# kahrendt/microWakeWord

Measured on AMD Instinct MI355X. Metric: spectrogram-windows/sec (train step) on default mixednet, higher is better.
Workload: dtype f32

## Files before the change

microwakeword_amd/csrc/block_launch.hip.h:

```cpp
#pragma once
#include "kernels_bwd.hip.h"

#define MWW_ODD_KS(X, CI, CO) X(CI, CO, 3) X(CI, CO, 5) X(CI, CO, 7) X(CI, CO, 9) X(CI, CO, 11) X(CI, CO, 13) X(CI, CO, 15) \
  X(CI, CO, 17) X(CI, CO, 19) X(CI, CO, 21) X(CI, CO, 23)
#define MWW_FIRST_KS(X, K1, CO, S) X(K1, 32, CO, 3, S) X(K1, 32, CO, 5, S) X(K1, 32, CO, 7, S)
#define MWW_FIRST_STRIDES(X, K1, CO) MWW_FIRST_KS(X, K1, CO, 1) MWW_FIRST_KS(X, K1, CO, 2) MWW_FIRST_KS(X, K1, CO, 3)
#ifdef MWW_SLIM
#define MWW_FIRST_SHAPES(X) X(3, 32, 48, 5, 1)
#define MWW_BLOCK_SHAPES(X) X(48, 48, 9) X(48, 48, 13) X(48, 48, 21)
#define MWW_FIRST_SHAPES_BF16(X) MWW_FIRST_SHAPES(X)
#define MWW_BLOCK_SHAPES_BF16(X) MWW_BLOCK_SHAPES(X)
#else
#define MWW_FIRST_SHAPES(X)                                                                                   \
  MWW_FIRST_STRIDES(X, 3, 32) MWW_FIRST_STRIDES(X, 3, 48) MWW_FIRST_STRIDES(X, 3, 64)                         \
  MWW_FIRST_STRIDES(X, 5, 32) MWW_FIRST_STRIDES(X, 5, 48) MWW_FIRST_STRIDES(X, 5, 64)
#define MWW_BLOCK_SHAPES(X)                                                                                   \
  MWW_ODD_KS(X, 32, 32) MWW_ODD_KS(X, 48, 48) MWW_ODD_KS(X, 64, 64) MWW_ODD_KS(X, 32, 48) MWW_ODD_KS(X, 32, 64)   \
  MWW_ODD_KS(X, 48, 64) MWW_ODD_KS(X, 48, 32) MWW_ODD_KS(X, 64, 48) MWW_ODD_KS(X, 64, 32)
#define MWW_FIRST_SHAPES_BF16(X) X(3, 32, 48, 5, 1) X(5, 32, 64, 5, 3) X(5, 32, 64, 5, 1) X(3, 32, 64, 5, 1) X(5, 32, 48, 5, 3) X(5, 32, 48, 5, 1)
#define MWW_BLOCK_SHAPES_BF16(X)                                                                              \
  X(48, 48, 5) X(48, 48, 9) X(48, 48, 13) X(48, 48, 21) X(48, 48, 11) X(48, 48, 15) X(48, 48, 23)             \
  X(64, 64, 11) X(64, 64, 15) X(64, 64, 23) X(64, 64, 5) X(64, 64, 9) X(64, 64, 13) X(64, 64, 21)
#endif

namespace mww {

bool k_launch_fwd_first(hipStream_t st, int mode, int k1, int c1, int cout, int k, int stride, const FwdFirstArgs& a, int grid, bool x6);
bool k_launch_fwd_block(hipStream_t st, int mode, int cin, int cout, int k, const FwdBlockArgs& a, int grid);
bool k_launch_bwd_first(hipStream_t st, int mode, int k1, int c1, int cout, int k, int stride, const BwdFirstArgs& a, int grid, bool x6);
bool k_launch_bwd_block(hipStream_t st, int mode, int cin, int cout, int k, bool last, const BwdBlockArgs& a, int grid);
bool k_launch_bwd_blockw(hipStream_t st, int mode, int cin, int cout, int k, bool last, const BwdBlockArgs& a, int grid);
bool k_launch_bwd_firstw(hipStream_t st, int k1, int c1, int cout, int k, int stride, const BwdFirstArgs& a, int grid, bool wide_x6);

}
```

microwakeword_amd/csrc/bwd_first_body.inc:

```
  constexpr int CIN = C1;
  constexpr int CPI = pitch(CIN), CPO = pitch(COUT);
  constexpr int RA = TT + K - 1;
  constexpr int TAIL = S > 1 ? K - 1 : 0;
  constexpr int TAILK = (TAIL + 3) / 4 * 4;
  constexpr int XR = (TT + TAILK - 1) * S + K1;
  constexpr int NT1 = C1 / 16;
  constexpr int M1 = K1 * FBINS;
  constexpr int MT1 = (M1 + 15) / 16;
  constexpr int MPW = (MT1 + 3) / 4;
  constexpr int MT = CIN / 16, NT = COUT / 16, KSO = COUT / 4;
  constexpr int NCH = nchunks(CIN), L = chunk_len(CIN);
  constexpr int QI = CIN / 4;
  constexpr int RAP = halo_rows_padded(CIN, K), TTP = tile_rows_padded(CIN);
  constexpr int OFF_A = 0, OFF_DP = OFF_A + RAP * CPI, OFF_U = OFF_DP + TT * CPO, OFF_DU = OFF_U + TTP * CPI;
  constexpr int PB = 96, PLB = XR * PB, GPB = 2 * CIN, GPL = TT * GPB;
  static_assert(!X6 || (S == 1 && CIN == 32 && (K1 * FBINS) % 8 == 0 && 3 * GPL <= (TT * CPO + TTP * CPI) * 4 && TTP == TT), "the x6 form serves the stride-1 first convolutions");
  constexpr int OFF_G0 = OFF_DU + RAP * CPI, OFF_END = X6 ? OFF_G0 : OFF_G0 + (TTP + TAILK) * CPI;
  static_assert(TAIL <= NCH && TTP + TAIL <= RAP, "tail rows");
  constexpr int PX = FBINS + 1;
  static_assert(OFF_END >= 4 * CIN * COUT && OFF_END >= NCH * (K + 1) * CIN, "scratch aliasing");
  static_assert(TT >= K - 1, "shape");

  float* sA = smem + OFF_A;
  float* sDP = smem + OFF_DP;
  float* sU = smem + OFF_U;
  float* sDU = smem + OFF_DU;
  float* sG0 = smem + OFF_G0;

  const int tid = threadIdx.x, lane = tid & 63, wave = tid >> 6, r16 = lane & 15, g = lane >> 4;
  const int c = tid % CIN, chunk = tid / CIN;
  const bool dw_active = chunk < NCH;
  const int Ta = (a.T - K1) / S + 1;

  const bool tailmode = TAIL > 0 && Ta > TT && Ta <= TT + TAIL;
  const int ntiles = tailmode ? 1 : (Ta + TT - 1) / TT;
  const int nsamp = (int)blockIdx.x < a.B ? (a.B - (int)blockIdx.x + (int)gridDim.x - 1) / (int)gridDim.x : 0;
  const int nitems = nsamp * ntiles;
  XStage<XR, PX, MWW_AUX_LD_XB> xs;
  DpStage<COUT, false, SB> dps;
  constexpr int NA = (RA * QI + kThreads - 1) / kThreads;
  float4 pre_a[NA];
  auto issue = [&](int it) {
    const int s = it / ntiles, b = blockIdx.x + s * gridDim.x, t0 = (it % ntiles) * TT;
    const int nrx = ((tailmode ? Ta : min(TT, Ta - t0)) - 1) * S + K1;
    xs.issue(a.x, a.xg, sXg, s, b, a.T, t0 * S, nrx, tid);
    const BufRsrc ra = tile_rsrc(a.a0 + ((size_t)b * Ta + t0) * CIN, min(RA, Ta - t0) * QI * 16);
#pragma unroll
    for (int j = 0; j < NA; ++j) pre_a[j] = tile_load4<MWW_AUX_LD_A0>(ra, (tid + j * kThreads) * 16);
    const int nvk = max(0, min(TT, a.Tout - t0)) * (COUT / 4);
    const size_t koff = ((size_t)b * a.Tout + t0) * COUT;
    dps.issue(elem_ptr<SB>(a.pk, koff), elem_ptr<SB>(a.gk, koff), nvk, tid);
  };
  int offm[MPW];
  bool okm[MPW];
  int xoff[MPW], goff[NT1];
  if constexpr (X6) {
    const int rowl = 4 * g + (r16 >> 2), cg = 4 * (r16 & 3);
#pragma unroll
    for (int mi = 0; mi < MPW; ++mi) {
      const int m = min((wave * MPW + mi) * 16 + cg, M1 - 4);
      xoff[mi] = (rowl + m / FBINS) * PB + (m % FBINS) * 2;
    }
#pragma unroll
    for (int nt = 0; nt < NT1; ++nt) goff[nt] = rowl * GPB + ((nt * 16 + cg) ^ ((rowl & 4) ? 16 : 0)) * 2;
  } else {
#pragma unroll
  for (int mi = 0; mi < MPW; ++mi) {
    const int m = (wave * MPW + mi) * 16 + r16;
    okm[mi] = m < M1;
    offm[mi] = okm[mi] ? (m / FBINS) * PX + (m % FBINS) : 0;
  }
  }
  if (a.xg.win) xgather_setup(a.xg, sXg, nsamp, tid);
  stagger_start<MWW_STAGGER_BWD>();
  if (nitems > 0) issue(0);

  WeightStage<CIN, COUT, 0, pitch_wt(CIN, BF)> wst;
  wst.load(a.pw_w, nullptr, tid);
  float dww[K], accw[K];
  float accb = 0.f, dwb = 0.f;
#pragma unroll
  for (int i = 0; i < K; ++i) {
    dww[i] = dw_active ? a.dw_w[i * CIN + c] : 0.f;
    accw[i] = 0.f;
  }
  if (dw_active) dwb = a.dw_b[c];
  for (int i = tid; i < COUT; i += kThreads) {
    const float krs = a.k_rstd[i];
    const float kmean = a.k_mean[i];
    float c1, mg, mgx;
    if (a.gfold.acc) {
      bn_grad_fold_channel(a.gfold, COUT, i, krs, c1, mg, mgx);
    } else {
      c1 = a.k_c1[i];
      mg = a.k_mg[i];
      mgx = a.k_mgx[i];
    }
    const float kA = -c1 * krs * mgx;
    sKp[0 * COUT + i] = c1;
    sKp[1 * COUT + i] = kA;
    sKp[2 * COUT + i] = -c1 * mg - kA * kmean;
    sKp[5 * COUT + i] = 0.f;
    sKp[6 * COUT + i] = 0.f;
  }
  wst.store(sWt, nullptr, tid);
  for (int i = RA * CPI + tid; i < RAP * CPI; i += kThreads) {
    sA[i] = 0.f;
    sDU[i] = 0.f;
  }
  if constexpr (!X6)
    for (int i = TTP * CPI + tid; i < (TTP + TAILK) * CPI; i += kThreads) sG0[i] = 0.f;
#pragma unroll
  for (int i = 0; i < K; ++i) pin(dww[i]);
  pin(dwb);
  f32x4 dwacc[MT][NT];
#pragma unroll
  for (int mt = 0; mt < MT; ++mt)
#pragma unroll
    for (int nt = 0; nt < NT; ++nt) dwacc[mt][nt] = zero4();
  f32x4 w1acc[MPW][NT1];
#pragma unroll
  for (int mi = 0; mi < MPW; ++mi)
#pragma unroll
    for (int nt = 0; nt < NT1; ++nt) w1acc[mi][nt] = zero4();
  __syncthreads();

  for (int it = 0; it < nitems; ++it) {
    rotate_priority(it, 2);
    const int t0 = (it % ntiles) * TT;
    const int nrows_new = max(0, min(TT, a.Tout - t0));
    const int rows_da = min(TT, Ta - t0);
    if constexpr (X6) xs.template commit_planes<PB, PLB>(reinterpret_cast<unsigned*>(sX), a.xg, sXg, it / ntiles, t0 * S, tid);
    else xs.commit(sX, a.xg, sXg, it / ntiles, t0 * S, tid);
#pragma unroll
    for (int j = 0; j < NA; ++j) {
      const int i = tid + j * kThreads;
      if (i < RA * QI) {
        const int r = i / QI, q = i - r * QI;
        *reinterpret_cast<float4*>(sA + r * CPI + q * 4) = pre_a[j];
      }
    }
    dps.commit(sDP, sKp, 0.f, nrows_new * (COUT / 4), tid);
    carry_du<K, CPI>(sDU, t0 == 0, tid);
    __syncthreads();
    if (it + 1 < nitems) issue(it + 1);
    if (dw_active) {
      if (chunk * L < nrows_new) {
        float o[L];
        dw_chunk<K, L>(sA, CPI, chunk * L, c, dww, dwb, o);
#pragma unroll
        for (int t = 0; t < L; ++t) {
          const int tl = chunk * L + t;
          sU[tl * CPI + c] = (tl < nrows_new) ? o[t] : 0.f;
        }
      } else {
#pragma unroll
        for (int t = 0; t < L; ++t) sU[(chunk * L + t) * CPI + c] = 0.f;
      }
    }
    __syncthreads();
    pointwise_backward_tile<CIN, COUT, K, BF>(sU, sDP, sDU, wave, r16, g, sWt, dwacc, wave * 16 < nrows_new);
    __syncthreads();
    if (dw_active) {
      float wdu[L + K - 1], wa[L + K - 1];
#pragma unroll
      for (int j = 0; j < L + K - 1; ++j) wdu[j] = sDU[(chunk * L + j) * CPI + c];
#pragma unroll
      for (int j = 0; j < L + K - 1; ++j) wa[j] = sA[(chunk * L + j) * CPI + c];
      lds_reads_first();
#pragma unroll
      for (int t = 0; t < L; ++t) {
        const int sl = chunk * L + t;
        float acc = 0.f;
#pragma unroll
        for (int i = 0; i < K; ++i) acc = fmaf(dww[K - 1 - i], wdu[t + i], acc);
        const float gv = (sl < rows_da && wa[t] > 0.f) ? acc : 0.f;
        if constexpr (X6) {
          unsigned h0, h1, h2;
          split3(gv, h0, h1, h2);
          unsigned short* gp = reinterpret_cast<unsigned short*>(sDP) + sl * CIN + (c ^ ((sl & 4) ? 16 : 0));
          gp[0] = (unsigned short)(h0 >> 16);
          gp[GPL / 2] = (unsigned short)(h1 >> 16);
          gp[GPL] = (unsigned short)(h2 >> 16);
        } else {
          sG0[sl * CPI + c] = gv;
        }
      }
      if (chunk * L < nrows_new) {
#pragma unroll
        for (int t = 0; t < L; ++t) {
          const float dut = wdu[K - 1 + t];
          accb += dut;
#pragma unroll
          for (int i = 0; i < K; ++i) accw[i] = fmaf(dut, wa[t + i], accw[i]);
        }
      }
      if constexpr (TAIL > 0) {
        if (tailmode && chunk < TAIL) {
          const int sl = TT + chunk;
          float acc = 0.f;
#pragma unroll
          for (int j = 0; j < K; ++j) acc = fmaf(dww[K - 1 - j], sl + j < RAP ? sDU[(sl + j) * CPI + c] : 0.f, acc);
          sG0[sl * CPI + c] = (sl < Ta && sA[sl * CPI + c] > 0.f) ? acc : 0.f;
        }
      }
    }
    __syncthreads();
    if constexpr (X6) {
      const char* xb = reinterpret_cast<const char*>(sX);
      const char* gb = reinterpret_cast<const char*>(sDP);
#pragma unroll
      for (int kb = 0; kb < TT / 32; ++kb)
#pragma unroll
        for (int nt = 0; nt < NT1; ++nt) {
          u32x4v gq[3];
#pragma unroll
          for (int p = 0; p < 3; ++p) {
            const u32x2v lo = lds_read_tr16(gb + goff[nt] + p * GPL + (32 * kb) * GPB), hi = lds_read_tr16(gb + goff[nt] + p * GPL + (32 * kb + 16) * GPB);
            gq[p] = u32x4v{lo.x, lo.y, hi.x, hi.y};
          }
#pragma unroll
          for (int mi = 0; mi < MPW; ++mi) {
            u32x4v xq[3];
#pragma unroll
            for (int p = 0; p < 3; ++p) {
              const u32x2v lo = lds_read_tr16(xb + xoff[mi] + p * PLB + (32 * kb) * S * PB), hi = lds_read_tr16(xb + xoff[mi] + p * PLB + (32 * kb + 16) * S * PB);
              xq[p] = u32x4v{lo.x, lo.y, hi.x, hi.y};
            }
            w1acc[mi][nt] = mfma_x6(xq, gq, w1acc[mi][nt]);
          }
        }
    } else {
      float av[2][MPW], bv[2][NT1];
      auto load_w1 = [&](int kk, int sl) {
        const int s = kk * 4 + g;
#pragma unroll
        for (int nt = 0; nt < NT1; ++nt) bv[sl][nt] = sG0[s * CPI + nt * 16 + r16];
#pragma unroll
        for (int mi = 0; mi < MPW; ++mi) {
          const float v = sX[s * S * PX + offm[mi]];
          av[sl][mi] = okm[mi] ? v : 0.f;
        }
      };
      load_w1(0, 0);
#pragma unroll
      for (int kk = 0; kk < TT / 4; ++kk) {
        if (kk + 1 < TT / 4) load_w1(kk + 1, (kk + 1) & 1);
#pragma unroll
        for (int mi = 0; mi < MPW; ++mi)
#pragma unroll
          for (int nt = 0; nt < NT1; ++nt) w1acc[mi][nt] = mfma4(av[kk & 1][mi], bv[kk & 1][nt], w1acc[mi][nt]);
      }
      __builtin_amdgcn_sched_group_barrier(0x100, MPW + NT1, 0);
      sched_read_mfma_groups<TT / 4 - 1, MPW + NT1, MPW * NT1>();
      sched_read_mfma_groups<1, 0, MPW * NT1>();
      if constexpr (TAIL > 0) {
        if (tailmode) {
#pragma unroll
          for (int ks = 0; ks < TAILK / 4; ++ks) {
            load_w1(TT / 4 + ks, 0);
#pragma unroll
            for (int mi = 0; mi < MPW; ++mi)
#pragma unroll
              for (int nt = 0; nt < NT1; ++nt) w1acc[mi][nt] = mfma4(av[0][mi], bv[0][nt], w1acc[mi][nt]);
          }
        }
      }
    }
    __syncthreads();
  }
  float* gdst = a.grad_part + (size_t)blockIdx.x * (M1 * C1 + (K + 1) * CIN + CIN * COUT);
#pragma unroll
  for (int mi = 0; mi < MPW; ++mi)
#pragma unroll
    for (int nt = 0; nt < NT1; ++nt)
#pragma unroll
      for (int r = 0; r < 4; ++r) {
        const int m = (wave * MPW + mi) * 16 + g * 4 + r;
        if (m < M1) gdst[m * C1 + nt * 16 + r16] = w1acc[mi][nt][r];
      }
  write_block_grad_partials<CIN, COUT, K>(smem, gdst + M1 * C1, dwacc, accw, accb, dw_active, c, chunk, tid, wave, r16, g);
```

microwakeword_amd/csrc/common.hip.h:

```cpp
#pragma once
#include <hip/hip_runtime.h>
#include <stdint.h>

namespace mww {

typedef float f32x4 __attribute__((ext_vector_type(4)));

constexpr int kThreads = 256;
constexpr int TT = 64;
constexpr int FBINS = 40;
constexpr float kBnEps = 1e-3f;
constexpr float kBnMomentum = 0.99f;
constexpr float kKerasEps = 1e-7f;

constexpr int kHeadTraining = 1, kHeadClippedLoss = 2;
__device__ __forceinline__ float bce_value(float z, float pr, float yy, bool clipped_form) {
  if (!clipped_form) return fmaxf(z, 0.f) - z * yy + log1pf(expf(-fabsf(z)));
  const float pc = fminf(fmaxf(pr, kKerasEps), 1.0f - kKerasEps);
  return -(yy * logf(pc) + (1.0f - yy) * logf(1.0f - pc));
}
__device__ __forceinline__ float bce_dz(float pr, float yy, bool clipped_form) {
  if (clipped_form && ((pr < kKerasEps) || (pr > 1.0f - kKerasEps))) return 0.f;
  return pr - yy;
}

__device__ __forceinline__ f32x4 mfma4(float a, float b, f32x4 c) {
  return __builtin_amdgcn_mfma_f32_16x16x4f32(a, b, c, 0, 0, 0);
}

typedef __bf16 bf16x4 __attribute__((ext_vector_type(4)));
typedef short s16x4 __attribute__((ext_vector_type(4)));

__device__ __forceinline__ f32x4 mfma_bf16(bf16x4 a, bf16x4 b, f32x4 c) {
  return __builtin_amdgcn_mfma_f32_16x16x16bf16_1k(__builtin_bit_cast(s16x4, a), __builtin_bit_cast(s16x4, b), c, 0, 0, 0);
}

__device__ __forceinline__ bf16x4 to_bf16x4(float a, float b, float c, float d) {
  bf16x4 v = {(__bf16)a, (__bf16)b, (__bf16)c, (__bf16)d};
  return v;
}

typedef __bf16 bf16x8 __attribute__((ext_vector_type(8)));
typedef unsigned u32x4v __attribute__((ext_vector_type(4)));
typedef unsigned u32x2v __attribute__((ext_vector_type(2)));
__device__ __forceinline__ f32x4 mfma_bf16k32(u32x4v a, u32x4v b, f32x4 c) {
  return __builtin_amdgcn_mfma_f32_16x16x32_bf16(__builtin_bit_cast(bf16x8, a), __builtin_bit_cast(bf16x8, b), c, 0, 0, 0);
}
__device__ __forceinline__ void split3(float v, unsigned& h0, unsigned& h1, unsigned& h2) {
  h0 = __float_as_uint(v) & 0xffff0000u;
  const float r1 = v - __uint_as_float(h0);
  h1 = __float_as_uint(r1) & 0xffff0000u;
  const float r2 = r1 - __uint_as_float(h1);
  h2 = __float_as_uint(r2) & 0xffff0000u;
}
__device__ __forceinline__ unsigned pack_hi2(unsigned a, unsigned b) { return (a >> 16) | b; }
__device__ __forceinline__ void split3x8(const float (&v)[8], u32x4v (&q)[3]) {
  unsigned h[3][8];
#pragma unroll
  for (int e = 0; e < 8; ++e) split3(v[e], h[0][e], h[1][e], h[2][e]);
#pragma unroll
  for (int p = 0; p < 3; ++p)
#pragma unroll
    for (int d = 0; d < 4; ++d) q[p][d] = pack_hi2(h[p][2 * d], h[p][2 * d + 1]);
}
__device__ __forceinline__ f32x4 mfma_x6(const u32x4v (&xs)[3], const u32x4v (&ws)[3], f32x4 acc) {
  acc = mfma_bf16k32(xs[2], ws[0], acc);
  acc = mfma_bf16k32(xs[1], ws[1], acc);
  acc = mfma_bf16k32(xs[0], ws[2], acc);
  acc = mfma_bf16k32(xs[1], ws[0], acc);
  acc = mfma_bf16k32(xs[0], ws[1], acc);
  acc = mfma_bf16k32(xs[0], ws[0], acc);
  return acc;
}
__device__ __forceinline__ void pin4(u32x4v& v) { asm volatile("" : "+v"(v)); }
__device__ __forceinline__ u32x2v lds_read_tr16(const void* lds_ptr) {
  typedef short s16x4t __attribute__((ext_vector_type(4)));
  const s16x4t v = __builtin_amdgcn_ds_read_tr16_b64_v4i16((__attribute__((address_space(3))) s16x4t*)(lds_ptr));
  return __builtin_bit_cast(u32x2v, v);
}

__device__ __forceinline__ f32x4 zero4() {
  f32x4 z = {0.f, 0.f, 0.f, 0.f};
  return z;
}

__host__ __device__ constexpr int pitch(int c) { return c + 4; }
#ifndef MWW_FWD_PITCH_A
#define MWW_FWD_PITCH_A 1
#endif
#ifndef MWW_FWD_PITCH_U
#define MWW_FWD_PITCH_U 1
#endif
__host__ __device__ constexpr int pitch_fa(int c) { return (MWW_FWD_PITCH_A && c == 48) ? 48 : c + 4; }
__host__ __device__ constexpr int pitch_fu(int c, bool bf) { return (MWW_FWD_PITCH_U && !bf) ? c + 2 : c + 4; }

__host__ __device__ constexpr int pitch_wt(int c, bool bf) { return bf ? c + 4 : (c % 32 == 16 ? c : c + 16); }

__host__ __device__ constexpr int nchunks(int c) { return kThreads / c; }
__host__ __device__ constexpr int chunk_len(int c) { return (TT + nchunks(c) - 1) / nchunks(c); }
__host__ __device__ constexpr int tile_rows_padded(int c) { return nchunks(c) * chunk_len(c); }
__host__ __device__ constexpr int halo_rows_padded(int c, int k) { return tile_rows_padded(c) + k - 1; }

typedef __amdgpu_buffer_rsrc_t BufRsrc;
typedef unsigned u32x4 __attribute__((ext_vector_type(4)));
typedef unsigned u32x2 __attribute__((ext_vector_type(2)));

__device__ __forceinline__ BufRsrc tile_rsrc(const void* base, int bytes) {
  const int n = __builtin_amdgcn_readfirstlane(bytes > 0 ? bytes : 0);
  return __builtin_amdgcn_make_buffer_rsrc(const_cast<void*>(base), (short)0, n, 0x00020000);
}
#ifndef MWW_AUX_ST_P
#define MWW_AUX_ST_P 16
#endif
#ifndef MWW_AUX_ST_G
#define MWW_AUX_ST_G 16
#endif
#ifndef MWW_AUX_ST_A0
#define MWW_AUX_ST_A0 2
#endif
#ifndef MWW_AUX_LD_FP
#define MWW_AUX_LD_FP 0
#endif
#ifndef MWW_AUX_LD_BP
#define MWW_AUX_LD_BP 2
#endif
#ifndef MWW_AUX_LD_A0
#define MWW_AUX_LD_A0 2
#endif
#ifndef MWW_AUX_LD_PK
#define MWW_AUX_LD_PK 2
#endif
#ifndef MWW_AUX_LD_GK
#define MWW_AUX_LD_GK 2
#endif
#ifndef MWW_AUX_LD_XF
#define MWW_AUX_LD_XF 0
#endif
#ifndef MWW_AUX_LD_XB
#define MWW_AUX_LD_XB 0
#endif
#ifndef MWW_AUX_LD_HP
#define MWW_AUX_LD_HP 0
#endif
#ifndef MWW_AUX_ST_GP
#define MWW_AUX_ST_GP 1
#endif
#ifndef MWW_AUX_GR_ST_P
#define MWW_AUX_GR_ST_P 1
#endif
#ifndef MWW_AUX_GR_ST_G
#define MWW_AUX_GR_ST_G 0
#endif
#ifndef MWW_AUX_GR_LD_GOLD
#define MWW_AUX_GR_LD_GOLD 0
#endif
#ifndef MWW_AUX_GR_ST_GP
#define MWW_AUX_GR_ST_GP 0
#endif
#ifndef MWW_AUX_GR_LD_DP
#define MWW_AUX_GR_LD_DP 0
#endif
template <int WT>
__device__ __forceinline__ void store_stream(float* p, float v) {
  if constexpr (WT != 0) __hip_atomic_store(p, v, __ATOMIC_RELAXED, __HIP_MEMORY_SCOPE_AGENT);
  else *p = v;
}
template <int AUX = 0>
__device__ __forceinline__ float4 tile_load4(BufRsrc r, int byte_off) {
  const u32x4 v = __builtin_amdgcn_raw_buffer_load_b128(r, byte_off, 0, AUX);
  return make_float4(__uint_as_float(v.x), __uint_as_float(v.y), __uint_as_float(v.z), __uint_as_float(v.w));
}
template <int AUX = 0>
__device__ __forceinline__ uint2 tile_load2(BufRsrc r, int byte_off) {
  const u32x2 v = __builtin_amdgcn_raw_buffer_load_b64(r, byte_off, 0, AUX);
  uint2 o;
  o.x = v.x;
  o.y = v.y;
  return o;
}
template <int AUX = 0>
__device__ __forceinline__ float tile_load1(BufRsrc r, int byte_off) {
  return __uint_as_float(__builtin_amdgcn_raw_buffer_load_b32(r, byte_off, 0, AUX));
}
template <int AUX = 0>
__device__ __forceinline__ void tile_store1(BufRsrc r, int byte_off, float v) {
  __builtin_amdgcn_raw_buffer_store_b32(__float_as_uint(v), r, byte_off, 0, AUX);
}
template <bool SB, int AUX = 0>
__device__ __forceinline__ float4 tile_load4s(BufRsrc r, int group) {
  if constexpr (!SB) {
    return tile_load4<AUX>(r, group * 16);
  } else {
    const uint2 v = tile_load2<AUX>(r, group * 8);
    return make_float4(__uint_as_float(v.x << 16), __uint_as_float(v.x & 0xffff0000u), __uint_as_float(v.y << 16),
                       __uint_as_float(v.y & 0xffff0000u));
  }
}
template <bool SB, int AUX = 0>
__device__ __forceinline__ void tile_store1s(BufRsrc r, int elem, float v) {
  if constexpr (!SB) {
    tile_store1<AUX>(r, elem * 4, v);
  } else {
    const __bf16 h = (__bf16)v;
    __builtin_amdgcn_raw_buffer_store_b16(__builtin_bit_cast(unsigned short, h), r, elem * 2, 0, AUX);
  }
}
template <bool SB>
__device__ __forceinline__ float load_elem(const float* base, size_t elem) {
  if constexpr (!SB) {
    return base[elem];
  } else {
    const unsigned dw = reinterpret_cast<const unsigned*>(base)[elem >> 1];
    return __uint_as_float((elem & 1) ? (dw & 0xffff0000u) : (dw << 16));
  }
}
__host__ __device__ constexpr int elem_bytes(bool sb) { return sb ? 2 : 4; }
template <bool SB>
__device__ __forceinline__ const float* elem_ptr(const float* base, size_t elem) {
  return reinterpret_cast<const float*>(reinterpret_cast<const char*>(base) + elem * (SB ? 2 : 4));
}
template <bool SB>
__device__ __forceinline__ float* elem_ptr(float* base, size_t elem) {
  return reinterpret_cast<float*>(reinterpret_cast<char*>(base) + elem * (SB ? 2 : 4));
}

constexpr int kOobOffset = 0x40000000;

__device__ __forceinline__ void lds_reads_first() {
  __builtin_amdgcn_sched_group_barrier(0x100, 64, 0);
  __builtin_amdgcn_sched_group_barrier(0x002, 2048, 0);
}

__device__ __forceinline__ void rotate_priority(int item, int levels) {
  const int p = ((int)(blockIdx.x >> 8) + item) & (levels - 1);
  if (levels == 2) {
    if (p) __builtin_amdgcn_s_setprio(1);
    else __builtin_amdgcn_s_setprio(0);
  } else {
    if (p == 0) __builtin_amdgcn_s_setprio(0);
    else if (p == 1) __builtin_amdgcn_s_setprio(1);
    else if (p == 2) __builtin_amdgcn_s_setprio(2);
    else __builtin_amdgcn_s_setprio(3);
  }
}

#ifndef MWW_STAGGER_BWD
#define MWW_STAGGER_BWD 47
#endif
#ifndef MWW_STAGGER_FWD
#define MWW_STAGGER_FWD 0
#endif
#ifndef MWW_STAGGER_GRAPH
#define MWW_STAGGER_GRAPH 0
#endif
#ifndef MWW_G_FWD_DIRECT
#define MWW_G_FWD_DIRECT 1
#endif
#ifndef MWW_G_WGRAD_EVEN
#define MWW_G_WGRAD_EVEN 1
#endif
#ifndef MWW_G_STEM_BREG
#define MWW_G_STEM_BREG 0
#endif
#ifndef MWW_G_WGRAD_XG_NARROW
#define MWW_G_WGRAD_XG_NARROW 0
#endif
template <int UNITS>
__device__ __forceinline__ void stagger_start() {
  if constexpr (UNITS > 0) {
    const int pos = (int)(blockIdx.x >> 8);
    for (int i = 0; i < pos; ++i) __builtin_amdgcn_s_sleep(UNITS);
  }
}

__device__ __forceinline__ void pin(float& v) { asm volatile("" : "+v"(v)); }
__device__ __forceinline__ void pin(int& v) { asm volatile("" : "+v"(v)); }

#ifdef MWW_PROFILE
#define MWW_ABLATE(a, bits) ((a).ablate & (bits))
#else
#define MWW_ABLATE(a, bits) 0
#endif
#ifdef MWW_PROFILE
#define MWW_PC_DECL PhaseClock pc;
#define MWW_PC_START(en) pc.start(en)
#define MWW_PC_MARK(i) pc.mark(i)
#define MWW_PC_DUMP(p) do { if (p) pc.dump(p); } while (0)
#define MWW_PC_AT(i) pc.at(i)
#else
#define MWW_PC_AT(i) ((void)0)
#define MWW_PC_DECL
#define MWW_PC_START(en) ((void)0)
#define MWW_PC_MARK(i) ((void)0)
#define MWW_PC_DUMP(p) ((void)0)
#endif
constexpr int kClkSlots = 12;
struct PhaseClock {
  unsigned long long last = 0, acc[8] = {0, 0, 0, 0, 0, 0, 0, 0}, stamp[4] = {0, 0, 0, 0};
  bool on = false;
  __device__ __forceinline__ void at(int i) { stamp[i] = __builtin_amdgcn_s_memtime(); }
  __device__ __forceinline__ void start(bool enable) {
    on = enable;
    if (on) last = __builtin_amdgcn_s_memtime();
  }
  __device__ __forceinline__ void mark(int slot) {
    if (on) {
      const unsigned long long t = __builtin_amdgcn_s_memtime();
      acc[slot] += t - last;
      last = t;
    }
  }
  __device__ __forceinline__ void dump(unsigned long long* dst) const {
    if (on) {
      for (int i = 0; i < 8; ++i) dst[i] = acc[i];
      for (int i = 0; i < 4; ++i) dst[8 + i] = stamp[i];
    }
  }
};

__device__ __forceinline__ void fast_divmod(int a, int b, int& q, int& r) {
  q = (int)((float)a * __frcp_rn((float)b));
  r = a - q * b;
  if (r >= b) {
    ++q;
    r -= b;
  } else if (r < 0) {
    --q;
    r += b;
  }
}
__device__ __forceinline__ int fast_div(int a, int b) {
  int q, r;
  fast_divmod(a, b, q, r);
  return q;
}

__device__ __forceinline__ int uniform_int(int v) { return __builtin_amdgcn_readfirstlane(v); }
__device__ __forceinline__ long long uniform_i64(long long v) {
  const unsigned lo = (unsigned)__builtin_amdgcn_readfirstlane((int)(unsigned)(unsigned long long)v);
  const unsigned hi = (unsigned)__builtin_amdgcn_readfirstlane((int)(unsigned)((unsigned long long)v >> 32));
  return (long long)(((unsigned long long)hi << 32) | lo);
}
__device__ __forceinline__ const void* uniform_ptr(const void* p) {
  return reinterpret_cast<const void*>((uintptr_t)uniform_i64((long long)(uintptr_t)p));
}

__device__ __forceinline__ float sum_over_groups(float v) {
  v += __shfl_xor(v, 16);
  v += __shfl_xor(v, 32);
  return v;
}

__device__ __forceinline__ float wave_sum(float v) {
  v += __shfl_xor(v, 1);
  v += __shfl_xor(v, 2);
  v += __shfl_xor(v, 4);
  v += __shfl_xor(v, 8);
  v += __shfl_xor(v, 16);
  v += __shfl_xor(v, 32);
  return v;
}

constexpr int kStatRows = 8;

struct StatAcc {
  double* acc;
  double* clear;
};

__device__ __forceinline__ void publish_stat(const StatAcc& s, float* row, int C2, int tid, float v) {
  if (s.acc) {
    unsafeAtomicAdd(s.acc + (size_t)(blockIdx.x % kStatRows) * C2 + tid, (double)v);
    for (int r = blockIdx.x; r < kStatRows; r += gridDim.x)
      __hip_atomic_store(s.clear + (size_t)r * C2 + tid, 0.0, __ATOMIC_RELAXED, __HIP_MEMORY_SCOPE_AGENT);
  } else {
    row[tid] = v;
  }
}

struct BnFoldArgs {
  const double* acc;
  float inv_n;
  int update_moving;
  const float* gamma;
  const float* beta;
  float* moving_mean;
  float* moving_var;
  float* scale;
  float* shift;
  float* mean;
  float* rstd;
};

__device__ __forceinline__ void bn_fold_channel(const BnFoldArgs& f, int C, int ch, float& sc, float& sh, float& meanf, float& rstd) {
  double s1 = 0.0, s2 = 0.0;
  double v1[kStatRows], v2[kStatRows];
#pragma unroll
  for (int j = 0; j < kStatRows; ++j) {
    v1[j] = f.acc[(size_t)j * 2 * C + ch];
    v2[j] = f.acc[(size_t)j * 2 * C + C + ch];
  }
  const float gam = f.gamma[ch], bet = f.beta[ch];
  float mm_old = 0.f, mv_old = 0.f;
  if (blockIdx.x == 0 && f.update_moving) {
    mm_old = f.moving_mean[ch];
    mv_old = f.moving_var[ch];
  }
#pragma unroll
  for (int j = 0; j < kStatRows; ++j) {
    s1 += v1[j];
    s2 += v2[j];
  }
  const double m = s1 * (double)f.inv_n;
  double var = s2 * (double)f.inv_n - m * m;
  if (var < 0.0) var = 0.0;
  meanf = (float)m;
  const float varf = (float)var;
  rstd = 1.0f / sqrtf(varf + kBnEps);
  sc = gam * rstd;
  sh = bet - meanf * sc;
  if (blockIdx.x == 0) {
    f.scale[ch] = sc;
    f.shift[ch] = sh;
    f.mean[ch] = meanf;
    f.rstd[ch] = rstd;
    if (f.update_moving) {
      f.moving_mean[ch] = mm_old * kBnMomentum + meanf * (1.0f - kBnMomentum);
      f.moving_var[ch] = mv_old * kBnMomentum + varf * (1.0f - kBnMomentum);
    }
  }
}

struct BnGradFoldArgs {
  const double* acc;
  float inv_n;
  float dscale;
  const float* gamma;
  float* c1;
  float* mg;
  float* mgx;
  float* dgamma;
  float* dbeta;
};

__device__ __forceinline__ void bn_grad_fold_channel(const BnGradFoldArgs& f, int C, int ch, float rstd, float& c1, float& mg, float& mgx) {
  double s1 = 0.0, s2 = 0.0;
  double v1[kStatRows], v2[kStatRows];
#pragma unroll
  for (int j = 0; j < kStatRows; ++j) {
    v1[j] = f.acc[(size_t)j * 2 * C + ch];
    v2[j] = f.acc[(size_t)j * 2 * C + C + ch];
  }
  const float gam = f.gamma[ch];
#pragma unroll
  for (int j = 0; j < kStatRows; ++j) {
    s1 += v1[j];
    s2 += v2[j];
  }
  c1 = gam * rstd;
  mg = (float)(s1 * (double)f.inv_n);
  mgx = (float)(s2 * (double)f.inv_n);
  if (blockIdx.x == 0) {
    f.dbeta[ch] = (float)s1 * f.dscale;
    f.dgamma[ch] = (float)s2 * f.dscale;
    f.c1[ch] = c1;
    f.mg[ch] = mg;
    f.mgx[ch] = mgx;
  }
}

}
```

microwakeword_amd/csrc/engine.hip.h:

```cpp
#pragma once
#include <hip/hip_runtime.h>

#include <map>
#include <string>
#include <utility>
#include <vector>

#include "../../include/mww.h"
#include "kernels_bwd.hip.h"
#include "kernels_data.hip.h"

#ifndef MWW_CONV1_X6_DEFAULT
#define MWW_CONV1_X6_DEFAULT 1
#endif
#ifndef MWW_CONV1_X6_FWD_DEFAULT
#define MWW_CONV1_X6_FWD_DEFAULT 0
#endif
#ifndef MWW_BWD_FIRST_WIDE_DEFAULT
#define MWW_BWD_FIRST_WIDE_DEFAULT 0
#endif
#ifndef MWW_BWD_WIDE_DEFAULT
#define MWW_BWD_WIDE_DEFAULT 1
#endif

namespace mww {

struct MetricState;

int fail(int code, const std::string& msg);

#define HIPCHK(expr)                                                                              \
  do {                                                                                            \
    hipError_t e_ = (expr);                                                                       \
    if (e_ != hipSuccess)                                                                         \
      return fail(MWW_ERR_HIP, std::string(#expr) + ": " + hipGetErrorString(e_));                \
  } while (0)

struct Layer {
  int cin, cout, k, tin, tout;
  int64_t o_dw_w, o_dw_b, o_pw_w, o_gamma, o_beta, o_mm, o_mv;
  float* p = nullptr;
  float* g = nullptr;
  float* stat_part = nullptr;
  float* gstat_part = nullptr;
  float* grad_part = nullptr;
  int grad_part_stride = 0;
  float* bn = nullptr;
  double* facc[2] = {nullptr, nullptr};
  double* gacc[2] = {nullptr, nullptr};
  double* facc_cur = nullptr;
  double* gacc_cur = nullptr;
};

struct GOp {
  int n_src = 0, src[MWW_MAX_OP_SOURCES] = {0, 0, 0}, toff[MWW_MAX_OP_SOURCES] = {0, 0, 0};
  int sc0[MWW_MAX_OP_SOURCES] = {0, 0, 0}, scn[MWW_MAX_OP_SOURCES] = {0, 0, 0};
  bool src_first[MWW_MAX_OP_SOURCES] = {false, false, false}, src_last[MWW_MAX_OP_SOURCES] = {false, false, false};
  int k = 1, dil = 1, cin = 0, cout = 0, groups = 1, slots = 0, tin = 0, tout = 0;
  int kind = MWW_OP_CONV, stride = 1, norm = MWW_NORM_BN, act = MWW_ACT_RELU;
  int res_src = -1, res_drop = 0;
  std::vector<int> adders;
  int64_t o_w = 0, o_gamma = 0, o_beta = 0, o_mm = 0, o_mv = 0;
  float *p = nullptr, *g = nullptr, *stat_part = nullptr, *gstat_part = nullptr, *grad_part = nullptr, *bn = nullptr;
  bool needs_dx = false;
  bool twin_next = false;
  int planes = 1, pc = 0;
  size_t lds_fwd = 0, lds_dx = 0, lds_wg = 0;
  double* facc[2] = {nullptr, nullptr};
  double* gacc[2] = {nullptr, nullptr};
  double* facc_cur = nullptr;
  double* gacc_cur = nullptr;
  int first_consumer = -1;
};

struct ProfileEntry {
  std::string name;
  hipEvent_t a, b;
};

struct RcclApi {
  void* so = nullptr;
  struct UniqueId { char internal[128]; };
  int (*GetUniqueId)(UniqueId*) = nullptr;
  int (*CommInitRank)(void**, int, UniqueId, int) = nullptr;
  int (*AllReduce)(const void*, void*, size_t, int, int, void*, hipStream_t) = nullptr;
  int (*CommDestroy)(void*) = nullptr;
  int (*CommCount)(void*, int*) = nullptr;
  const char* (*GetErrorString)(int) = nullptr;
};

constexpr int kRing = 8;
constexpr int kDenseChunks = 32;

}

struct mww_ctx {
  mww_mixednet_desc d;
  int device = 0;
  hipStream_t stream = nullptr;
  bool own_stream = false;
  int n_cu = 256;
  int grid_fwd = 0, grid_bwd = 0, grid_head = 0;
  bool conv1_x6 = MWW_CONV1_X6_DEFAULT != 0;
  bool conv1_x6_fwd = MWW_CONV1_X6_FWD_DEFAULT != 0;
  bool bwd_first_wide = MWW_BWD_FIRST_WIDE_DEFAULT != 0;
  bool bwd_wide = MWW_BWD_WIDE_DEFAULT != 0;
  int64_t P = 0, S = 0;
  int64_t o_conv1 = 0, o_dense_w = 0, o_dense_b = 0;
  int t_last = 0, c_last = 0, dwd_stride = 0;
  std::vector<mww::Layer> L;
  bool generic = false;
  std::vector<mww::GOp> G;
  float dropout = 0.f;
  float* keep = nullptr;
  bool keep_explicit = false;
  unsigned long long dropout_seed = 0x5EEDull, dropout_counter = 0;
  bool head2 = false;
  bool head_att = false;
  int head_pool = 0;
  int64_t o_att = 0;
  float *hact = nullptr, *watt_part = nullptr;
  size_t lds_head2 = 0;
  float *ones = nullptr, *zeros = nullptr;
  int grid_g = 0;
  int g_cap_fwd = 4, g_cap_bwd = 4;
  int metric_launches = 0;
  bool g_planar = true;
  bool g_static = true;
  int g_chunks = 0;
  int g_dgrad_share = 50;
  bool grid_g_auto = true;
  std::map<std::pair<const void*, size_t>, int> g_occ;
  mww_allreduce_fn hook = nullptr;
  void* hook_user = nullptr;
  int world = 1;
  bool sync_bn = false, reduce_grads = false;
  struct RcclState* rccl = nullptr;
  float* sync_buf = nullptr;
  std::vector<int64_t> sync_off;
  float *params = nullptr, *grads = nullptr, *adam_m = nullptr, *adam_v = nullptr, *mask = nullptr;
  unsigned char* direct = nullptr;
  std::vector<unsigned char> direct_host;
  bool exchange_pending = false;
  int grad_buckets = 1;
  float* bn_state = nullptr;
  float *x = nullptr, *y = nullptr, *sw = nullptr, *z = nullptr, *prob = nullptr, *dz = nullptr, *loss_part = nullptr;
  float* a0 = nullptr;
  float* gbuf[2] = {nullptr, nullptr};
  float* dwd_part = nullptr;
  mww::MetricState* metrics = nullptr;
  char* mail_host[mww::kRing] = {};
  char* mail_dev[mww::kRing] = {};
  hipEvent_t mail_ev[mww::kRing] = {};
  int mail_cur = 0;
  bool mail_open = false;
  size_t mail_off_masks = 0, mail_off_y = 0, mail_off_sw = 0, mail_off_hyper = 0, mail_bytes = 0;
  int targets_in_mail = 0;
  hipStream_t copy_stream = nullptr;
  char* mail_hbm[mww::kRing] = {};
  hipEvent_t ev_copy[mww::kRing] = {};
  hipStream_t side = nullptr;
  hipEvent_t ev_fork = nullptr, ev_join = nullptr;
  bool side_pending = false;
  int asm_split = 2;
  bool fused_input = true;
  bool x_lazy = false;
  int lazy_slot = -1;
  mww::AssembleArgs lazy_a;
  const float* y_cur = nullptr;
  const float* sw_cur = nullptr;
  bool bn_inline = true;
  bool g_role_split = true;
  bool g_inline_ok = false;
  int fpar = 0, gpar = 0;
  bool tail_pending = false, tail_metrics = false;
  bool tail_in_reduce = false;
  bool tail_roles = true;
  void* store[MWW_MAX_STORES] = {};
  int store_dtype[MWW_MAX_STORES] = {};
  int64_t store_elems[MWW_MAX_STORES] = {};
  int64_t step = 0;
  int have_batch = 0, have_targets = 0;
  bool use_graphs = false, profile = false;
  bool profile_split = false;
  bool use_side = false;
  bool pw_bf16 = false;
  bool st_bf16 = false;
  bool bce_clipped = false;
  bool bn_eval_ready = false;
  int ablate = 0;
  unsigned long long* phase_clk = nullptr;
  std::vector<mww::ProfileEntry> prof;
  struct GraphEntry { int B, flags, mail, par; hipGraphExec_t exec; };
  std::vector<GraphEntry> graphs;
};

namespace mww {

struct Launcher {
  mww_ctx* c;
  hipEvent_t ea = nullptr;
  const char* name = nullptr;
  size_t idx = 0;
  void begin(const char* n, int layer = -1) {
    if (!c->profile) return;
    name = n;
    idx = c->prof.size();
    ProfileEntry e;
    e.name = n;
    if (layer >= 0) e.name += std::to_string(layer + 1);
    (void)hipEventCreate(&e.a);
    (void)hipEventCreate(&e.b);
    (void)hipEventRecord(e.a, c->stream);
    c->prof.push_back(e);
  }
  void end() {
    if (!c->profile || idx >= c->prof.size()) return;
    (void)hipEventRecord(c->prof[idx].b, c->stream);
  }
};

enum { BN_SCALE = 0, BN_SHIFT, BN_MEAN, BN_RSTD, BN_C1, BN_MG, BN_MGX };

const float* mail_hyper(mww_ctx* c);
int materialise_x(mww_ctx* c);
XGather x_gather(mww_ctx* c);
int enqueue_side_work(mww_ctx* c, int B, bool metrics, bool loss, const float* p_last, const float* scale, const float* shift, const float* keep);
struct StatSource { const float* part; int G; float inv_n; float dscale; };
int exchange_stats(mww_ctx* c, Launcher& lp, const char* what, int layer, const float* part, int G, int C, int bwd, float local_inv_n, StatSource* out);
int enqueue_grad_assembly(mww_ctx* c, int B, GradReduceArgs& ga, bool fuse_adam, int64_t lo = 0, int64_t hi = -1, bool last_range = true);

constexpr size_t kMaxDynLds = 144 * 1024;
constexpr long long kPlanePad = 1088;
int g_planes(const mww_ctx* c, const GOp& o);
long long g_pstride(const mww_ctx* c, const GOp& o);
bool g_stem_gathers(const mww_ctx* c);
struct GPlan {
  std::vector<GOp> ops;
  int64_t P = 0, S = 0;
  bool inline_ok = false;
  int chunks = 0;
};
int g_plan_convnet(const mww_convnet_desc& d, GPlan* plan);
int g_enqueue_forward(mww_ctx* c, int B, bool training, bool update_moving, bool loss, bool metrics);
int g_enqueue_backward(mww_ctx* c, int B, bool fuse_adam);

}
```

microwakeword_amd/csrc/kernels_bwd.hip.h:

```cpp
#pragma once
#include "kernels_fwd.hip.h"

namespace mww {

struct BwdBlockArgs {
  const float* in;
  const float* in_scale;
  const float* in_shift;
  const float* in_mean;
  const float* in_rstd;
  const float* pk;
  const float* gk;
  const float* k_mean;
  const float* k_rstd;
  const float* k_c1;
  const float* k_mg;
  const float* k_mgx;
  const float* k_scale;
  const float* k_shift;
  const float* wd;
  const float* dz;
  const float* dw_w;
  const float* dw_b;
  const float* pw_w;
  float* g_out;
  float* gstat_part;
  float* grad_part;
  int B, Tin, Tout;
  int ablate;
  unsigned long long* phase_clk;
  StatAcc gacc;
  BnGradFoldArgs gfold;
};

template <int COUT, bool LAST, bool SB = false>
struct DpStage {
  static constexpr int QO = COUT / 4, CPO = pitch(COUT), N = (TT * QO + kThreads - 1) / kThreads;
  float4 pk[N], gg[N];

  __device__ __forceinline__ void issue(const float* pk_base, const float* g_base, int nvalid, int tid) {
    constexpr bool SG = SB && !LAST;
    const BufRsrc rp = tile_rsrc(pk_base, nvalid * 4 * elem_bytes(SB)), rg = tile_rsrc(g_base, nvalid * 4 * elem_bytes(SG));
#pragma unroll
    for (int j = 0; j < N; ++j) {
      pk[j] = tile_load4s<SB, MWW_AUX_LD_PK>(rp, tid + j * kThreads);
      gg[j] = tile_load4s<SG, MWW_AUX_LD_GK>(rg, tid + j * kThreads);
    }
  }

  __device__ __forceinline__ void commit(float* sDP, const float* sKp, float dzb, int nvalid, int tid) const {
#pragma unroll
    for (int j = 0; j < N; ++j) {
      const int i = tid + j * kThreads;
      if (i < TT * QO) {
        const int r = i / QO, q = i - r * QO;
        float4 dp = make_float4(0.f, 0.f, 0.f, 0.f);
        if (i < nvalid) {
          const float4 p = pk[j];
          const float4 c1 = *reinterpret_cast<const float4*>(sKp + 0 * COUT + q * 4);
          const float4 kA = *reinterpret_cast<const float4*>(sKp + 1 * COUT + q * 4);
          const float4 kB = *reinterpret_cast<const float4*>(sKp + 2 * COUT + q * 4);
          float4 g = gg[j];
          if (LAST) {
            const float4 sc = *reinterpret_cast<const float4*>(sKp + 5 * COUT + q * 4);
            const float4 sh = *reinterpret_cast<const float4*>(sKp + 6 * COUT + q * 4);
            g.x = fmaf(p.x, sc.x, sh.x) > 0.f ? dzb * g.x : 0.f;
            g.y = fmaf(p.y, sc.y, sh.y) > 0.f ? dzb * g.y : 0.f;
            g.z = fmaf(p.z, sc.z, sh.z) > 0.f ? dzb * g.z : 0.f;
            g.w = fmaf(p.w, sc.w, sh.w) > 0.f ? dzb * g.w : 0.f;
          }
          dp.x = fmaf(g.x, c1.x, fmaf(p.x, kA.x, kB.x));
          dp.y = fmaf(g.y, c1.y, fmaf(p.y, kA.y, kB.y));
          dp.z = fmaf(g.z, c1.z, fmaf(p.z, kA.z, kB.z));
          dp.w = fmaf(g.w, c1.w, fmaf(p.w, kA.w, kB.w));
        }
        *reinterpret_cast<float4*>(sDP + r * CPO + q * 4) = dp;
      }
    }
  }
};

template <int CIN, int COUT, int KD, int PWT = pitch(CIN)>
struct WeightStage {
  static constexpr int CPI = PWT, NW = (CIN * COUT + kThreads - 1) / kThreads, ND = KD > 0 ? (KD * CIN + kThreads - 1) / kThreads : 1;
  float w[NW], d[ND];
  __device__ __forceinline__ void load(const float* pw_w, const float* dw_w, int tid) {
#pragma unroll
    for (int j = 0; j < NW; ++j) w[j] = (tid + j * kThreads < CIN * COUT) ? pw_w[tid + j * kThreads] : 0.f;
#pragma unroll
    for (int j = 0; j < ND; ++j) d[j] = (KD > 0 && tid + j * kThreads < KD * CIN) ? dw_w[tid + j * kThreads] : 0.f;
  }
  __device__ __forceinline__ void store(float* sWt, float* sDW, int tid) const {
#pragma unroll
    for (int j = 0; j < NW; ++j) {
      const int i = tid + j * kThreads;
      if (i < CIN * COUT) sWt[(i % COUT) * CPI + i / COUT] = w[j];
    }
    if (KD > 0) {
#pragma unroll
      for (int j = 0; j < ND; ++j)
        if (tid + j * kThreads < KD * CIN) sDW[tid + j * kThreads] = d[j];
    }
  }
};

template <int K, int CPI>
__device__ __forceinline__ void carry_du(float* sDU, bool first_tile, int tid) {
  for (int i = tid; i < (K - 1) * CPI; i += kThreads) sDU[i] = first_tile ? 0.f : sDU[TT * CPI + i];
}

template <int REPS, int READS, int MFMAS>
__device__ __forceinline__ void sched_read_mfma_groups() {
  if constexpr (REPS > 0) {
    if constexpr (READS > 0) __builtin_amdgcn_sched_group_barrier(0x100, READS, 0);
    __builtin_amdgcn_sched_group_barrier(0x008, MFMAS, 0);
    sched_read_mfma_groups<REPS - 1, READS, MFMAS>();
  }
}

template <int CIN, int COUT, int K, bool BF>
__device__ __forceinline__ void pointwise_backward_tile(const float* sU, const float* sDP, float* sDU, int wave, int r16,
                                                        int g, const float* sWt,
                                                        f32x4 (&dwacc)[CIN / 16][COUT / 16], bool live) {
  constexpr int CPI = pitch(CIN), CPO = pitch(COUT), MT = CIN / 16, NT = COUT / 16, KSO = COUT / 4;
  constexpr int PWT = pitch_wt(CIN, BF);
  f32x4 du[MT];
#pragma unroll
  for (int mt = 0; mt < MT; ++mt) du[mt] = zero4();
  if (!live) {
  } else if constexpr (!BF) {
    {
      float av[2][MT], bv[2][NT];
      auto load_dw = [&](int kk, int s) {
        const int row = wave * 16 + kk + 4 * g;
#pragma unroll
        for (int mt = 0; mt < MT; ++mt) av[s][mt] = sU[row * CPI + mt * 16 + r16];
#pragma unroll
        for (int nt = 0; nt < NT; ++nt) bv[s][nt] = sDP[row * CPO + nt * 16 + r16];
      };
      float a2[2], b2[2][MT];
      auto load_du = [&](int kk, int s) {
        a2[s] = sDP[(wave * 16 + r16) * CPO + kk * 4 + g];
#pragma unroll
        for (int mt = 0; mt < MT; ++mt) b2[s][mt] = sWt[(kk * 4 + g) * PWT + mt * 16 + r16];
      };
      load_dw(0, 0);
#pragma unroll
      for (int kk = 0; kk < 4; ++kk) {
        if (kk + 1 < 4) load_dw(kk + 1, (kk + 1) & 1);
        else load_du(0, 0);
#pragma unroll
        for (int mt = 0; mt < MT; ++mt)
#pragma unroll
          for (int nt = 0; nt < NT; ++nt) dwacc[mt][nt] = mfma4(av[kk & 1][mt], bv[kk & 1][nt], dwacc[mt][nt]);
      }
#pragma unroll
      for (int kk = 0; kk < KSO; ++kk) {
        if (kk + 1 < KSO) load_du(kk + 1, (kk + 1) & 1);
#pragma unroll
        for (int mt = 0; mt < MT; ++mt) du[mt] = mfma4(a2[kk & 1], b2[kk & 1][mt], du[mt]);
      }
      __builtin_amdgcn_sched_group_barrier(0x100, MT + NT, 0);
      sched_read_mfma_groups<3, MT + NT, MT * NT>();
      sched_read_mfma_groups<1, 1 + MT, MT * NT>();
      sched_read_mfma_groups<KSO - 1, 1 + MT, MT>();
      sched_read_mfma_groups<1, 0, MT>();
    }
  } else {
    const int row = wave * 16 + 4 * g;
    bf16x4 av[MT], bv[NT];
#pragma unroll
    for (int mt = 0; mt < MT; ++mt) {
      const float* col = sU + row * CPI + mt * 16 + r16;
      av[mt] = to_bf16x4(col[0], col[CPI], col[2 * CPI], col[3 * CPI]);
    }
#pragma unroll
    for (int nt = 0; nt < NT; ++nt) {
      const float* col = sDP + row * CPO + nt * 16 + r16;
      bv[nt] = to_bf16x4(col[0], col[CPO], col[2 * CPO], col[3 * CPO]);
    }
#pragma unroll
    for (int mt = 0; mt < MT; ++mt)
#pragma unroll
      for (int nt = 0; nt < NT; ++nt) dwacc[mt][nt] = mfma_bf16(av[mt], bv[nt], dwacc[mt][nt]);
#pragma unroll
    for (int kk = 0; kk < COUT / 16; ++kk) {
      const float4 v = *reinterpret_cast<const float4*>(sDP + (wave * 16 + r16) * CPO + kk * 16 + 4 * g);
      const bf16x4 a4 = to_bf16x4(v.x, v.y, v.z, v.w);
#pragma unroll
      for (int mt = 0; mt < MT; ++mt) {
        const float* col = sWt + (kk * 16 + 4 * g) * PWT + mt * 16 + r16;
        du[mt] = mfma_bf16(a4, to_bf16x4(col[0], col[PWT], col[2 * PWT], col[3 * PWT]), du[mt]);
      }
    }
  }
#pragma unroll
  for (int mt = 0; mt < MT; ++mt)
#pragma unroll
    for (int r = 0; r < 4; ++r) sDU[(K - 1 + wave * 16 + g * 4 + r) * CPI + mt * 16 + r16] = du[mt][r];
}

template <int CIN, int COUT, int K>
__device__ __forceinline__ void write_block_grad_partials(float* scratch, float* dst, const f32x4 (&dwacc)[CIN / 16][COUT / 16],
                                                          const float (&accw)[K], float accb, bool dw_active, int c,
                                                          int chunk, int tid, int wave, int r16, int g) {
  constexpr int MT = CIN / 16, NT = COUT / 16, NCH = nchunks(CIN);
  __syncthreads();
#pragma unroll
  for (int mt = 0; mt < MT; ++mt)
#pragma unroll
    for (int nt = 0; nt < NT; ++nt)
#pragma unroll
      for (int r = 0; r < 4; ++r)
        scratch[(wave * CIN + mt * 16 + g * 4 + r) * COUT + nt * 16 + r16] = dwacc[mt][nt][r];
  __syncthreads();
  for (int e = tid; e < CIN * COUT; e += kThreads)
    store_stream<MWW_AUX_ST_GP>(dst + (K + 1) * CIN + e, (scratch[e] + scratch[CIN * COUT + e]) + (scratch[2 * CIN * COUT + e] + scratch[3 * CIN * COUT + e]));
  __syncthreads();
  if (dw_active) {
#pragma unroll
    for (int i = 0; i < K; ++i) scratch[(chunk * (K + 1) + i) * CIN + c] = accw[i];
    scratch[(chunk * (K + 1) + K) * CIN + c] = accb;
  }
  __syncthreads();
  for (int e = tid; e < (K + 1) * CIN; e += kThreads) {
    float v = 0.f;
#pragma unroll
    for (int j = 0; j < NCH; ++j) v += scratch[j * (K + 1) * CIN + e];
    store_stream<MWW_AUX_ST_GP>(dst + e, v);
  }
  __syncthreads();
}


template <int CIN, int COUT, int K>
struct BwdBlockLds {
  static constexpr int CPI = pitch(CIN), CPO = pitch(COUT);
  static constexpr int RAP = halo_rows_padded(CIN, K), TTP = tile_rows_padded(CIN);
  static constexpr int OFF_END = RAP * CPI + TT * CPO + TTP * CPI + RAP * CPI;
  static constexpr int up4(int v) { return (v + 3) / 4 * 4; }
  static constexpr int KP = OFF_END, WT = KP + up4(7 * COUT), DW = WT + COUT * pitch_wt(CIN, false), ACT = DW + up4(K * CIN), END = ACT + 2 * CIN;
};
template <int K1, int C1, int COUT, int K, int S>
struct BwdFirstLds {
  static constexpr int CIN = C1, CPI = pitch(CIN), CPO = pitch(COUT);
  static constexpr int RAP = halo_rows_padded(CIN, K), TTP = tile_rows_padded(CIN);
  static constexpr int TAIL = S > 1 ? K - 1 : 0;
  static constexpr int TAILK = (TAIL + 3) / 4 * 4;
  static constexpr int OFF_END = RAP * CPI + TT * CPO + TTP * CPI + RAP * CPI + (TTP + TAILK) * CPI;
  static constexpr int XR = (TT + TAILK - 1) * S + K1, PX = FBINS + 1;
  static constexpr int up4(int v) { return (v + 3) / 4 * 4; }
  static constexpr int KP = OFF_END, WT = KP + up4(7 * COUT), X = WT + COUT * pitch_wt(CIN, false), XG = X + up4(XR * PX);
  static constexpr int END = XG + up4((int)(sizeof(XShared) + 3) / 4);
};

template <int CIN, int COUT, int K, bool LAST, bool BF, bool SB = false>
__global__ __launch_bounds__(kThreads, ((CIN > 48 || BwdBlockLds<CIN, COUT, K>::END * 4 > 80 * 1024) ? 1 : 2)) void bwd_block_kernel(BwdBlockArgs a) {
  typedef BwdBlockLds<CIN, COUT, K> Lds;
  __shared__ __attribute__((aligned(16))) float smem[Lds::OFF_END];
  __shared__ __attribute__((aligned(16))) float sKp[7 * COUT];
  __shared__ __attribute__((aligned(16))) float sWt[COUT * pitch_wt(CIN, BF)];
  __shared__ __attribute__((aligned(16))) float sDW[K * CIN];
  __shared__ __attribute__((aligned(16))) float sAct[2 * CIN];
#include "bwd_block_body.inc"
}

struct BwdFirstArgs {
  const float* x;
  const float* a0;
  const float* pk;
  const float* gk;
  const float* k_mean;
  const float* k_rstd;
  const float* k_c1;
  const float* k_mg;
  const float* k_mgx;
  const float* dw_w;
  const float* dw_b;
  const float* pw_w;
  float* grad_part;
  int B, T, Tout;
  BnGradFoldArgs gfold;
  XGather xg;
};

template <int K1, int C1, int COUT, int K, int S, bool BF, bool SB = false, bool X6 = false>
__global__ __launch_bounds__(kThreads, (S > 1 ? 1 : 2)) void bwd_first_kernel(BwdFirstArgs a) {
  typedef BwdFirstLds<K1, C1, COUT, K, S> Lds;
  __shared__ __attribute__((aligned(16))) float sX[X6 ? 3 * Lds::XR * 96 / 4 : Lds::XR * Lds::PX];
  __shared__ XShared sXg;
  __shared__ __attribute__((aligned(16))) float smem[X6 ? Lds::OFF_END - (Lds::TTP + Lds::TAILK) * Lds::CPI : Lds::OFF_END];
  __shared__ __attribute__((aligned(16))) float sKp[7 * COUT];
  __shared__ __attribute__((aligned(16))) float sWt[COUT * pitch_wt(C1, BF)];
#include "bwd_first_body.inc"
}

struct BnBwdFinalizeArgs {
  const float* gstat_part;
  int G, C;
  float inv_n;
  const float* gamma;
  const float* rstd;
  float* c1;
  float* mg;
  float* mgx;
  float* dgamma;
  float* dbeta;
  float dscale;
};

__device__ __forceinline__ void bn_bwd_finalize_body(const BnBwdFinalizeArgs& a, int c, double* sAcc, double* sOut, int tid) {
  float gam = 0.f, rs = 0.f;
  if (tid == 0) {
    gam = a.gamma[c];
    rs = a.rstd[c];
  }
  const double r = reduce_partials_256(a.gstat_part, a.G, a.C, c, sAcc, tid);
  if ((tid & 127) == 0) sOut[tid >> 7] = r;
  __syncthreads();
  if (tid == 0) {
    const double s1 = sOut[0], s2 = sOut[1];
    a.dbeta[c] = (float)s1 * a.dscale;
    a.dgamma[c] = (float)s2 * a.dscale;
    a.c1[c] = gam * rs;
    a.mg[c] = (float)(s1 * (double)a.inv_n);
    a.mgx[c] = (float)(s2 * (double)a.inv_n);
  }
}

#ifndef MWW_BLOCK_TU
__global__ __launch_bounds__(kThreads) void bn_bwd_finalize_kernel(BnBwdFinalizeArgs a) {
  __shared__ __attribute__((aligned(16))) double sAcc[256 + 16];
  __shared__ double sOut[2];
  bn_bwd_finalize_body(a, blockIdx.x, sAcc, sOut, threadIdx.x);
}
#endif

struct GradSegment {
  const float* part;
  int G;
  int stride;
  int n;
  int dst;
};
constexpr int kMaxSegments = 112;
struct GradReduceArgs {
  GradSegment seg[kMaxSegments];
  int nseg;
};

struct AdamArgs {
  float* param;
  const float* grad;
  float* m;
  float* v;
  const float* hyper;
  int P;
  float beta1, beta2, eps;
};

#ifndef MWW_BLOCK_TU
__global__ __launch_bounds__(kThreads) void adam_kernel(AdamArgs a) {
  const int p = blockIdx.x * kThreads + threadIdx.x;
  if (p >= a.P) return;
  const float alpha = a.hyper[0];
  const float gg = a.grad[p] * a.hyper[1];
  float m = a.m[p], v = a.v[p];
  m += (gg - m) * (1.0f - a.beta1);
  v += (gg * gg - v) * (1.0f - a.beta2);
  a.m[p] = m;
  a.v[p] = v;
  a.param[p] -= alpha * m / (sqrtf(v) + a.eps);
}
#endif

}
```

microwakeword_amd/csrc/kernels_bwdw.hip.h:

```cpp
#pragma once
#include "kernels_bwd.hip.h"

#ifndef MWW_WIDE_RELANE_K
#define MWW_WIDE_RELANE_K 15
#endif
#ifndef MWW_WIDE_TWO_GROUPS_UPTO
#define MWW_WIDE_TWO_GROUPS_UPTO 19
#endif

namespace mww {

template <int C, int NTH>
struct WidePitch;
template <>
struct WidePitch<48, 512> {
  static constexpr int P = 48, D = 1, PW = 52;
};
template <>
struct WidePitch<64, 512> {
  static constexpr int P = 72, D = 2, PW = 68;
};

template <int C, bool LAST, bool SB, int NTH, int P>
struct DpStageW {
  static constexpr int Q = C / 4, N = (TT * Q + NTH - 1) / NTH;
  float4 pk[N], gg[N];

  __device__ __forceinline__ void issue(const float* pk_base, const float* g_base, int nvalid, int tid) {
    constexpr bool SG = SB && !LAST;
    const BufRsrc rp = tile_rsrc(pk_base, nvalid * 4 * elem_bytes(SB)), rg = tile_rsrc(g_base, nvalid * 4 * elem_bytes(SG));
#pragma unroll
    for (int j = 0; j < N; ++j) {
      pk[j] = tile_load4s<SB, MWW_AUX_LD_PK>(rp, tid + j * NTH);
      gg[j] = tile_load4s<SG, MWW_AUX_LD_GK>(rg, tid + j * NTH);
    }
  }

  __device__ __forceinline__ void commit(float* sDP, const float* sKp, float dzb, int nvalid, int tid) const {
#pragma unroll
    for (int j = 0; j < N; ++j) {
      const int i = tid + j * NTH;
      if (i < TT * Q) {
        const int r = i / Q, q = i - r * Q;
        float4 dp = make_float4(0.f, 0.f, 0.f, 0.f);
        if (i < nvalid) {
          const float4 p = pk[j];
          const float4 c1 = *reinterpret_cast<const float4*>(sKp + 0 * C + q * 4);
          const float4 kA = *reinterpret_cast<const float4*>(sKp + 1 * C + q * 4);
          const float4 kB = *reinterpret_cast<const float4*>(sKp + 2 * C + q * 4);
          float4 g = gg[j];
          if (LAST) {
            const float4 sc = *reinterpret_cast<const float4*>(sKp + 5 * C + q * 4);
            const float4 sh = *reinterpret_cast<const float4*>(sKp + 6 * C + q * 4);
            g.x = fmaf(p.x, sc.x, sh.x) > 0.f ? dzb * g.x : 0.f;
            g.y = fmaf(p.y, sc.y, sh.y) > 0.f ? dzb * g.y : 0.f;
            g.z = fmaf(p.z, sc.z, sh.z) > 0.f ? dzb * g.z : 0.f;
            g.w = fmaf(p.w, sc.w, sh.w) > 0.f ? dzb * g.w : 0.f;
          }
          dp.x = fmaf(g.x, c1.x, fmaf(p.x, kA.x, kB.x));
          dp.y = fmaf(g.y, c1.y, fmaf(p.y, kA.y, kB.y));
          dp.z = fmaf(g.z, c1.z, fmaf(p.z, kA.z, kB.z));
          dp.w = fmaf(g.w, c1.w, fmaf(p.w, kA.w, kB.w));
        }
        *reinterpret_cast<float4*>(sDP + r * P + q * 4) = dp;
      }
    }
  }
};

template <int NTW, int NBLK, int BLK, int D, int PA, int PB = PA>
__device__ __forceinline__ void wide_dw_rows(const float* sU, const float* sDP, int row0, int nrows, int mcol, int ncol0,
                                             int r16, int g, f32x4 (&acc)[NTW]) {
  constexpr int KSB = BLK / 4;
  static_assert(BLK % (4 * D) == 0, "a block holds whole groups of 4 D rows");
  const float* pu = sU + (row0 + D * g) * PA + mcol + r16;
  const float* pd = sDP + (row0 + D * g) * PB + ncol0 + r16;
#pragma unroll
  for (int blk = 0; blk < NBLK; ++blk) {
    if (row0 + blk * BLK < nrows) {
      float av[2], bv[2][NTW];
      auto ld = [&](int kk, int s) {
        const int ro = blk * BLK + (kk / D) * 4 * D + (kk % D);
        av[s] = pu[ro * PA];
#pragma unroll
        for (int nt = 0; nt < NTW; ++nt) bv[s][nt] = pd[ro * PB + nt * 16];
      };
      ld(0, 0);
#pragma unroll
      for (int kk = 0; kk < KSB; ++kk) {
        if (kk + 1 < KSB) ld(kk + 1, (kk + 1) & 1);
#pragma unroll
        for (int nt = 0; nt < NTW; ++nt) acc[nt] = mfma4(av[kk & 1], bv[kk & 1][nt], acc[nt]);
      }
      __builtin_amdgcn_sched_group_barrier(0x100, 1 + NTW, 0);
      sched_read_mfma_groups<KSB - 1, 1 + NTW, NTW>();
      sched_read_mfma_groups<1, 0, NTW>();
    }
  }
}

template <int C, int NMU, int K, int P, int PW, int PD = P>
__device__ __forceinline__ void wide_du_tiles(const float* sDP, const float* sWt, float* sDU, int rt, int nrows, int mcol0,
                                              int r16, int g) {
  f32x4 du[NMU];
#pragma unroll
  for (int mu = 0; mu < NMU; ++mu) du[mu] = zero4();
  if (rt * 16 < nrows) {
    const float* pa = sDP + (rt * 16 + r16) * P + 4 * g;
    const float* pb = sWt + (4 * g) * PW + mcol0 + r16;
    float4 a4[2];
    a4[0] = *reinterpret_cast<const float4*>(pa);
#pragma unroll
    for (int kb = 0; kb < C / 16; ++kb) {
      if (kb + 1 < C / 16) a4[(kb + 1) & 1] = *reinterpret_cast<const float4*>(pa + (kb + 1) * 16);
      float bv[4][NMU];
#pragma unroll
      for (int s = 0; s < 4; ++s)
#pragma unroll
        for (int mu = 0; mu < NMU; ++mu) bv[s][mu] = pb[(kb * 16 + s) * PW + mu * 16];
      const float4 av = a4[kb & 1];
      const float as[4] = {av.x, av.y, av.z, av.w};
#pragma unroll
      for (int s = 0; s < 4; ++s)
#pragma unroll
        for (int mu = 0; mu < NMU; ++mu) du[mu] = mfma4(as[s], bv[s][mu], du[mu]);
    }
  }
  float* pd = sDU + (K - 1 + rt * 16 + g * 4) * PD + mcol0 + r16;
#pragma unroll
  for (int mu = 0; mu < NMU; ++mu)
#pragma unroll
    for (int r = 0; r < 4; ++r) pd[r * PD + mu * 16] = du[mu][r];
}

template <int NTW, int NBLK, int PA, int PB = PA>
__device__ __forceinline__ void wide_dw_rows_bf16(const float* sU, const float* sDP, int row0, int nrows, int mcol, int ncol0,
                                                  int r16, int g, f32x4 (&acc)[NTW]) {
  const float* pu = sU + (row0 + g) * PA + mcol + r16;
  const float* pd = sDP + (row0 + g) * PB + ncol0 + r16;
#pragma unroll
  for (int blk = 0; blk < NBLK; ++blk) {
    if (row0 + blk * 16 < nrows) {
      const float* cu = pu + blk * 16 * PA;
      const bf16x4 av = to_bf16x4(cu[0], cu[4 * PA], cu[8 * PA], cu[12 * PA]);
      bf16x4 bv[NTW];
#pragma unroll
      for (int nt = 0; nt < NTW; ++nt) {
        const float* cd = pd + blk * 16 * PB + nt * 16;
        bv[nt] = to_bf16x4(cd[0], cd[4 * PB], cd[8 * PB], cd[12 * PB]);
      }
#pragma unroll
      for (int nt = 0; nt < NTW; ++nt) acc[nt] = mfma_bf16(av, bv[nt], acc[nt]);
    }
  }
}

template <int C, int NMU, int K, int P, int PW, int PD = P>
__device__ __forceinline__ void wide_du_tiles_bf16(const float* sDP, const float* sWt, float* sDU, int rt, int nrows, int mcol0,
                                                   int r16, int g) {
  f32x4 du[NMU];
#pragma unroll
  for (int mu = 0; mu < NMU; ++mu) du[mu] = zero4();
  if (rt * 16 < nrows) {
    const float* pa = sDP + (rt * 16 + r16) * P + 4 * g;
    const float* pb = sWt + (4 * g) * PW + mcol0 + r16;
#pragma unroll
    for (int kb = 0; kb < C / 16; ++kb) {
      const float4 v = *reinterpret_cast<const float4*>(pa + kb * 16);
      const bf16x4 a4 = to_bf16x4(v.x, v.y, v.z, v.w);
#pragma unroll
      for (int mu = 0; mu < NMU; ++mu) {
        const float* col = pb + kb * 16 * PW + mu * 16;
        du[mu] = mfma_bf16(a4, to_bf16x4(col[0], col[PW], col[2 * PW], col[3 * PW]), du[mu]);
      }
    }
  }
  float* pd = sDU + (K - 1 + rt * 16 + g * 4) * PD + mcol0 + r16;
#pragma unroll
  for (int mu = 0; mu < NMU; ++mu)
#pragma unroll
    for (int r = 0; r < 4; ++r) pd[r * PD + mu * 16] = du[mu][r];
}

template <int K, int L, int I0, int I1, bool REV>
__device__ __forceinline__ void dw_tap_group(const float* src_c, int pitch, const float* taps_c, int tap_pitch, float (&acc)[L]) {
  constexpr int N = I1 - I0;
  float win[L + N - 1], w[N];
#pragma unroll
  for (int j = 0; j < L + N - 1; ++j) win[j] = src_c[(I0 + j) * pitch];
#pragma unroll
  for (int i = 0; i < N; ++i) w[i] = taps_c[(REV ? K - 1 - (I0 + i) : I0 + i) * tap_pitch];
#ifndef MWW_WIDE_NOREADSFIRST
  lds_reads_first();
#endif
#pragma unroll
  for (int t = 0; t < L; ++t)
#pragma unroll
    for (int i = 0; i < N; ++i) acc[t] = fmaf(w[i], win[t + i], acc[t]);
}
template <int K, int L, int I0, int I1>
__device__ __forceinline__ void dw_wgrad_group(const float* src_c, int pitch, const float (&du)[L], float (&accw)[K]) {
  constexpr int N = I1 - I0;
  float win[L + N - 1];
#pragma unroll
  for (int j = 0; j < L + N - 1; ++j) win[j] = src_c[(I0 + j) * pitch];
#ifndef MWW_WIDE_NOREADSFIRST
  lds_reads_first();
#endif
#pragma unroll
  for (int t = 0; t < L; ++t)
#pragma unroll
    for (int i = 0; i < N; ++i) accw[I0 + i] = fmaf(du[t], win[t + i], accw[I0 + i]);
}
template <int K>
struct TapGroups {
#ifdef MWW_WIDE_FEWGROUPS
  static constexpr int N = K <= 15 ? 1 : 2;
#else
  static constexpr int N = K <= 11 ? 1 : (K <= MWW_WIDE_TWO_GROUPS_UPTO ? 2 : 3);
#endif
  static constexpr int lo(int gidx) { return gidx * K / N; }
};
template <int K, int L, bool REV, int G = 0>
__device__ __forceinline__ void dw_all_groups(const float* src_c, int pitch, const float* taps_c, int tap_pitch, float (&acc)[L]) {
  if constexpr (G < TapGroups<K>::N) {
    dw_tap_group<K, L, TapGroups<K>::lo(G), TapGroups<K>::lo(G + 1), REV>(src_c, pitch, taps_c, tap_pitch, acc);
    if constexpr (G + 1 < TapGroups<K>::N) __builtin_amdgcn_sched_barrier(0);
    dw_all_groups<K, L, REV, G + 1>(src_c, pitch, taps_c, tap_pitch, acc);
  }
}
template <int K, int L, int G = 0>
__device__ __forceinline__ void dw_wgrad_all_groups(const float* src_c, int pitch, const float (&du)[L], float (&accw)[K]) {
  if constexpr (G < TapGroups<K>::N) {
    dw_wgrad_group<K, L, TapGroups<K>::lo(G), TapGroups<K>::lo(G + 1)>(src_c, pitch, du, accw);
    if constexpr (G + 1 < TapGroups<K>::N) __builtin_amdgcn_sched_barrier(0);
    dw_wgrad_all_groups<K, L, G + 1>(src_c, pitch, du, accw);
  }
}

template <int C, int NW>
struct WideRoles;
template <>
struct WideRoles<48, 8> {
  static constexpr int NTW = 3, NPART = 2;
  static __device__ __forceinline__ bool has_dw(int w) { return w < 6; }
  static __device__ __forceinline__ int part(int w) { return w / 3; }
  static __device__ __forceinline__ int mt(int w) { return w % 3; }
  static __device__ __forceinline__ int nt0(int) { return 0; }
};
template <>
struct WideRoles<64, 8> {
  static constexpr int NTW = 2, NPART = 1;
  static __device__ __forceinline__ bool has_dw(int) { return true; }
  static __device__ __forceinline__ int part(int) { return 0; }
  static __device__ __forceinline__ int mt(int w) { return w / 2; }
  static __device__ __forceinline__ int nt0(int w) { return 2 * (w % 2); }
};

template <int C, int K, int NTH>
struct BwdWideLds {
  typedef WidePitch<C, NTH> WP;
  static constexpr int NCH = NTH / C, L = (TT + NCH - 1) / NCH, TTP = NCH * L, RAP = TTP + K - 1;
  static constexpr int OFF_P = 0, OFF_DP = OFF_P + RAP * WP::P, OFF_U = OFF_DP + TT * WP::P, OFF_DU = OFF_U + TTP * WP::P;
  static constexpr int OFF_END = OFF_DU + RAP * WP::P;
  static constexpr int BYTES = (OFF_END + 7 * C + C * WP::PW + K * C + 2 * C) * 4;
};

template <int C, int K, int NTH>
constexpr int wide_waves_per_simd() {
  return (BwdWideLds<C, K, NTH>::BYTES <= 80 * 1024 ? 2 : 1) * (NTH / 64) / 4;
}

template <int CIN, int COUT, int K, bool LAST, int NTH, bool BF = false, bool SB = false>
__global__ __launch_bounds__(NTH, (wide_waves_per_simd<CIN, K, NTH>())) void bwd_blockw_kernel(BwdBlockArgs a) {
  static_assert(CIN == COUT, "the wide form is instantiated for square blocks");
  constexpr int C = CIN;
  typedef WidePitch<C, NTH> WP;
  typedef BwdWideLds<C, K, NTH> Lds;
  constexpr int NW = NTH / 64;
  typedef WideRoles<C, NW> Roles;
  constexpr int P = WP::P, PW = WP::PW, D = WP::D;
  constexpr int NCH = Lds::NCH, L = Lds::L, TTP = Lds::TTP, RA = TT + K - 1, RAP = Lds::RAP;
  constexpr int Q = C / 4, MT = C / 16;
  static_assert(NCH * L >= TT && TT >= K - 1, "tile geometry");
  static_assert(Lds::OFF_END >= Roles::NPART * C * C && Lds::OFF_END >= NCH * (K + 1) * C, "scratch aliasing");

  __shared__ __attribute__((aligned(16))) float smem[Lds::OFF_END];
  __shared__ __attribute__((aligned(16))) float sKp[7 * C];
  __shared__ __attribute__((aligned(16))) float sWt[C * PW];
  __shared__ __attribute__((aligned(16))) float sDW[K * C];
  __shared__ __attribute__((aligned(16))) float sAct[2 * C];
  float* sP = smem + Lds::OFF_P;
  float* sDP = smem + Lds::OFF_DP;
  float* sU = smem + Lds::OFF_U;
  float* sDU = smem + Lds::OFF_DU;

  const int tid = threadIdx.x, lane = tid & 63, wave = __builtin_amdgcn_readfirstlane(tid >> 6), r16_ = lane & 15, g_ = lane >> 4;
  const int c = tid % C, chunk = tid / C;
  const bool dw_active = chunk < NCH;
  MWW_PC_DECL
  MWW_PC_AT(0);

  const int ntiles = (a.Tin + TT - 1) / TT;
  const int nsamp = (int)blockIdx.x < a.B ? (a.B - (int)blockIdx.x + (int)gridDim.x - 1) / (int)gridDim.x : 0;
  const int nitems = nsamp * ntiles;
  constexpr int NP = (RA * Q + NTH - 1) / NTH;
  float4 pre_p[NP];
  DpStageW<C, LAST, SB, NTH, P> dps;
  float pre_dz = 0.f;
  auto issue = [&](int it) {
    const int b = blockIdx.x + (it / ntiles) * gridDim.x, t0 = (it % ntiles) * TT;
    const int nvp = min(RA, a.Tin - t0) * Q;
    const BufRsrc src = tile_rsrc(elem_ptr<SB>(a.in, ((size_t)b * a.Tin + t0) * C), nvp * 4 * elem_bytes(SB));
#pragma unroll
    for (int j = 0; j < NP; ++j) pre_p[j] = tile_load4s<SB, MWW_AUX_LD_BP>(src, tid + j * NTH);
    const int nvk = max(0, min(TT, a.Tout - t0)) * Q;
    const size_t koff = ((size_t)b * a.Tout + t0) * C;
    dps.issue(elem_ptr<SB>(a.pk, koff), LAST ? a.wd + (size_t)t0 * C : elem_ptr<SB>(a.gk, koff), nvk, tid);
    if (LAST) pre_dz = tile_load1(tile_rsrc(a.dz, a.B * 4), b * 4);
  };
  stagger_start<MWW_STAGGER_BWD>();
  if (nitems > 0) issue(0);

  constexpr int NWL = (C * C + NTH - 1) / NTH, NDL = (K * C + NTH - 1) / NTH;
  float wl[NWL], dl[NDL];
#pragma unroll
  for (int j = 0; j < NWL; ++j) wl[j] = (tid + j * NTH < C * C) ? a.pw_w[tid + j * NTH] : 0.f;
#pragma unroll
  for (int j = 0; j < NDL; ++j) dl[j] = (tid + j * NTH < K * C) ? a.dw_w[tid + j * NTH] : 0.f;
  float accw[K];
  float accb = 0.f, gs1 = 0.f, gs2 = 0.f, dwb = 0.f;
  float sc_c = 0.f, sh_c = 0.f, mu_c = 0.f, rs_c = 0.f;
#pragma unroll
  for (int i = 0; i < K; ++i) accw[i] = 0.f;
  if (dw_active) {
    dwb = a.dw_b[c];
    sc_c = a.in_scale[c];
    sh_c = a.in_shift[c];
    mu_c = a.in_mean[c];
    rs_c = a.in_rstd[c];
  }
  for (int i = tid; i < C; i += NTH) {
    const float krs = a.k_rstd[i];
    const float kmean = a.k_mean[i];
    const float ksc = LAST ? a.k_scale[i] : 0.f, ksh = LAST ? a.k_shift[i] : 0.f;
    float c1, mg, mgx;
    if (a.gfold.acc) {
      bn_grad_fold_channel(a.gfold, C, i, krs, c1, mg, mgx);
    } else {
      c1 = a.k_c1[i];
      mg = a.k_mg[i];
      mgx = a.k_mgx[i];
    }
    const float kA = -c1 * krs * mgx;
    sKp[0 * C + i] = c1;
    sKp[1 * C + i] = kA;
    sKp[2 * C + i] = -c1 * mg - kA * kmean;
    sKp[5 * C + i] = ksc;
    sKp[6 * C + i] = ksh;
  }
#pragma unroll
  for (int j = 0; j < NWL; ++j) {
    const int i = tid + j * NTH;
    if (i < C * C) sWt[(i % C) * PW + i / C] = wl[j];
  }
#pragma unroll
  for (int j = 0; j < NDL; ++j)
    if (tid + j * NTH < K * C) sDW[tid + j * NTH] = dl[j];
  for (int i = RA * P + tid; i < RAP * P; i += NTH) {
    sP[i] = 0.f;
    sDU[i] = 0.f;
  }
  f32x4 dwacc[Roles::NTW];
#pragma unroll
  for (int nt = 0; nt < Roles::NTW; ++nt) dwacc[nt] = zero4();
  if (chunk == 0) {
    sAct[c] = sc_c;
    sAct[C + c] = sh_c;
  }
  float xk1 = sc_c != 0.f ? rs_c / sc_c : 0.f;
  float xk0 = -(sh_c + mu_c * sc_c) * xk1;
  pin(dwb); pin(xk1); pin(xk0);
  __syncthreads();

  MWW_PC_AT(1);
  MWW_PC_START(MWW_ABLATE(a, 16) && tid == 0);
  for (int it = 0; it < nitems; ++it) {
#ifndef MWW_WIDE_NOPRIO
    rotate_priority(it, 2);
#endif
    const int b = blockIdx.x + (it / ntiles) * gridDim.x, t0 = (it % ntiles) * TT;
    const int nrows_new = max(0, min(TT, a.Tout - t0));
    const int rows_da = min(TT, a.Tin - t0);
#pragma unroll
    for (int j = 0; j < NP; ++j) {
      const int i = tid + j * NTH;
      if (i < RA * Q) {
        const int r = i / Q, q = i - r * Q;
        const float4 s4 = *reinterpret_cast<const float4*>(sAct + q * 4), h4 = *reinterpret_cast<const float4*>(sAct + C + q * 4);
        float4 v = pre_p[j];
        v.x = fmaxf(fmaf(v.x, s4.x, h4.x), 0.f);
        v.y = fmaxf(fmaf(v.y, s4.y, h4.y), 0.f);
        v.z = fmaxf(fmaf(v.z, s4.z, h4.z), 0.f);
        v.w = fmaxf(fmaf(v.w, s4.w, h4.w), 0.f);
        *reinterpret_cast<float4*>(sP + r * P + q * 4) = v;
      }
    }
    dps.commit(sDP, sKp, pre_dz, nrows_new * Q, tid);
    for (int i = tid; i < (K - 1) * P; i += NTH) sDU[i] = (t0 == 0) ? 0.f : sDU[TT * P + i];
    MWW_PC_MARK(0);
    __syncthreads();
    MWW_PC_MARK(1);
    if (it + 1 < nitems) issue(it + 1);
    if (dw_active) {
      if (chunk * L < nrows_new) {
        float o[L];
#pragma unroll
        for (int t = 0; t < L; ++t) o[t] = dwb;
        dw_all_groups<K, L, false>(sP + chunk * L * P + c, P, sDW + c, C, o);
#pragma unroll
        for (int t = 0; t < L; ++t) {
          const int tl = chunk * L + t;
          sU[tl * P + c] = (tl < nrows_new) ? o[t] : 0.f;
        }
      } else {
#pragma unroll
        for (int t = 0; t < L; ++t) sU[(chunk * L + t) * P + c] = 0.f;
      }
    }
    MWW_PC_MARK(2);
    __syncthreads();
    MWW_PC_MARK(3);
    int r16 = r16_, g = g_;
    if constexpr (MWW_WIDE_RELANE_K > 0 && K >= MWW_WIDE_RELANE_K) {
      int lm = lane;
      pin(lm);
      r16 = lm & 15;
      g = lm >> 4;
    }
    if constexpr (C == 48 && NW == 8) {
      if (wave < 6) {
        if constexpr (BF) {
          wide_dw_rows_bf16<3, 2, P>(sU, sDP, 32 * (wave / 3), nrows_new, 16 * (wave % 3), 0, r16, g, dwacc);
          wide_du_tiles_bf16<C, 1, K, P, PW>(sDP, sWt, sDU, 2 + wave / 3, nrows_new, 16 * (wave % 3), r16, g);
        } else {
          wide_dw_rows<3, 2, 16, D, P>(sU, sDP, 32 * (wave / 3), nrows_new, 16 * (wave % 3), 0, r16, g, dwacc);
          wide_du_tiles<C, 1, K, P, PW>(sDP, sWt, sDU, 2 + wave / 3, nrows_new, 16 * (wave % 3), r16, g);
        }
      } else {
        if constexpr (BF) wide_du_tiles_bf16<C, 3, K, P, PW>(sDP, sWt, sDU, wave - 6, nrows_new, 0, r16, g);
        else wide_du_tiles<C, 3, K, P, PW>(sDP, sWt, sDU, wave - 6, nrows_new, 0, r16, g);
      }
    } else if constexpr (BF) {
      wide_dw_rows_bf16<2, 4, P>(sU, sDP, 0, nrows_new, 16 * (wave / 2), 32 * (wave % 2), r16, g, dwacc);
      wide_du_tiles_bf16<C, 2, K, P, PW>(sDP, sWt, sDU, wave / 2, nrows_new, 32 * (wave % 2), r16, g);
    } else {
      wide_dw_rows<2, 4, 16, D, P>(sU, sDP, 0, nrows_new, 16 * (wave / 2), 32 * (wave % 2), r16, g, dwacc);
      wide_du_tiles<C, 2, K, P, PW>(sDP, sWt, sDU, wave / 2, nrows_new, 32 * (wave % 2), r16, g);
    }
    MWW_PC_MARK(4);
    __syncthreads();
    MWW_PC_MARK(5);
    {
      const int cch = dw_active ? chunk : NCH - 1;
      const BufRsrc gtile = tile_rsrc(elem_ptr<SB>(a.g_out, ((size_t)b * a.Tin + t0) * C), rows_da * C * elem_bytes(SB));
      const int goff = (dw_active ? 0 : kOobOffset / 4) + cch * L * C + c;
      const float* wdu_p = sDU + cch * L * P + c;
      const float* wa_p = sP + cch * L * P + c;
      {
        float da[L], am[L];
#pragma unroll
        for (int t = 0; t < L; ++t) da[t] = 0.f;
        if (cch * L < rows_da) dw_all_groups<K, L, true>(wdu_p, P, sDW + c, C, da);
        __builtin_amdgcn_sched_barrier(0);
#pragma unroll
        for (int t = 0; t < L; ++t) am[t] = wa_p[t * P];
#pragma unroll
        for (int t = 0; t < L; ++t) {
          const int sl = cch * L + t;
          const float gg = (sl < rows_da && am[t] > 0.f) ? da[t] : 0.f;
          tile_store1s<SB, MWW_AUX_ST_G>(gtile, goff + t * C, gg);
          gs1 += gg;
          gs2 = fmaf(gg, fmaf(am[t], xk1, xk0), gs2);
        }
      }
      __builtin_amdgcn_sched_barrier(0);
      if (cch * L < nrows_new) {
        float duk[L];
#pragma unroll
        for (int t = 0; t < L; ++t) duk[t] = wdu_p[(K - 1 + t) * P];
#pragma unroll
        for (int t = 0; t < L; ++t) accb += duk[t];
        dw_wgrad_all_groups<K, L>(wa_p, P, duk, accw);
      }
    }
    MWW_PC_MARK(6);
    __syncthreads();
    MWW_PC_MARK(7);
  }
  MWW_PC_AT(2);

  float* gdst = a.grad_part + (size_t)blockIdx.x * ((K + 1) * C + C * C);
  float* scratch = smem;
  if (Roles::has_dw(wave)) {
    float* sp = scratch + Roles::part(wave) * C * C + (Roles::mt(wave) * 16 + g_ * 4) * C + Roles::nt0(wave) * 16 + r16_;
#pragma unroll
    for (int nt = 0; nt < Roles::NTW; ++nt)
#pragma unroll
      for (int r = 0; r < 4; ++r) sp[r * C + nt * 16] = dwacc[nt][r];
  }
  __syncthreads();
  for (int e = tid; e < C * C; e += NTH) {
    float v = scratch[e];
    if constexpr (Roles::NPART == 2) v += scratch[C * C + e];
    store_stream<MWW_AUX_ST_GP>(gdst + (K + 1) * C + e, v);
  }
  __syncthreads();
  if (dw_active) {
#pragma unroll
    for (int i = 0; i < K; ++i) scratch[(chunk * (K + 1) + i) * C + c] = accw[i];
    scratch[(chunk * (K + 1) + K) * C + c] = accb;
  }
  __syncthreads();
  for (int e = tid; e < (K + 1) * C; e += NTH) {
    float v = 0.f;
#pragma unroll
    for (int j = 0; j < NCH; ++j) v += scratch[j * (K + 1) * C + e];
    store_stream<MWW_AUX_ST_GP>(gdst + e, v);
  }
  __syncthreads();
  if (dw_active) {
    scratch[(chunk * 2 + 0) * C + c] = gs1;
    scratch[(chunk * 2 + 1) * C + c] = gs2;
  }
  __syncthreads();
  if (tid < 2 * C) {
    float v = 0.f;
#pragma unroll
    for (int j = 0; j < NCH; ++j) v += scratch[j * 2 * C + tid];
    publish_stat(a.gacc, a.gstat_part + (size_t)blockIdx.x * 2 * C, 2 * C, tid, v);
  }
  MWW_PC_AT(3);
  MWW_PC_DUMP(a.phase_clk ? a.phase_clk + (size_t)blockIdx.x * kClkSlots : nullptr);
}

template <int K1, int C1, int COUT, int K, int S, int NTH, bool X6 = false>
struct BwdFirstWideLds {
  static constexpr int PI = C1 + 4;
  static constexpr int PO = COUT + 4;
  static constexpr int PG = C1 + 5;
  static constexpr int PW = C1 + 4;
  static constexpr int PX = FBINS + 1;
  static constexpr int NCH = NTH / C1, L = (TT + NCH - 1) / NCH, TTP = NCH * L, RAP = TTP + K - 1;
  static constexpr int TAIL = S > 1 ? K - 1 : 0;
  static constexpr int TAILK = (TAIL + 3) / 4 * 4;
  static constexpr int XR = (TT + TAILK - 1) * S + K1;
  static constexpr int up4(int v) { return (v + 3) / 4 * 4; }
  static constexpr int OFF_A = 0, OFF_DP = OFF_A + up4(RAP * PI), OFF_U = OFF_DP + TT * PO, OFF_DU = OFF_U + up4(TTP * PI);
  static constexpr int PB = 96, PLB = XR * PB, GPB = 2 * C1, GPL = TT * GPB;
  static constexpr int XFLOATS = X6 ? 3 * PLB / 4 : up4(XR * PX);
  static constexpr int OFF_G0 = OFF_DU + up4(RAP * PI), OFF_END = X6 ? OFF_G0 : OFF_G0 + up4((TTP + TAILK) * PG);
  static constexpr int BYTES = (OFF_END + XFLOATS + 7 * COUT + COUT * PW) * 4 + (int)sizeof(XShared);
};

template <int K1, int C1, int COUT, int K, int S, int NTH, bool X6 = false>
constexpr int wide_first_waves_per_simd() {
  return (BwdFirstWideLds<K1, C1, COUT, K, S, NTH, X6>::BYTES <= 80 * 1024 ? 2 : 1) * (NTH / 64) / 4;
}

template <int K1, int C1, int COUT, int K, int S, int NTH, bool X6 = false>
__global__ __launch_bounds__(NTH, (wide_first_waves_per_simd<K1, C1, COUT, K, S, NTH, X6>())) void bwd_firstw_kernel(BwdFirstArgs a) {
  typedef BwdFirstWideLds<K1, C1, COUT, K, S, NTH, X6> Lds;
  constexpr bool SB = false;
  constexpr int CIN = C1;
  constexpr int PI = Lds::PI, PO = Lds::PO, PG = Lds::PG, PW = Lds::PW, PX = Lds::PX;
  constexpr int NW = NTH / 64, NCH = Lds::NCH, L = Lds::L, TTP = Lds::TTP, RA = TT + K - 1, RAP = Lds::RAP;
  constexpr int TAIL = Lds::TAIL, XR = Lds::XR;
  constexpr int NT1 = C1 / 16, M1 = K1 * FBINS, MT1 = (M1 + 15) / 16, MPW = (MT1 + NW - 1) / NW;
  constexpr int MT = CIN / 16, NT = COUT / 16, QI = CIN / 4, QO = COUT / 4;
  static_assert(NW == 8 && MT == 2 && NCH * L == TT && TT >= K - 1, "geometry of the wide first-block kernel");
  static_assert(TAIL <= NCH && TTP + TAIL <= RAP, "tail rows");
  static_assert(Lds::OFF_END >= 2 * CIN * COUT && Lds::OFF_END >= NCH * (K + 1) * CIN, "scratch aliasing");
  constexpr int PB = Lds::PB, PLB = Lds::PLB, GPB = Lds::GPB, GPL = Lds::GPL;
  static_assert(!X6 || (S == 1 && CIN == 32 && (K1 * FBINS) % 8 == 0 && 3 * GPL <= (TT * PO + TTP * PI) * 4 && TTP == TT), "the x6 form serves the stride-1 first convolutions");

  __shared__ __attribute__((aligned(16))) float sX[Lds::XFLOATS];
  __shared__ XShared sXg;
  __shared__ __attribute__((aligned(16))) float smem[Lds::OFF_END];
  __shared__ __attribute__((aligned(16))) float sKp[7 * COUT];
  __shared__ __attribute__((aligned(16))) float sWt[COUT * PW];
  float* sA = smem + Lds::OFF_A;
  float* sDP = smem + Lds::OFF_DP;
  float* sU = smem + Lds::OFF_U;
  float* sDU = smem + Lds::OFF_DU;
  float* sG0 = smem + Lds::OFF_G0;

  const int tid = threadIdx.x, lane = tid & 63, wave = __builtin_amdgcn_readfirstlane(tid >> 6), r16 = lane & 15, g = lane >> 4;
  const int c = tid % CIN, chunk = tid / CIN;
  const int Ta = (a.T - K1) / S + 1;

  const bool tailmode = TAIL > 0 && Ta > TT && Ta <= TT + TAIL;
  const int ntiles = tailmode ? 1 : (Ta + TT - 1) / TT;
  const int nsamp = (int)blockIdx.x < a.B ? (a.B - (int)blockIdx.x + (int)gridDim.x - 1) / (int)gridDim.x : 0;
  const int nitems = nsamp * ntiles;
  XStage<XR, PX, MWW_AUX_LD_XB, NTH> xs;
  DpStageW<COUT, false, SB, NTH, PO> dps;
  constexpr int NA = (RA * QI + NTH - 1) / NTH;
  float4 pre_a[NA];
  auto issue = [&](int it) {
    const int s = it / ntiles, b = blockIdx.x + s * gridDim.x, t0 = (it % ntiles) * TT;
    const int nrx = ((tailmode ? Ta : min(TT, Ta - t0)) - 1) * S + K1;
    xs.issue(a.x, a.xg, sXg, s, b, a.T, t0 * S, nrx, tid);
    const BufRsrc ra = tile_rsrc(a.a0 + ((size_t)b * Ta + t0) * CIN, min(RA, Ta - t0) * QI * 16);
#pragma unroll
    for (int j = 0; j < NA; ++j) pre_a[j] = tile_load4<MWW_AUX_LD_A0>(ra, (tid + j * NTH) * 16);
    const int nvk = max(0, min(TT, a.Tout - t0)) * QO;
    const size_t koff = ((size_t)b * a.Tout + t0) * COUT;
    dps.issue(elem_ptr<SB>(a.pk, koff), elem_ptr<SB>(a.gk, koff), nvk, tid);
  };
  int offm[MPW];
  bool okm[MPW];
  int xoff[MPW], goff[NT1];
  if constexpr (X6) {
    const int rowl = 4 * g + (r16 >> 2), cg = 4 * (r16 & 3);
#pragma unroll
    for (int mi = 0; mi < MPW; ++mi) {
      const int m = min((mi * NW + wave) * 16 + cg, M1 - 4);
      xoff[mi] = (rowl + m / FBINS) * PB + (m % FBINS) * 2;
    }
#pragma unroll
    for (int nt = 0; nt < NT1; ++nt) goff[nt] = rowl * GPB + ((nt * 16 + cg) ^ ((rowl & 4) ? 16 : 0)) * 2;
  } else {
#pragma unroll
  for (int mi = 0; mi < MPW; ++mi) {
    const int m = (mi * NW + wave) * 16 + r16;
    okm[mi] = m < M1;
    offm[mi] = okm[mi] ? (m / FBINS) * PX + (m % FBINS) : 0;
  }
  }
  if (a.xg.win) xgather_setup(a.xg, sXg, nsamp, tid);
  stagger_start<MWW_STAGGER_BWD>();
  if (nitems > 0) issue(0);

  constexpr int NWL = (CIN * COUT + NTH - 1) / NTH;
  float wl[NWL];
#pragma unroll
  for (int j = 0; j < NWL; ++j) wl[j] = (tid + j * NTH < CIN * COUT) ? a.pw_w[tid + j * NTH] : 0.f;
  float accw[K];
  float accb = 0.f;
#pragma unroll
  for (int i = 0; i < K; ++i) accw[i] = 0.f;
  float dwb = a.dw_b[c];
  float dww[K];
#pragma unroll
  for (int i = 0; i < K; ++i) dww[i] = a.dw_w[i * CIN + c];
  for (int i = tid; i < COUT; i += NTH) {
    const float krs = a.k_rstd[i];
    const float kmean = a.k_mean[i];
    float c1, mg, mgx;
    if (a.gfold.acc) {
      bn_grad_fold_channel(a.gfold, COUT, i, krs, c1, mg, mgx);
    } else {
      c1 = a.k_c1[i];
      mg = a.k_mg[i];
      mgx = a.k_mgx[i];
    }
    const float kA = -c1 * krs * mgx;
    sKp[0 * COUT + i] = c1;
    sKp[1 * COUT + i] = kA;
    sKp[2 * COUT + i] = -c1 * mg - kA * kmean;
    sKp[5 * COUT + i] = 0.f;
    sKp[6 * COUT + i] = 0.f;
  }
#pragma unroll
  for (int j = 0; j < NWL; ++j) {
    const int i = tid + j * NTH;
    if (i < CIN * COUT) sWt[(i % COUT) * PW + i / COUT] = wl[j];
  }
  for (int i = RA * PI + tid; i < RAP * PI; i += NTH) {
    sA[i] = 0.f;
    sDU[i] = 0.f;
  }
  if constexpr (!X6)
    for (int i = TT * PG + tid; i < (TTP + Lds::TAILK) * PG; i += NTH) sG0[i] = 0.f;
#pragma unroll
  for (int i = 0; i < K; ++i) pin(dww[i]);
  pin(dwb);
  f32x4 dwacc[NT];
#pragma unroll
  for (int nt = 0; nt < NT; ++nt) dwacc[nt] = zero4();
  f32x4 w1acc[MPW][NT1];
#pragma unroll
  for (int mi = 0; mi < MPW; ++mi)
#pragma unroll
    for (int nt = 0; nt < NT1; ++nt) w1acc[mi][nt] = zero4();
  __syncthreads();

  for (int it = 0; it < nitems; ++it) {
#ifndef MWW_WIDE_NOPRIO
    rotate_priority(it, 2);
#endif
    const int t0 = (it % ntiles) * TT;
    const int nrows_new = max(0, min(TT, a.Tout - t0));
    const int rows_da = min(TT, Ta - t0);
    if constexpr (X6) xs.template commit_planes<PB, PLB>(reinterpret_cast<unsigned*>(sX), a.xg, sXg, it / ntiles, t0 * S, tid);
    else xs.commit(sX, a.xg, sXg, it / ntiles, t0 * S, tid);
#pragma unroll
    for (int j = 0; j < NA; ++j) {
      const int i = tid + j * NTH;
      if (i < RA * QI) {
        const int r = i / QI, q = i - r * QI;
        *reinterpret_cast<float4*>(sA + r * PI + q * 4) = pre_a[j];
      }
    }
    dps.commit(sDP, sKp, 0.f, nrows_new * QO, tid);
    for (int i = tid; i < (K - 1) * PI; i += NTH) sDU[i] = (t0 == 0) ? 0.f : sDU[TT * PI + i];
    __syncthreads();
    if (it + 1 < nitems) issue(it + 1);
    if (chunk * L < nrows_new) {
      float o[L];
      dw_chunk<K, L>(sA, PI, chunk * L, c, dww, dwb, o);
#pragma unroll
      for (int t = 0; t < L; ++t) {
        const int tl = chunk * L + t;
        sU[tl * PI + c] = (tl < nrows_new) ? o[t] : 0.f;
      }
    } else {
#pragma unroll
      for (int t = 0; t < L; ++t) sU[(chunk * L + t) * PI + c] = 0.f;
    }
    __syncthreads();
    if (wave < 4) {
      wide_du_tiles<COUT, MT, K, PO, PW, PI>(sDP, sWt, sDU, wave, nrows_new, 0, r16, g);
    } else {
      const int v = wave - 4;
      wide_dw_rows<NT, 2, 16, 4, PI, PO>(sU, sDP, 32 * (v / 2), nrows_new, 16 * (v % 2), 0, r16, g, dwacc);
    }
    __syncthreads();
    {
      float wdu[L + K - 1], wa[L + K - 1];
#pragma unroll
      for (int j = 0; j < L + K - 1; ++j) wdu[j] = sDU[(chunk * L + j) * PI + c];
#pragma unroll
      for (int j = 0; j < L + K - 1; ++j) wa[j] = sA[(chunk * L + j) * PI + c];
      lds_reads_first();
#pragma unroll
      for (int t = 0; t < L; ++t) {
        const int sl = chunk * L + t;
        float acc = 0.f;
#pragma unroll
        for (int i = 0; i < K; ++i) acc = fmaf(dww[K - 1 - i], wdu[t + i], acc);
        const float gv = (sl < rows_da && wa[t] > 0.f) ? acc : 0.f;
        if constexpr (X6) {
          unsigned h0, h1, h2;
          split3(gv, h0, h1, h2);
          unsigned short* gp = reinterpret_cast<unsigned short*>(sDP) + sl * CIN + (c ^ ((sl & 4) ? 16 : 0));
          gp[0] = (unsigned short)(h0 >> 16);
          gp[GPL / 2] = (unsigned short)(h1 >> 16);
          gp[GPL] = (unsigned short)(h2 >> 16);
        } else {
          sG0[sl * PG + c] = gv;
        }
      }
      if (chunk * L < nrows_new) {
#pragma unroll
        for (int t = 0; t < L; ++t) {
          const float dut = wdu[K - 1 + t];
          accb += dut;
#pragma unroll
          for (int i = 0; i < K; ++i) accw[i] = fmaf(dut, wa[t + i], accw[i]);
        }
      }
      if constexpr (TAIL > 0) {
        if (tailmode && chunk < TAIL) {
          const int sl = TT + chunk;
          float acc = 0.f;
#pragma unroll
          for (int j = 0; j < K; ++j) acc = fmaf(dww[K - 1 - j], sl + j < RAP ? sDU[(sl + j) * PI + c] : 0.f, acc);
          sG0[sl * PG + c] = (sl < Ta && sA[sl * PI + c] > 0.f) ? acc : 0.f;
        }
      }
    }
    __syncthreads();
    if constexpr (X6) {
      const char* xb = reinterpret_cast<const char*>(sX);
      const char* gb = reinterpret_cast<const char*>(sDP);
#pragma unroll
      for (int kb = 0; kb < TT / 32; ++kb)
#pragma unroll
        for (int nt = 0; nt < NT1; ++nt) {
          u32x4v gq[3];
#pragma unroll
          for (int p = 0; p < 3; ++p) {
            const u32x2v lo = lds_read_tr16(gb + goff[nt] + p * GPL + (32 * kb) * GPB), hi = lds_read_tr16(gb + goff[nt] + p * GPL + (32 * kb + 16) * GPB);
            gq[p] = u32x4v{lo.x, lo.y, hi.x, hi.y};
          }
#pragma unroll
          for (int mi = 0; mi < MPW; ++mi)
            if (mi * NW + wave < MT1) {
              u32x4v xq[3];
#pragma unroll
              for (int p = 0; p < 3; ++p) {
                const u32x2v lo = lds_read_tr16(xb + xoff[mi] + p * PLB + (32 * kb) * S * PB), hi = lds_read_tr16(xb + xoff[mi] + p * PLB + (32 * kb + 16) * S * PB);
                xq[p] = u32x4v{lo.x, lo.y, hi.x, hi.y};
              }
              w1acc[mi][nt] = mfma_x6(xq, gq, w1acc[mi][nt]);
            }
        }
    } else {
      float av[2][MPW], bv[2][NT1];
      auto load_w1 = [&](int srow, int sl) {
#pragma unroll
        for (int nt = 0; nt < NT1; ++nt) bv[sl][nt] = sG0[srow * PG + nt * 16 + r16];
#pragma unroll
        for (int mi = 0; mi < MPW; ++mi) {
          const float v = sX[srow * S * PX + offm[mi]];
          av[sl][mi] = okm[mi] ? v : 0.f;
        }
      };
      load_w1(16 * g, 0);
#pragma unroll
      for (int kk = 0; kk < TT / 4; ++kk) {
        if (kk + 1 < TT / 4) load_w1(kk + 1 + 16 * g, (kk + 1) & 1);
#pragma unroll
        for (int mi = 0; mi < MPW; ++mi)
          if (mi * NW + wave < MT1) {
#pragma unroll
            for (int nt = 0; nt < NT1; ++nt) w1acc[mi][nt] = mfma4(av[kk & 1][mi], bv[kk & 1][nt], w1acc[mi][nt]);
          }
      }
      if constexpr (TAIL > 0) {
        if (tailmode) {
#pragma unroll
          for (int ks = 0; ks < Lds::TAILK / 4; ++ks) {
            load_w1(TT + 4 * ks + g, 0);
#pragma unroll
            for (int mi = 0; mi < MPW; ++mi)
              if (mi * NW + wave < MT1) {
#pragma unroll
                for (int nt = 0; nt < NT1; ++nt) w1acc[mi][nt] = mfma4(av[0][mi], bv[0][nt], w1acc[mi][nt]);
              }
          }
        }
      }
    }
    __syncthreads();
  }

  float* gdst = a.grad_part + (size_t)blockIdx.x * (M1 * C1 + (K + 1) * CIN + CIN * COUT);
#pragma unroll
  for (int mi = 0; mi < MPW; ++mi)
#pragma unroll
    for (int nt = 0; nt < NT1; ++nt)
#pragma unroll
      for (int r = 0; r < 4; ++r) {
        const int m = (mi * NW + wave) * 16 + g * 4 + r;
        if (m < M1) store_stream<MWW_AUX_ST_GP>(gdst + m * C1 + nt * 16 + r16, w1acc[mi][nt][r]);
      }
  float* gblk = gdst + M1 * C1;
  float* scratch = smem;
  if (wave >= 4) {
    const int v = wave - 4;
    float* sp = scratch + (v / 2) * CIN * COUT + ((v % 2) * 16 + g * 4) * COUT + r16;
#pragma unroll
    for (int nt = 0; nt < NT; ++nt)
#pragma unroll
      for (int r = 0; r < 4; ++r) sp[r * COUT + nt * 16] = dwacc[nt][r];
  }
  __syncthreads();
  for (int e = tid; e < CIN * COUT; e += NTH) store_stream<MWW_AUX_ST_GP>(gblk + (K + 1) * CIN + e, scratch[e] + scratch[CIN * COUT + e]);
  __syncthreads();
#pragma unroll
  for (int i = 0; i < K; ++i) scratch[(chunk * (K + 1) + i) * CIN + c] = accw[i];
  scratch[(chunk * (K + 1) + K) * CIN + c] = accb;
  __syncthreads();
  for (int e = tid; e < (K + 1) * CIN; e += NTH) {
    float v = 0.f;
#pragma unroll
    for (int j = 0; j < NCH; ++j) v += scratch[j * (K + 1) * CIN + e];
    store_stream<MWW_AUX_ST_GP>(gblk + e, v);
  }
}

}
```

microwakeword_amd/csrc/mww_lib.hip:

```cpp
#include <hip/hip_runtime.h>

#include <dlfcn.h>

#include <cmath>
#include <cstdio>
#include <climits>
#include <cstring>
#include <map>
#include <string>
#include <vector>

#include "engine.hip.h"
#include "block_launch.hip.h"
#include "kernels_data.hip.h"
#include "kernels_head.hip.h"
#include "kernels_tail.hip.h"

using namespace mww;

namespace {
thread_local std::string g_err;
}

int mww::fail(int code, const std::string& msg) {
  g_err = msg;
  return code;
}

namespace {

int launch_fwd_first(mww_ctx* c, int k1, int c1, int cout, int k, int st, const FwdFirstArgs& a, int grid) {
  if (k_launch_fwd_first(c->stream, c->st_bf16 ? 2 : (c->pw_bf16 ? 1 : 0), k1, c1, cout, k, st, a, grid, c->conv1_x6_fwd)) return MWW_OK;
  return fail(MWW_ERR_UNSUPPORTED, "no first-block kernel for this (conv1 kernel, filters, pointwise, depthwise) shape");
}

int launch_bwd_first(mww_ctx* c, int k1, int c1, int cout, int k, int st, const BwdFirstArgs& a, int grid) {
  if (c->bwd_wide && !c->pw_bf16 && !c->st_bf16 && k_launch_bwd_firstw(c->stream, k1, c1, cout, k, st, a, grid, c->conv1_x6 && c->bwd_first_wide)) return MWW_OK;
  if (k_launch_bwd_first(c->stream, c->st_bf16 ? 2 : (c->pw_bf16 ? 1 : 0), k1, c1, cout, k, st, a, grid, c->conv1_x6)) return MWW_OK;
  return fail(MWW_ERR_UNSUPPORTED, "no first-block backward kernel for this shape");
}

int launch_fwd_block(mww_ctx* c, int cin, int cout, int k, const FwdBlockArgs& a, int grid) {
  if (k_launch_fwd_block(c->stream, c->st_bf16 ? 2 : (c->pw_bf16 ? 1 : 0), cin, cout, k, a, grid)) return MWW_OK;
  return fail(MWW_ERR_UNSUPPORTED, "no block kernel for this (cin, cout, depthwise) shape");
}

int launch_bwd_block(mww_ctx* c, int cin, int cout, int k, bool last, const BwdBlockArgs& a, int grid) {
  const int mode = c->st_bf16 ? 2 : (c->pw_bf16 ? 1 : 0);
  if (c->bwd_wide && k_launch_bwd_blockw(c->stream, mode, cin, cout, k, last, a, grid)) return MWW_OK;
  if (k_launch_bwd_block(c->stream, c->st_bf16 ? 2 : (c->pw_bf16 ? 1 : 0), cin, cout, k, last, a, grid)) return MWW_OK;
  return fail(MWW_ERR_UNSUPPORTED, "no block backward kernel for this shape");
}

constexpr int kHeadMaxRows = 24;
int head_frame_limit(int ch) { return (kThreads / (ch / 4)) * kHeadMaxRows; }

int launch_head(mww_ctx* c, int ch, int jmax, const HeadArgs& a, int grid) {
#define X(C, J)                                                                                                \
  if (ch == C && jmax <= J) {                                                                                  \
    if (c->st_bf16)                                                                                            \
      hipLaunchKernelGGL((head_kernel<C, J, true>), dim3(grid), dim3(kThreads), 0, c->stream, a);              \
    else                                                                                                       \
      hipLaunchKernelGGL((head_kernel<C, J>), dim3(grid), dim3(kThreads), 0, c->stream, a);                    \
    return MWW_OK;                                                                                             \
  }
  static_assert(kHeadMaxRows == 24, "the widest instantiation below");
  X(32, 2) X(32, 4) X(32, 8) X(32, 12) X(32, 16) X(32, 24) X(48, 2) X(48, 4) X(48, 8) X(48, 12) X(48, 16) X(48, 24) X(64, 2) X(64, 4) X(64, 8) X(64, 12) X(64, 16) X(64, 24)
#undef X
  return fail(MWW_ERR_UNSUPPORTED, "no head kernel for this (channels, frames) shape");
}

bool shape_supported(const mww_mixednet_desc& d, std::string* why, bool bf16 = false) {
  if (d.n_blocks < 2 || d.n_blocks > MWW_MAX_BLOCKS) { *why = "the block kernels serve 2.." + std::to_string(MWW_MAX_BLOCKS) + " blocks"; return false; }
  bool ok = false;
#define X(K1, C1, CO, K, S) ok = ok || (d.conv1_kernel == K1 && d.conv1_filters == C1 && d.block_filters[0] == CO && d.block_kernel[0] == K && d.conv1_stride == S);
  if (bf16) { MWW_FIRST_SHAPES_BF16(X) } else { MWW_FIRST_SHAPES(X) }
#undef X
  if (!ok) { *why = "first block (conv1 kernel/filters/stride, pointwise filters, depthwise kernel) not instantiated"; return false; }
  for (int i = 1; i < d.n_blocks; ++i) {
    ok = false;
#define X(CI, CO, K) ok = ok || (d.block_filters[i - 1] == CI && d.block_filters[i] == CO && d.block_kernel[i] == K);
    if (bf16) { MWW_BLOCK_SHAPES_BF16(X) } else { MWW_BLOCK_SHAPES(X) }
#undef X
    if (!ok) { *why = "block " + std::to_string(i) + " (cin, cout, depthwise kernel) not instantiated"; return false; }
  }
  const int cl = d.block_filters[d.n_blocks - 1];
  if (cl != 32 && cl != 48 && cl != 64) { *why = "head kernel needs 32, 48 or 64 channels"; return false; }
  int t = d.frames >= d.conv1_kernel && d.conv1_stride > 0 ? (d.frames - d.conv1_kernel) / d.conv1_stride + 1 : 0;
  for (int i = 0; i < d.n_blocks; ++i) t -= d.block_kernel[i] - 1;
  if (t > head_frame_limit(cl)) {
    *why = "head kernel holds at most " + std::to_string(head_frame_limit(cl)) + " final frames at " + std::to_string(cl) + " channels (" + std::to_string(t) + " here)";
    return false;
  }
  return true;
}

float* bn_slot(Layer& l, int i) { return l.bn + (size_t)i * l.cout; }

}

namespace mww {

const float* mail_hyper(mww_ctx* c) { return reinterpret_cast<const float*>(c->mail_dev[c->mail_cur] + c->mail_off_hyper); }

static int bring_targets(mww_ctx* c) {
  if (c->y_cur == c->y) return MWW_OK;
  const size_t n = (size_t)c->lazy_a.B * sizeof(float);
  HIPCHK(hipMemcpyAsync(c->y, c->y_cur, n, hipMemcpyDeviceToDevice, c->stream));
  HIPCHK(hipMemcpyAsync(c->sw, c->sw_cur, n, hipMemcpyDeviceToDevice, c->stream));
  c->y_cur = c->y;
  c->sw_cur = c->sw;
  return MWW_OK;
}

int materialise_x(mww_ctx* c) {
  int rc = bring_targets(c);
  if (rc || !c->x_lazy) return rc;
  AssembleArgs a = c->lazy_a;
  a.n_targets = 0;
  Launcher lp{c};
  lp.begin("assemble");
  hipLaunchKernelGGL(assemble_kernel, dim3(a.B * a.split), dim3(kThreads), 0, c->stream, a);
  lp.end();
  HIPCHK(hipGetLastError());
  c->x_lazy = false;
  return MWW_OK;
}

XGather x_gather(mww_ctx* c) {
  XGather g;
  memset(&g, 0, sizeof(g));
  if (!c->x_lazy) return g;
  const AssembleArgs& a = c->lazy_a;
  g.win = a.win;
  g.masks = a.masks;
  for (int i = 0; i < MWW_MAX_STORES; ++i) { g.store[i] = a.store[i]; g.dtype[i] = a.dtype[i]; }
  g.ntm = a.ntm;
  g.nfm = a.nfm;
  g.T = a.T;
  return g;
}

static int join_side(mww_ctx* c) {
  if (c->side_pending) {
    HIPCHK(hipStreamWaitEvent(c->stream, c->ev_join, 0));
    c->side_pending = false;
  }
  return MWW_OK;
}

int enqueue_side_work(mww_ctx* c, int B, bool metrics, bool loss, const float* p_last, const float* scale,
                      const float* shift, const float* keep) {
  Launcher lp{c};
  if (metrics || loss) {
    const bool inline_side = c->profile || !c->use_side;
    hipStream_t ss = inline_side ? c->stream : c->side;
    if (!inline_side) {
      HIPCHK(hipEventRecord(c->ev_fork, c->stream));
      HIPCHK(hipStreamWaitEvent(c->side, c->ev_fork, 0));
    }
    const bool one_launch = metrics && loss && inline_side;
    if (metrics && !one_launch) {
      MetricsArgs ma{c->prob, c->y_cur, c->metrics, B, c->bce_clipped ? nullptr : c->z};
      lp.begin("metrics");
      hipLaunchKernelGGL(metrics_kernel, dim3(1), dim3(1024), 0, ss, ma);
      c->metric_launches += 1;
      lp.end();
    }
    if (loss) {
      const int dchunk = (B + kDenseChunks - 1) / kDenseChunks;
      const int ndchunks = (B + dchunk - 1) / dchunk;
      DenseGradArgs dg{p_last, scale, shift, c->dz, c->dwd_part, B, c->t_last * c->c_last, c->c_last, c->dwd_stride, dchunk, keep,
                       nullptr, nullptr, nullptr, 0, 0, c->st_bf16 ? 1 : 0};
      if (c->generic && !c->head2 && c->G.back().res_src >= 0) {
        GOp& rr = c->G[c->G.back().res_src];
        dg.rp = rr.p;
        dg.rscale = rr.bn + (size_t)BN_SCALE * rr.cout;
        dg.rshift = rr.bn + (size_t)BN_SHIFT * rr.cout;
        dg.rT = rr.tout;
        dg.rdrop = c->G.back().res_drop;
      }
      if (one_launch) {
        HeadTailArgs ht;
        memset(&ht, 0, sizeof(ht));
        ht.dense = dg;
        ht.met = MetricsArgs{c->prob, c->y_cur, c->metrics, B, c->bce_clipped ? nullptr : c->z};
        ht.n_fin = 0;
        ht.ndx = (dg.n + 1 + kThreads - 1) / kThreads;
        ht.ndy = ndchunks;
        ht.do_metrics = 1;
        c->metric_launches += 1;
        lp.begin("dense_grad+metrics");
        hipLaunchKernelGGL(head_tail_kernel, dim3(ht.ndx * ht.ndy + 1), dim3(kThreads), 0, ss, ht);
        lp.end();
      } else {
        lp.begin("dense_grad");
        hipLaunchKernelGGL(dense_grad_kernel, dim3((dg.n + 1 + kThreads - 1) / kThreads, ndchunks), dim3(kThreads), 0, ss, dg);
        lp.end();
      }
    }
    if (!inline_side) {
      HIPCHK(hipEventRecord(c->ev_join, c->side));
      c->side_pending = true;
    }
  }
  return MWW_OK;
}


int exchange_stats(mww_ctx* c, Launcher& lp, const char* what, int layer, const float* part, int G, int C, int bwd,
                   float local_inv_n, StatSource* out) {
  out->part = part;
  out->G = G;
  out->inv_n = local_inv_n;
  out->dscale = 1.0f;
  if (!(c->hook && c->sync_bn)) return MWW_OK;
  float* buf = c->sync_buf + c->sync_off[layer] + (bwd ? 2 * C : 0);
  StatCollapseArgs a{part, G, C, buf};
  lp.begin(what, layer);
  hipLaunchKernelGGL(stat_collapse_kernel, dim3(C), dim3(kThreads), 0, c->stream, a);
  lp.end();
  if (c->hook(c->hook_user, buf, 2 * C, MWW_EXCHANGE_IN_ORDER) != 0) return fail(MWW_ERR_STATE, "all-reduce hook failed");
  out->part = buf;
  out->G = 1;
  out->inv_n = local_inv_n / (float)c->world;
  out->dscale = 1.0f / (float)c->world;
  return MWW_OK;
}

}

namespace {

int fwd_block_grid(const mww_ctx* c, const Layer& l, int B) {
  const int per_cu = l.cin > 48 ? 2 : (l.k > 13 ? 3 : 4);
  const long long items = (long long)B * ((l.tout + TT - 1) / TT);
  return (int)std::min<long long>(items, std::min(c->grid_fwd, c->n_cu * per_cu));
}

int enqueue_forward(mww_ctx* c, int B, bool training, bool update_moving, bool loss, bool metrics) {
  if (c->generic) return g_enqueue_forward(c, B, training, update_moving, loss, metrics);
  Launcher lp{c};
  const mww_mixednet_desc& d = c->d;
  const int nb = d.n_blocks;
  if (!training && !c->bn_eval_ready) {
    for (int i = 0; i < nb; ++i) {
      Layer& l = c->L[i];
      BnEvalPrepareArgs a{c->params + l.o_gamma, c->params + l.o_beta, c->bn_state + l.o_mm, c->bn_state + l.o_mv,
                          bn_slot(l, BN_SCALE), bn_slot(l, BN_SHIFT), l.cout};
      lp.begin("bn_eval_prepare", i);
      hipLaunchKernelGGL(bn_eval_prepare_kernel, dim3(1), dim3(64), 0, c->stream, a);
      lp.end();
    }
  }
  const bool inl = training && c->bn_inline && !(c->hook && c->sync_bn);
  auto fold_of = [&](Layer& pl) {
    BnFoldArgs f;
    memset(&f, 0, sizeof(f));
    if (!inl) return f;
    f.acc = pl.facc_cur;
    f.inv_n = 1.0f / ((float)B * (float)pl.tout);
    f.update_moving = update_moving ? 1 : 0;
    f.gamma = c->params + pl.o_gamma;
    f.beta = c->params + pl.o_beta;
    f.moving_mean = c->bn_state + pl.o_mm;
    f.moving_var = c->bn_state + pl.o_mv;
    f.scale = bn_slot(pl, BN_SCALE);
    f.shift = bn_slot(pl, BN_SHIFT);
    f.mean = bn_slot(pl, BN_MEAN);
    f.rstd = bn_slot(pl, BN_RSTD);
    return f;
  };
  for (int i = 0; i < nb; ++i) {
    Layer& l = c->L[i];
    const int grid = i == 0 ? std::min(B, c->grid_fwd) : fwd_block_grid(c, l, B);
    StatAcc sacc{nullptr, nullptr};
    if (inl) {
      sacc.acc = l.facc[c->fpar];
      sacc.clear = l.facc[c->fpar ^ 1];
      l.facc_cur = sacc.acc;
    }
    if (i == 0) {
      FwdFirstArgs a{c->x, c->params + c->o_conv1, c->params + l.o_dw_w, c->params + l.o_dw_b, c->params + l.o_pw_w,
                     l.p, l.stat_part, B, d.frames, l.tout, 0, sacc, x_gather(c), training ? c->a0 : nullptr};
      lp.begin("fwd_block", i);
      int rc = launch_fwd_first(c, d.conv1_kernel, d.conv1_filters, l.cout, l.k, d.conv1_stride, a, grid);
      lp.end();
      if (rc) return rc;
    } else {
      Layer& pl = c->L[i - 1];
      FwdBlockArgs a{pl.p, bn_slot(pl, BN_SCALE), bn_slot(pl, BN_SHIFT), c->params + l.o_dw_w, c->params + l.o_dw_b,
                     c->params + l.o_pw_w, l.p, l.stat_part, B, l.tin, l.tout, c->ablate, c->phase_clk + (size_t)(2 * i) * 2048 * kClkSlots,
                     sacc, fold_of(pl)};
      lp.begin("fwd_block", i);
      int rc = launch_fwd_block(c, l.cin, l.cout, l.k, a, grid);
      lp.end();
      if (rc) return rc;
    }
    if (training && !inl) {
      StatSource ss;
      int rcs = exchange_stats(c, lp, "bn_stat_exchange", i, l.stat_part, grid, l.cout, 0, 1.0f / ((float)B * (float)l.tout), &ss);
      if (rcs) return rcs;
      BnFwdFinalizeArgs f{ss.part, ss.G, l.cout, ss.inv_n, c->params + l.o_gamma,
                          c->params + l.o_beta, c->bn_state + l.o_mm, c->bn_state + l.o_mv, bn_slot(l, BN_SCALE),
                          bn_slot(l, BN_SHIFT), bn_slot(l, BN_MEAN), bn_slot(l, BN_RSTD), update_moving ? 1 : 0};
      lp.begin("bn_fwd_finalize", i);
      hipLaunchKernelGGL(bn_fwd_finalize_kernel, dim3(l.cout), dim3(kThreads), 0, c->stream, f);
      lp.end();
    }
  }
  Layer& ll = c->L[nb - 1];
  const int ghead = std::min(B, c->grid_head);
  HeadArgs h;
  h.p = ll.p;
  h.scale = bn_slot(ll, BN_SCALE);
  h.shift = bn_slot(ll, BN_SHIFT);
  h.mean = bn_slot(ll, BN_MEAN);
  h.rstd = bn_slot(ll, BN_RSTD);
  h.wd = c->params + c->o_dense_w;
  h.bd = c->params + c->o_dense_b;
  h.y = (loss || metrics) ? c->y_cur : nullptr;
  h.sw = c->sw_cur;
  h.z = c->z;
  h.prob = c->prob;
  h.dz = c->dz;
  h.loss_part = c->loss_part;
  h.gstat_part = ll.gstat_part;
  h.B = B;
  h.T = ll.tout;
  h.inv_b = 1.0f / (float)B;
  h.training = (loss ? kHeadTraining : 0) | (c->bce_clipped ? kHeadClippedLoss : 0);
  h.fold = fold_of(ll);
  if (inl) c->fpar ^= 1;
  const bool tail_late = loss && inl && c->tail_roles;
  h.gacc = StatAcc{nullptr, nullptr};
  if (tail_late) {
    h.gacc.acc = ll.gacc[c->gpar];
    h.gacc.clear = ll.gacc[c->gpar ^ 1];
    ll.gacc_cur = h.gacc.acc;
  }
  const int q = ll.cout / 4, nrg = kThreads / q;
  lp.begin("head");
  int rc = launch_head(c, ll.cout, (ll.tout + nrg - 1) / nrg, h, ghead);
  lp.end();
  if (rc) return rc;
  if (tail_late) {
    c->tail_in_reduce = true;
    c->tail_metrics = metrics;
    return MWW_OK;
  }
  if (loss && !(c->hook && c->sync_bn)) {
    c->tail_pending = true;
    c->tail_metrics = metrics;
    return MWW_OK;
  }
  return enqueue_side_work(c, B, metrics, loss, ll.p, bn_slot(ll, BN_SCALE), bn_slot(ll, BN_SHIFT), nullptr);
}

int enqueue_adam(mww_ctx* c);

int assemble_range(mww_ctx* c, int B, const GradReduceArgs& ga, int64_t lo, int64_t hi, bool tail_dense, bool metrics, bool apply_adam) {
  Launcher lp{c};
  std::vector<FinalSegment> segs;
  for (int i = 0; i < ga.nseg; ++i) {
    const GradSegment& g = ga.seg[i];
    if (g.dst < lo || g.dst >= hi) continue;
    if (g.dst + g.n > hi) return fail(MWW_ERR_STATE, "gradient segment straddles a bucket boundary");
    segs.push_back(FinalSegment{g.part, g.G, g.stride, g.n, g.dst, kSegPartials, 0});
  }
  GradFinalArgs a;
  memset(&a, 0, sizeof(a));
  if (tail_dense && c->o_dense_w >= lo && c->o_dense_w < hi) {
    Layer& ll = c->L[c->d.n_blocks - 1];
    a.dense = DenseGradArgs{ll.p, bn_slot(ll, BN_SCALE), bn_slot(ll, BN_SHIFT), c->dz, nullptr, B, c->t_last * c->c_last,
                            c->c_last, 0, (B + kDenseChunks - 1) / kDenseChunks, nullptr, nullptr, nullptr, nullptr, 0, 0, c->st_bf16 ? 1 : 0};
    segs.push_back(FinalSegment{nullptr, B, 0, c->t_last * c->c_last + 1, (int)c->o_dense_w, kSegDense, 0});
  }
  std::sort(segs.begin(), segs.end(), [](const FinalSegment& x, const FinalSegment& y) { return x.dst < y.dst; });
  std::vector<FinalSegment> all;
  int64_t cur = lo;
  auto fill = [&](int64_t upto) {
    while (cur < upto) {
      const bool dir = c->direct_host[(size_t)cur] != 0;
      int64_t e = cur;
      while (e < upto && (c->direct_host[(size_t)e] != 0) == dir) ++e;
      all.push_back(FinalSegment{nullptr, 1, 0, (int)(e - cur), (int)cur, dir ? kSegDirect : kSegZero, 0});
      cur = e;
    }
  };
  for (const FinalSegment& sgm : segs) {
    if (sgm.dst < cur) return fail(MWW_ERR_STATE, "overlapping gradient segments");
    fill(sgm.dst);
    all.push_back(sgm);
    cur = sgm.dst + sgm.n;
  }
  fill(hi);
  a.met = MetricsArgs{c->prob, c->y_cur, c->metrics, B, c->bce_clipped ? nullptr : c->z};
  a.mask = c->mask;
  a.grad = c->grads;
  a.scale = 1.0f;
  a.adam = AdamArgs{c->params, c->grads, c->adam_m, c->adam_v, mail_hyper(c), (int)c->P, 0.9f, 0.999f, 1e-7f};
  a.apply_adam = apply_adam ? 1 : 0;
  for (size_t first = 0; first < all.size() || (metrics && first == 0); first += kMaxFinalSegments) {
    const int n = (int)std::min<size_t>(kMaxFinalSegments, all.size() - first);
    int nb = 0, ns = 0;
    for (int pass = 0; pass < 2; ++pass)
      for (int i = 0; i < n; ++i) {
        const FinalSegment& sg = all[first + i];
        if ((sg.kind == kSegDense) != (pass == 0)) continue;
        a.seg[ns] = sg;
        a.seg[ns].block0 = nb;
        a.block0[ns] = nb;
        nb += (sg.n + kFinalCols - 1) / kFinalCols;
        ++ns;
      }
    for (int i = ns; i < kMaxFinalSegments; ++i) a.block0[i] = INT_MAX;
    a.nseg = n;
    a.nblocks = nb;
    a.do_metrics = (metrics && first == 0) ? 1 : 0;
    if (nb + a.do_metrics == 0) break;
    c->metric_launches += a.do_metrics;
    lp.begin(apply_adam ? "grad_final+adam" : "grad_final");
    hipLaunchKernelGGL(grad_final_kernel, dim3(nb + a.do_metrics), dim3(kThreads), 0, c->stream, a);
    lp.end();
    if (all.empty()) break;
  }
  return MWW_OK;
}

int exchange_range(mww_ctx* c, int64_t lo, int64_t hi, int flags) {
  if (c->hook(c->hook_user, flags == MWW_EXCHANGE_FLUSH ? nullptr : c->grads + lo, flags == MWW_EXCHANGE_FLUSH ? 0 : hi - lo, flags) != 0)
    return fail(MWW_ERR_STATE, "all-reduce hook failed");
  return MWW_OK;
}

}

namespace mww {

int enqueue_grad_assembly(mww_ctx* c, int B, GradReduceArgs& ga, bool fuse_adam, int64_t lo, int64_t hi, bool last_range) {
  if (hi < 0) hi = c->P;
  int rcj = join_side(c);
  if (rcj) return rcj;
  const bool tail_here = c->tail_in_reduce && c->o_dense_w >= lo && c->o_dense_w < hi;
  if (tail_here) c->tail_in_reduce = false;
  if (!tail_here && c->o_dense_w >= lo && c->o_dense_w < hi) {
    const int dchunk = (B + kDenseChunks - 1) / kDenseChunks;
    GradSegment s;
    s.part = c->dwd_part;
    s.G = (B + dchunk - 1) / dchunk;
    s.stride = c->dwd_stride;
    s.n = c->t_last * c->c_last + 1;
    s.dst = (int)c->o_dense_w;
    ga.seg[ga.nseg++] = s;
  }
  const bool exchange = fuse_adam && c->hook && c->reduce_grads;
  int rc = assemble_range(c, B, ga, lo, hi, tail_here, tail_here && c->tail_metrics, fuse_adam && !exchange);
  if (rc || !exchange) return rc;
  rc = exchange_range(c, lo, hi, last_range ? MWW_EXCHANGE_IN_ORDER : MWW_EXCHANGE_DEFERRED);
  if (!last_range) c->exchange_pending = true;
  if (rc || !last_range) return rc;
  if (c->exchange_pending) {
    rc = exchange_range(c, 0, 0, MWW_EXCHANGE_FLUSH);
    c->exchange_pending = false;
    if (rc) return rc;
  }
  return enqueue_adam(c);
}

}

namespace {

void block_segments(mww_ctx* c, int gbwd, int b0, int b1, GradReduceArgs* ga) {
  memset(ga, 0, sizeof(*ga));
  for (int i = b0; i < b1; ++i) {
    Layer& l = c->L[i];
    GradSegment s;
    s.part = l.grad_part;
    s.G = gbwd;
    s.stride = l.grad_part_stride;
    s.n = l.grad_part_stride;
    s.dst = (int)(i == 0 ? c->o_conv1 : l.o_dw_w);
    ga->seg[ga->nseg++] = s;
  }
}

int enqueue_backward(mww_ctx* c, int B, bool fuse_adam) {
  if (c->generic) return g_enqueue_backward(c, B, fuse_adam);
  Launcher lp{c};
  const mww_mixednet_desc& d = c->d;
  const int nb = d.n_blocks;
  const int gbwd = std::min(B, c->grid_bwd);
  const int ghead = std::min(B, c->grid_head);
  const bool inl = c->bn_inline && !(c->hook && c->sync_bn);
  const int split = nb >= 3 ? nb - 2 : 0;
  const bool bucketed = fuse_adam && c->hook && c->reduce_grads && !c->sync_bn && inl && c->tail_in_reduce && c->grad_buckets == 2 && split > 0;
  for (int i = nb - 1; i >= 0; --i) {
    Layer& l = c->L[i];
    const bool last = (i == nb - 1);
    const bool fold_here = inl && (!last || c->tail_in_reduce);
    StatSource ss{nullptr, 0, 0.f, 1.0f};
    if (!fold_here) {
      int rcs = exchange_stats(c, lp, "bn_gstat_exchange", i, l.gstat_part, last ? ghead : gbwd, l.cout, 1,
                               1.0f / ((float)B * (float)l.tout), &ss);
      if (rcs) return rcs;
    }
    BnBwdFinalizeArgs f{ss.part, ss.G, l.cout, ss.inv_n,
                        c->params + l.o_gamma, bn_slot(l, BN_RSTD), bn_slot(l, BN_C1), bn_slot(l, BN_MG),
                        bn_slot(l, BN_MGX), c->grads + l.o_gamma, c->grads + l.o_beta, ss.dscale};
    BnGradFoldArgs gf;
    memset(&gf, 0, sizeof(gf));
    if (fold_here) {
      gf.acc = l.gacc_cur;
      gf.inv_n = 1.0f / ((float)B * (float)l.tout);
      gf.dscale = 1.0f;
      gf.gamma = c->params + l.o_gamma;
      gf.c1 = bn_slot(l, BN_C1);
      gf.mg = bn_slot(l, BN_MG);
      gf.mgx = bn_slot(l, BN_MGX);
      gf.dgamma = c->grads + l.o_gamma;
      gf.dbeta = c->grads + l.o_beta;
    }
    if (fold_here) {
    } else if (last && c->tail_pending) {
      c->tail_pending = false;
      const int dchunk = (B + kDenseChunks - 1) / kDenseChunks;
      HeadTailArgs ht;
      ht.fin = f;
      ht.dense = DenseGradArgs{l.p, bn_slot(l, BN_SCALE), bn_slot(l, BN_SHIFT), c->dz, c->dwd_part, B, c->t_last * c->c_last,
                               c->c_last, c->dwd_stride, dchunk, nullptr, nullptr, nullptr, nullptr, 0, 0, c->st_bf16 ? 1 : 0};
      ht.met = MetricsArgs{c->prob, c->y_cur, c->metrics, B, c->bce_clipped ? nullptr : c->z};
      ht.n_fin = l.cout;
      ht.ndx = (ht.dense.n + 1 + kThreads - 1) / kThreads;
      ht.ndy = (B + dchunk - 1) / dchunk;
      ht.do_metrics = c->tail_metrics ? 1 : 0;
      c->metric_launches += ht.do_metrics;
      lp.begin("head_tail");
      hipLaunchKernelGGL(head_tail_kernel, dim3(ht.n_fin + ht.ndx * ht.ndy + ht.do_metrics), dim3(kThreads), 0, c->stream, ht);
      lp.end();
    } else {
      lp.begin("bn_bwd_finalize", i);
      hipLaunchKernelGGL(bn_bwd_finalize_kernel, dim3(l.cout), dim3(kThreads), 0, c->stream, f);
      lp.end();
    }
    if (i > 0) {
      Layer& pl = c->L[i - 1];
      BwdBlockArgs a;
      a.in = pl.p;
      a.in_scale = bn_slot(pl, BN_SCALE);
      a.in_shift = bn_slot(pl, BN_SHIFT);
      a.in_mean = bn_slot(pl, BN_MEAN);
      a.in_rstd = bn_slot(pl, BN_RSTD);
      a.pk = l.p;
      a.gk = l.g;
      a.k_mean = bn_slot(l, BN_MEAN);
      a.k_rstd = bn_slot(l, BN_RSTD);
      a.k_c1 = bn_slot(l, BN_C1);
      a.k_mg = bn_slot(l, BN_MG);
      a.k_mgx = bn_slot(l, BN_MGX);
      a.k_scale = bn_slot(l, BN_SCALE);
      a.k_shift = bn_slot(l, BN_SHIFT);
      a.wd = c->params + c->o_dense_w;
      a.dz = c->dz;
      a.dw_w = c->params + l.o_dw_w;
      a.dw_b = c->params + l.o_dw_b;
      a.pw_w = c->params + l.o_pw_w;
      a.g_out = pl.g;
      a.gstat_part = pl.gstat_part;
      a.grad_part = l.grad_part;
      a.B = B;
      a.Tin = l.tin;
      a.Tout = l.tout;
      a.ablate = c->ablate;
      a.phase_clk = c->phase_clk + (size_t)(2 * i + 1) * 2048 * kClkSlots;
      a.gacc = StatAcc{nullptr, nullptr};
      if (inl) {
        a.gacc.acc = pl.gacc[c->gpar];
        a.gacc.clear = pl.gacc[c->gpar ^ 1];
        pl.gacc_cur = a.gacc.acc;
      }
      a.gfold = gf;
      lp.begin("bwd_block", i);
      int rc = launch_bwd_block(c, l.cin, l.cout, l.k, last, a, gbwd);
      lp.end();
      if (rc) return rc;
      if (bucketed && i == split) {
        GradReduceArgs gb;
        block_segments(c, gbwd, split, nb, &gb);
        rc = enqueue_grad_assembly(c, B, gb, fuse_adam, l.o_dw_w, c->P, false);
        if (rc) return rc;
      }
    } else {
      if (last) return fail(MWW_ERR_UNSUPPORTED, "single-block models are not supported");
      BwdFirstArgs a{c->x, c->a0, l.p, l.g, bn_slot(l, BN_MEAN), bn_slot(l, BN_RSTD), bn_slot(l, BN_C1),
                     bn_slot(l, BN_MG), bn_slot(l, BN_MGX), c->params + l.o_dw_w, c->params + l.o_dw_b,
                     c->params + l.o_pw_w, l.grad_part, B, d.frames, l.tout, gf, x_gather(c)};
      lp.begin("bwd_block", i);
      int rc = launch_bwd_first(c, d.conv1_kernel, d.conv1_filters, l.cout, l.k, d.conv1_stride, a, gbwd);
      lp.end();
      if (rc) return rc;
    }
  }
  if (inl) c->gpar ^= 1;
  GradReduceArgs ga;
  block_segments(c, gbwd, 0, bucketed ? split : nb, &ga);
  return enqueue_grad_assembly(c, B, ga, fuse_adam, 0, bucketed ? c->L[split].o_dw_w : c->P, true);
}

int enqueue_adam(mww_ctx* c) {
  Launcher lp{c};
  AdamArgs a{c->params, c->grads, c->adam_m, c->adam_v, mail_hyper(c), (int)c->P, 0.9f, 0.999f, 1e-7f};
  lp.begin("adam");
  hipLaunchKernelGGL(adam_kernel, dim3(((int)c->P + kThreads - 1) / kThreads), dim3(kThreads), 0, c->stream, a);
  lp.end();
  return MWW_OK;
}

int mail_begin(mww_ctx* c) {
  if (!c->mail_open) {
    HIPCHK(hipEventSynchronize(c->mail_ev[c->mail_cur]));
    c->mail_open = true;
  }
  return MWW_OK;
}
int mail_commit(mww_ctx* c) {
  HIPCHK(hipEventRecord(c->mail_ev[c->mail_cur], c->stream));
  c->mail_cur = (c->mail_cur + 1) % kRing;
  c->mail_open = false;
  c->targets_in_mail = 0;
  return MWW_OK;
}
int push_hyper(mww_ctx* c, float alpha, float gscale) {
  int rc = mail_begin(c);
  if (rc) return rc;
  float* h = reinterpret_cast<float*>(c->mail_host[c->mail_cur] + c->mail_off_hyper);
  h[0] = alpha;
  h[1] = gscale;
  return MWW_OK;
}
int flush_targets(mww_ctx* c) {
  if (c->targets_in_mail > 0) {
    const char* m = c->mail_host[c->mail_cur];
    const size_t n = (size_t)c->targets_in_mail * sizeof(float);
    HIPCHK(hipMemcpyAsync(c->y, m + c->mail_off_y, n, hipMemcpyHostToDevice, c->stream));
    HIPCHK(hipMemcpyAsync(c->sw, m + c->mail_off_sw, n, hipMemcpyHostToDevice, c->stream));
    c->targets_in_mail = 0;
    c->y_cur = c->y;
    c->sw_cur = c->sw;
  }
  return MWW_OK;
}

float adam_alpha(float lr, int64_t t) {
  const float b1p = powf(0.9f, (float)t), b2p = powf(0.999f, (float)t);
  return lr * sqrtf(1.0f - b2p) / (1.0f - b1p);
}

int step_sequence(mww_ctx* c, int B, int flags) {
  c->metric_launches = 0;
  int rc = enqueue_forward(c, B, true, true, true, !(flags & MWW_STEP_NO_METRICS));
  if (rc) return rc;
  rc = enqueue_backward(c, B, !(flags & MWW_STEP_NO_APPLY));
  if (rc) return rc;
  if (c->metric_launches > 1) return fail(MWW_ERR_STATE, "internal: more than one launch of this step carries the metric update");
  return MWW_OK;
}

template <typename T>
int dev_alloc(T** p, size_t n) {
  HIPCHK(hipMalloc((void**)p, std::max<size_t>(n, 1) * sizeof(T)));
  HIPCHK(hipMemset(*p, 0, std::max<size_t>(n, 1) * sizeof(T)));
  return MWW_OK;
}

struct BnSlots { int64_t o_gamma, o_beta, o_mv; int n; };

int init_defaults(mww_ctx* c, const std::vector<BnSlots>& bn) {
  std::vector<float> ones((size_t)c->P, 1.0f);
  std::vector<unsigned char> dir((size_t)c->P, 0);
  std::vector<float> st((size_t)c->S, 0.0f);
  for (const BnSlots& b : bn)
    for (int j = 0; j < b.n; ++j) {
      dir[(size_t)b.o_gamma + j] = 1;
      dir[(size_t)b.o_beta + j] = 1;
      if (b.o_mv >= 0) st[(size_t)b.o_mv + j] = 1.0f;
    }
  HIPCHK(hipMemcpy(c->mask, ones.data(), ones.size() * sizeof(float), hipMemcpyHostToDevice));
  HIPCHK(hipMemcpy(c->direct, dir.data(), dir.size(), hipMemcpyHostToDevice));
  c->direct_host = dir;
  HIPCHK(hipMemcpy(c->bn_state, st.data(), st.size() * sizeof(float), hipMemcpyHostToDevice));
  return MWW_OK;
}

int alloc_common(mww_ctx* c) {
  const mww_mixednet_desc& d = c->d;
  const size_t mb = (size_t)d.max_batch;
  int rc = 0;
#define A(call) if ((rc = (call)) != 0) return rc;
#define H(call) if ((call) != hipSuccess) return fail(MWW_ERR_HIP, #call);
  A(dev_alloc(&c->params, c->P));
  A(dev_alloc(&c->grads, c->P));
  A(dev_alloc(&c->adam_m, c->P));
  A(dev_alloc(&c->adam_v, c->P));
  A(dev_alloc(&c->mask, c->P));
  A(dev_alloc(&c->direct, c->P));
  A(dev_alloc(&c->bn_state, c->S));
  A(dev_alloc(&c->x, mb * d.frames * MWW_FEATURE_BINS));
  A(dev_alloc(&c->y, mb));
  A(dev_alloc(&c->sw, mb));
  c->y_cur = c->y;
  c->sw_cur = c->sw;
  A(dev_alloc(&c->z, mb));
  A(dev_alloc(&c->prob, mb));
  A(dev_alloc(&c->dz, mb));
  A(dev_alloc(&c->loss_part, mb));
  A(dev_alloc(&c->dwd_part, (size_t)kDenseChunks * c->dwd_stride));
  A(dev_alloc(&c->metrics, 1));
  A(dev_alloc(&c->phase_clk, (size_t)2 * MWW_MAX_BLOCKS * 2048 * kClkSlots));
  c->mail_off_masks = mb * sizeof(mww_window);
  c->mail_off_y = c->mail_off_masks + mb * kMaxMasks * 2 * sizeof(int);
  c->mail_off_sw = c->mail_off_y + mb * sizeof(float);
  c->mail_off_hyper = c->mail_off_sw + mb * sizeof(float);
  c->mail_bytes = c->mail_off_hyper + 16;
  for (int i = 0; i < kRing; ++i) {
    H(hipHostMalloc((void**)&c->mail_host[i], c->mail_bytes, hipHostMallocMapped));
    memset(c->mail_host[i], 0, c->mail_bytes);
    H(hipHostGetDevicePointer((void**)&c->mail_dev[i], c->mail_host[i], 0));
    H(hipEventCreateWithFlags(&c->mail_ev[i], hipEventDisableTiming));
  }
  H(hipStreamCreateWithFlags(&c->copy_stream, hipStreamNonBlocking));
  for (int i = 0; i < kRing; ++i) {
    A(dev_alloc(&c->mail_hbm[i], c->mail_bytes));
    H(hipEventCreateWithFlags(&c->ev_copy[i], hipEventDisableTiming));
  }
  H(hipStreamCreateWithFlags(&c->side, hipStreamNonBlocking));
  H(hipEventCreateWithFlags(&c->ev_fork, hipEventDisableTiming));
  H(hipEventCreateWithFlags(&c->ev_join, hipEventDisableTiming));
#undef A
#undef H
  return MWW_OK;
}

int open_device(mww_ctx* c, int device, void* stream) {
  int ndev = 0;
  HIPCHK(hipGetDeviceCount(&ndev));
  if (ndev <= 0) return fail(MWW_ERR_HIP, "no HIP device visible");
  if (device < 0 || device >= ndev) return fail(MWW_ERR_INVALID, "device index out of range");
  HIPCHK(hipSetDevice(device));
  c->device = device;
  hipDeviceProp_t prop;
  HIPCHK(hipGetDeviceProperties(&prop, device));
  c->n_cu = prop.multiProcessorCount > 0 ? prop.multiProcessorCount : 256;
  if (stream) {
    c->stream = (hipStream_t)stream;
  } else {
    HIPCHK(hipStreamCreateWithFlags(&c->stream, hipStreamNonBlocking));
    c->own_stream = true;
  }
  c->grid_fwd = c->n_cu * 4;
  c->grid_bwd = c->n_cu * 2;
  bool wide64 = false;
  for (int i = 0; i < c->d.n_blocks; ++i) wide64 = wide64 || c->d.block_filters[i] > 48;
  if (!c->generic && wide64) {
    c->grid_fwd = c->n_cu * 2;
    c->grid_bwd = c->n_cu;
  }
  c->grid_head = c->n_cu * 2;
  c->grid_g = c->n_cu * 3;
  return MWW_OK;
}

}

extern "C" {

const char* mww_last_error(void) { return g_err.c_str(); }

int mww_device_count(void) {
  int n = 0;
  if (hipGetDeviceCount(&n) != hipSuccess) return 0;
  return n;
}

int mww_block_kernels_cover(const mww_mixednet_desc* desc, int bf16) {
  if (!desc) return fail(MWW_ERR_INVALID, "null descriptor");
  std::string why;
  if (shape_supported(*desc, &why, bf16 != 0)) return 1;
  g_err = why;
  return 0;
}

int mww_create(const mww_mixednet_desc* desc, int device, void* stream, mww_ctx** out) {
  if (!desc || !out) return fail(MWW_ERR_INVALID, "null argument");
  const mww_mixednet_desc& d = *desc;
  if (d.n_blocks < 2 || d.n_blocks > MWW_MAX_BLOCKS) return fail(MWW_ERR_INVALID, "n_blocks must be in [2, 8]");
  if (d.conv1_stride < 1 || d.frames < d.conv1_kernel) return fail(MWW_ERR_INVALID, "bad first-conv stride / kernel");
  if (d.conv1_filters <= 0) return fail(MWW_ERR_UNSUPPORTED, "first_conv_filters == 0 is not implemented");
  if (d.max_batch <= 0 || d.frames <= 0) return fail(MWW_ERR_INVALID, "frames and max_batch must be positive");
  std::string why;
  if (!shape_supported(d, &why)) return fail(MWW_ERR_UNSUPPORTED, why);
  mww_ctx* c = new mww_ctx();
  c->d = d;
  {
    int rco = open_device(c, device, stream);
    if (rco) { delete c; return rco; }
  }
  int64_t off = 0, soff = 0;
  c->o_conv1 = off;
  off += (int64_t)d.conv1_kernel * MWW_FEATURE_BINS * d.conv1_filters;
  int t = (d.frames - d.conv1_kernel) / d.conv1_stride + 1, ch = d.conv1_filters;
  c->L.resize(d.n_blocks);
  for (int i = 0; i < d.n_blocks; ++i) {
    Layer& l = c->L[i];
    l.cin = ch;
    l.cout = d.block_filters[i];
    l.k = d.block_kernel[i];
    l.tin = t;
    l.tout = t - (l.k - 1);
    if (l.tout <= 0) { mww_destroy(c); return fail(MWW_ERR_INVALID, "spectrogram too short for the kernel sizes"); }
    l.o_dw_w = off; off += (int64_t)l.k * l.cin;
    l.o_dw_b = off; off += l.cin;
    l.o_pw_w = off; off += (int64_t)l.cin * l.cout;
    l.o_gamma = off; off += l.cout;
    l.o_beta = off; off += l.cout;
    l.o_mm = soff; soff += l.cout;
    l.o_mv = soff; soff += l.cout;
    t = l.tout;
    ch = l.cout;
  }
  c->t_last = t;
  c->c_last = ch;
  c->o_dense_w = off; off += (int64_t)t * ch;
  c->o_dense_b = off; off += 1;
  c->P = off;
  c->S = soff;
  c->dwd_stride = t * ch + 4;
  const size_t mb = (size_t)d.max_batch;
  const int gmax_f = c->n_cu * 4, gmax_b = c->n_cu * 2;
  int rc = 0;
#define A(call) if ((rc = (call)) != 0) { mww_destroy(c); return rc; }
  A(alloc_common(c));
  A(dev_alloc(&c->a0, mb * c->L[0].tin * d.conv1_filters));
#ifndef MWW_G_PINGPONG
#define MWW_G_PINGPONG 1
#endif
  if (MWW_G_PINGPONG) {
    size_t need[2] = {0, 0};
    for (int i = 0; i < d.n_blocks; ++i) need[i & 1] = std::max(need[i & 1], mb * c->L[i].tout * c->L[i].cout);
    for (int par = 0; par < 2; ++par)
      if (need[par]) A(dev_alloc(&c->gbuf[par], need[par]));
  }
  for (int i = 0; i < d.n_blocks; ++i) {
    Layer& l = c->L[i];
    A(dev_alloc(&l.p, mb * l.tout * l.cout));
    if (MWW_G_PINGPONG) l.g = c->gbuf[i & 1];
    else A(dev_alloc(&l.g, mb * l.tout * l.cout));
    A(dev_alloc(&l.stat_part, (size_t)gmax_f * 2 * l.cout));
    A(dev_alloc(&l.gstat_part, (size_t)std::max(gmax_b, c->n_cu * 4) * 2 * l.cout));
    for (int par = 0; par < 2; ++par) {
      A(dev_alloc(&l.facc[par], (size_t)kStatRows * 2 * l.cout));
      A(dev_alloc(&l.gacc[par], (size_t)kStatRows * 2 * l.cout));
    }
    l.grad_part_stride = (l.k + 1) * l.cin + l.cin * l.cout;
    if (i == 0) l.grad_part_stride += d.conv1_kernel * MWW_FEATURE_BINS * d.conv1_filters;
    A(dev_alloc(&l.grad_part, (size_t)gmax_b * l.grad_part_stride));
    A(dev_alloc(&l.bn, (size_t)9 * l.cout));
  }
  {
    std::vector<BnSlots> bn;
    for (int i = 0; i < d.n_blocks; ++i) bn.push_back(BnSlots{c->L[i].o_gamma, c->L[i].o_beta, c->L[i].o_mv, c->L[i].cout});
    A(init_defaults(c, bn));
  }
#undef A
  HIPCHK(hipDeviceSynchronize());
  *out = c;
  return MWW_OK;
}

int mww_create_convnet(const mww_convnet_desc* desc, int device, void* stream, mww_ctx** out) {
  if (!desc || !out) return fail(MWW_ERR_INVALID, "null argument");
  const mww_convnet_desc& d = *desc;
  GPlan plan;
  {
    int rcp = g_plan_convnet(d, &plan);
    if (rcp) return rcp;
  }
  int64_t off = plan.P;
  const int64_t soff = plan.S;

  mww_ctx* c = new mww_ctx();
  memset(&c->d, 0, sizeof(c->d));
  c->d.frames = d.frames;
  c->d.max_batch = d.max_batch;
  c->generic = true;
  c->dropout = d.dropout;
  c->G = std::move(plan.ops);
  c->g_chunks = plan.chunks;
  c->g_inline_ok = plan.inline_ok;
  {
// ... 424 lines not shown
  return rc;
}
int mww_get_batch(mww_ctx* c, float* hx, int B) {
  if (!c || !hx || B <= 0 || B > c->d.max_batch) return fail(MWW_ERR_INVALID, "bad batch size");
  HIPCHK(hipSetDevice(c->device));
  int rc = materialise_x(c);
  if (rc) return rc;
  return copy_out(c, hx, c->x, (size_t)B * c->d.frames * MWW_FEATURE_BINS * sizeof(float));
}

int mww_set_targets(mww_ctx* c, const float* hy, const float* hw, int B) {
  if (!c || !hy || !hw || B <= 0 || B > c->d.max_batch) return fail(MWW_ERR_INVALID, "bad batch size");
  HIPCHK(hipSetDevice(c->device));
  int rc = mail_begin(c);
  if (rc) return rc;
  char* mh = c->mail_host[c->mail_cur];
  memcpy(mh + c->mail_off_y, hy, (size_t)B * sizeof(float));
  memcpy(mh + c->mail_off_sw, hw, (size_t)B * sizeof(float));
  c->targets_in_mail = B;
  c->have_targets = B;
  return MWW_OK;
}

int mww_assemble_prefetched(mww_ctx* c, mww_prefetcher* p, float* out_labels, float* out_weights) {
  if (!c || !p) return fail(MWW_ERR_INVALID, "null context / prefetcher");
  const mww_window* win = nullptr;
  const int32_t* masks = nullptr;
  const float *y = nullptr, *w = nullptr;
  int rc = mww_prefetch_acquire(p, &win, &masks, &y, &w, nullptr, nullptr);
  if (rc) return fail(rc, "the prefetcher's sampler failed (a provider's truncation strategy cannot form a fixed-length window)");
  int B = 0, ntm = 0, nfm = 0;
  mww_prefetch_shape(p, &B, &ntm, &nfm);
  rc = mww_set_targets(c, y, w, B);
  if (!rc) rc = mww_assemble_batch(c, win, masks, B, ntm, nfm);
  if (!rc && out_labels) memcpy(out_labels, y, (size_t)B * sizeof(float));
  if (!rc && out_weights) memcpy(out_weights, w, (size_t)B * sizeof(float));
  mww_prefetch_release(p);
  return rc;
}

int mww_train_step(mww_ctx* c, int B, float lr, int flags) {
  if (!c || B <= 0 || B > c->d.max_batch) return fail(MWW_ERR_INVALID, "bad batch size");
  if (c->have_batch < B || c->have_targets < B) return fail(MWW_ERR_STATE, "train step needs a batch and targets of at least B rows");
  HIPCHK(hipSetDevice(c->device));
  int rc = flush_targets(c);
  if (rc) return rc;
  if (c->lazy_slot != c->mail_cur) {
    rc = materialise_x(c);
    if (rc) return rc;
  }
  const bool apply = !(flags & MWW_STEP_NO_APPLY);
  if (apply) {
    c->step += 1;
    rc = push_hyper(c, adam_alpha(lr, c->step), (c->hook && c->reduce_grads) ? 1.0f / (float)c->world : 1.0f);
    if (rc) return rc;
  }
  const bool gen_dropout = c->generic && c->dropout > 0.f && !c->keep_explicit;
  if (gen_dropout) {
    rc = mail_begin(c);
    if (rc) return rc;
    unsigned* h = reinterpret_cast<unsigned*>(c->mail_host[c->mail_cur] + c->mail_off_hyper);
    h[2] = (unsigned)(c->dropout_counter & 0xFFFFFFFFull);
    h[3] = (unsigned)(c->dropout_counter >> 32);
    c->dropout_counter += 1;
  }
  if (c->use_graphs && !c->profile && !c->hook) {
    const int mail = (apply || gen_dropout || c->x_lazy) ? c->mail_cur : -1;
    const bool flips = c->bn_inline && (!c->generic || (c->g_inline_ok && !c->profile_split));
    const int par = (flips ? (4 | c->fpar | (c->gpar << 1)) : 0) | (c->x_lazy ? 8 : 0) | (c->y_cur != c->y ? 16 : 0) | (c->tail_roles ? 32 : 0) | (c->g_role_split ? 64 : 0) | (c->grid_g_auto ? 128 : 0) | (c->g_dgrad_share << 8) | (c->g_cap_fwd << 16) | (c->g_cap_bwd << 20) | (c->g_chunks << 24);
    hipGraphExec_t exec = nullptr;
    for (auto& g : c->graphs)
      if (g.B == B && g.flags == flags && g.mail == mail && g.par == par) exec = g.exec;
    if (exec && flips) {
      c->fpar ^= 1;
      c->gpar ^= 1;
    }
    if (!exec) {
      hipGraph_t graph;
      HIPCHK(hipStreamBeginCapture(c->stream, hipStreamCaptureModeThreadLocal));
      rc = step_sequence(c, B, flags);
      hipError_t e = hipStreamEndCapture(c->stream, &graph);
      if (rc) return rc;
      if (e != hipSuccess) return fail(MWW_ERR_HIP, std::string("hipStreamEndCapture: ") + hipGetErrorString(e));
      HIPCHK(hipGraphInstantiate(&exec, graph, nullptr, nullptr, 0));
      HIPCHK(hipGraphDestroy(graph));
      c->graphs.push_back({B, flags, mail, par, exec});
    }
    HIPCHK(hipGraphLaunch(exec, c->stream));
    return mail_commit(c);
  }
  rc = step_sequence(c, B, flags);
  if (rc) return rc;
  HIPCHK(hipGetLastError());
  return mail_commit(c);
}

int mww_apply_gradients(mww_ctx* c, float lr, float gscale) {
  if (!c) return fail(MWW_ERR_INVALID, "null context");
  HIPCHK(hipSetDevice(c->device));
  c->step += 1;
  int rc = push_hyper(c, adam_alpha(lr, c->step), gscale);
  if (rc) return rc;
  rc = enqueue_adam(c);
  if (rc) return rc;
  HIPCHK(hipGetLastError());
  return mail_commit(c);
}

int mww_forward(mww_ctx* c, int B, int training, int update_metrics) {
  if (!c || B <= 0 || B > c->d.max_batch) return fail(MWW_ERR_INVALID, "bad batch size");
  if (c->have_batch < B) return fail(MWW_ERR_STATE, "forward needs a batch of at least B rows");
  if (update_metrics && c->have_targets < B) return fail(MWW_ERR_STATE, "metric update needs targets");
  HIPCHK(hipSetDevice(c->device));
  int rc = flush_targets(c);
  if (rc) return rc;
  if (c->lazy_slot != c->mail_cur) {
    rc = materialise_x(c);
    if (rc) return rc;
  }
  rc = enqueue_forward(c, B, training != 0, false, false, update_metrics != 0);
  if (rc) return rc;
  rc = join_side(c);
  if (rc) return rc;
  HIPCHK(hipGetLastError());
  return mail_commit(c);
}

int mww_evaluate_windows(mww_ctx* c, const mww_window* windows, const float* labels, int64_t n, int batch) {
  if (!c || !windows || !labels || n < 0 || batch <= 0 || batch > c->d.max_batch) return fail(MWW_ERR_INVALID, "bad evaluation arguments");
  std::vector<float> ones((size_t)batch, 1.0f);
  int rc = MWW_OK;
  for (int64_t s = 0; s < n && !rc; s += batch) {
    const int b = (int)std::min<int64_t>(batch, n - s);
    rc = mww_set_targets(c, labels + s, ones.data(), b);
    if (!rc) rc = mww_assemble_batch(c, windows + s, nullptr, b, 0, 0);
    if (!rc) rc = mww_forward(c, b, 0, 1);
    c->bn_eval_ready = !c->generic;
  }
  c->bn_eval_ready = false;
  return rc;
}

int mww_read_outputs(mww_ctx* c, int B, float* probs, float* logits, float* loss) {
  if (!c || B <= 0 || B > c->d.max_batch) return fail(MWW_ERR_INVALID, "bad batch size");
  if (probs) HIPCHK(hipMemcpyAsync(probs, c->prob, (size_t)B * sizeof(float), hipMemcpyDeviceToHost, c->stream));
  if (logits) HIPCHK(hipMemcpyAsync(logits, c->z, (size_t)B * sizeof(float), hipMemcpyDeviceToHost, c->stream));
  std::vector<float> lp;
  if (loss) {
    lp.resize(B);
    HIPCHK(hipMemcpyAsync(lp.data(), c->loss_part, (size_t)B * sizeof(float), hipMemcpyDeviceToHost, c->stream));
  }
  HIPCHK(hipStreamSynchronize(c->stream));
  if (loss) {
    double s = 0.0;
    for (int i = 0; i < B; ++i) s += lp[i];
    *loss = (float)s;
  }
  return MWW_OK;
}

int mww_metrics_read(mww_ctx* c, mww_metrics* out) {
  if (!c || !out) return fail(MWW_ERR_INVALID, "null argument");
  static_assert(sizeof(mww_metrics) == sizeof(MetricState), "metric layouts must match");
  return copy_out(c, out, c->metrics, sizeof(MetricState));
}
int mww_metrics_reset(mww_ctx* c) {
  if (!c) return fail(MWW_ERR_INVALID, "null context");
  HIPCHK(hipMemsetAsync(c->metrics, 0, sizeof(MetricState), c->stream));
  return MWW_OK;
}

void* mww_device_ptr(mww_ctx* c, int which) {
  if (!c) return nullptr;
  switch (which) {
    case MWW_BUF_PARAMS: return c->params;
    case MWW_BUF_GRADS: return c->grads;
    case MWW_BUF_BN_STATE: return c->bn_state;
    case MWW_BUF_X: return c->x;
    case MWW_HANDLE_STREAM: return c->stream;
    default: return nullptr;
  }
}

int64_t mww_debug_read(mww_ctx* c, const char* name, int B, float* host, int64_t cap) {
  if (!c || !name || !host || B <= 0 || B > c->d.max_batch) return fail(MWW_ERR_INVALID, "bad debug_read arguments");
  const float* src = nullptr;
  int64_t n = 0;
  const int nb = c->d.n_blocks;
  auto idx = [&](const char* prefix) -> int {
    const size_t pl = strlen(prefix);
    if (strncmp(name, prefix, pl) != 0) return -1;
    const int k = atoi(name + pl);
    return (k >= 1 && k <= nb && name[pl] >= '0' && name[pl] <= '9') ? k - 1 : -1;
  };
  int k;
  if (c->generic) {
    const int no = (int)c->G.size();
    auto gidx = [&](const char* prefix) -> int {
      const size_t pl = strlen(prefix);
      if (strncmp(name, prefix, pl) != 0 || name[pl] < '0' || name[pl] > '9') return -1;
      const int kk = atoi(name + pl);
      return (kk >= 1 && kk <= no) ? kk - 1 : -1;
    };
    if ((k = gidx("p")) >= 0) { src = c->G[k].p; n = (int64_t)B * c->G[k].tout * c->G[k].cout; }
    else if ((k = gidx("g")) >= 0) { src = c->G[k].g; n = (int64_t)B * c->G[k].tout * c->G[k].cout; }
    else if ((k = gidx("bn")) >= 0) { src = c->G[k].bn; n = (int64_t)9 * c->G[k].cout; }
    else if (!strcmp(name, "dz")) { src = c->dz; n = B; }
    else if (!strcmp(name, "keep")) { src = c->keep; n = (int64_t)B * c->t_last * c->c_last; }
    else if (!strcmp(name, "x")) {
      if (materialise_x(c)) return -1;
      src = c->x;
      n = (int64_t)B * c->d.frames * MWW_FEATURE_BINS;
    }
    else return fail(MWW_ERR_INVALID, std::string("unknown tensor name: ") + name);
    if (n > cap) return fail(MWW_ERR_INVALID, "host buffer too small");
    const int kpl = gidx("p") >= 0 ? gidx("p") : gidx("g");
    if (kpl >= 0 && g_planes(c, c->G[kpl]) > 1) {
      const GOp& o = c->G[kpl];
      const int planes = g_planes(c, o);
      std::vector<float> tmp((size_t)B * o.tout * o.pc);
      for (int pl = 0; pl < planes; ++pl) {
        int rcp = copy_out(c, tmp.data(), src + (size_t)pl * g_pstride(c, o), tmp.size() * sizeof(float));
        if (rcp) return rcp;
        for (int64_t r = 0; r < (int64_t)B * o.tout; ++r)
          for (int cc = 0; cc < o.pc; ++cc) host[r * o.cout + pl * o.pc + cc] = tmp[(size_t)r * o.pc + cc];
      }
      return n;
    }
    int rcg = copy_out(c, host, src, (size_t)n * sizeof(float));
    return rcg ? rcg : n;
  }
  bool stored = false;
  if ((k = idx("p")) >= 0) { src = c->L[k].p; n = (int64_t)B * c->L[k].tout * c->L[k].cout; stored = true; }
  else if ((k = idx("g")) >= 0) { src = c->L[k].g; n = (int64_t)B * c->L[k].tout * c->L[k].cout; stored = true; }
  else if ((k = idx("bn")) >= 0) { src = c->L[k].bn; n = (int64_t)9 * c->L[k].cout; }
  else if (!strcmp(name, "dz")) { src = c->dz; n = B; }
  else if (!strcmp(name, "a0")) { src = c->a0; n = (int64_t)B * c->L[0].tin * c->d.conv1_filters; }
  else if (!strncmp(name, "clkf", 4) || !strncmp(name, "clkb", 4)) {
    const int kk = atoi(name + 4);
    if (kk < 1 || kk > nb) return fail(MWW_ERR_INVALID, "bad layer");
    src = reinterpret_cast<const float*>(c->phase_clk + (size_t)(2 * (kk - 1) + (name[3] == 'b' ? 1 : 0)) * 2048 * kClkSlots);
    n = 2048 * kClkSlots * 2;
  }
  else if (!strcmp(name, "x")) { src = c->x; n = (int64_t)B * c->d.frames * MWW_FEATURE_BINS; }
  else return fail(MWW_ERR_INVALID, std::string("unknown tensor name: ") + name);
  if (n > cap) return fail(MWW_ERR_INVALID, "host buffer too small");
  if (stored && c->st_bf16) {
    std::vector<unsigned short> half((size_t)n);
    int rch = copy_out(c, half.data(), src, (size_t)n * sizeof(unsigned short));
    if (rch) return rch;
    for (int64_t i = 0; i < n; ++i) {
      const unsigned bits = (unsigned)half[(size_t)i] << 16;
      memcpy(host + i, &bits, 4);
    }
    return n;
  }
  int rc = copy_out(c, host, src, (size_t)n * sizeof(float));
  return rc ? rc : n;
}

int mww_set_option(mww_ctx* c, const char* name, int64_t v) {
  if (!c || !name) return fail(MWW_ERR_INVALID, "null argument");
  if (!strcmp(name, "graphs")) c->use_graphs = v != 0;
  else if (!strcmp(name, "profile")) {
    c->profile = v != 0;
    for (auto& e : c->prof) { (void)hipEventDestroy(e.a); (void)hipEventDestroy(e.b); }
    c->prof.clear();
  }
  else if (!strcmp(name, "ablate")) c->ablate = (int)v;
  else if (!strcmp(name, "side_stream")) c->use_side = v != 0;
  else if (!strcmp(name, "bn_inline")) c->bn_inline = v != 0;
  else if (!strcmp(name, "graph_role_split")) c->g_role_split = v != 0;
  else if (!strcmp(name, "graph_static_shapes")) c->g_static = v != 0;
  else if (!strcmp(name, "graph_planar")) c->g_planar = v != 0;
  else if (!strcmp(name, "graph_fwd_wg_per_cu")) { if (v < 1 || v > 8) return fail(MWW_ERR_INVALID, "graph_fwd_wg_per_cu must be 1..8"); c->g_cap_fwd = (int)v; }
  else if (!strcmp(name, "graph_bwd_wg_per_cu")) { if (v < 1 || v > 8) return fail(MWW_ERR_INVALID, "graph_bwd_wg_per_cu must be 1..8"); c->g_cap_bwd = (int)v; }
  else if (!strcmp(name, "graph_frame_chunks")) { if (v < 0 || v > 4) return fail(MWW_ERR_INVALID, "graph_frame_chunks must be 0..4"); c->g_chunks = (int)v; }
  else if (!strcmp(name, "graph_dgrad_share")) { if (v < 10 || v > 90) return fail(MWW_ERR_INVALID, "graph_dgrad_share must be 10..90"); c->g_dgrad_share = (int)v; }
  else if (!strcmp(name, "tail_roles")) c->tail_roles = v != 0;
  else if (!strcmp(name, "bce_from_logits")) c->bce_clipped = v == 0;
  else if (!strcmp(name, "grad_buckets")) { if (v < 1 || v > 2) return fail(MWW_ERR_INVALID, "grad_buckets must be 1 or 2"); c->grad_buckets = (int)v; }
  else if (!strcmp(name, "fused_input")) {
    c->fused_input = v != 0;
    if (!v) { int rc = materialise_x(c); if (rc) return rc; }
  }
  else if (!strcmp(name, "assemble_split")) { if (v < 1 || v > 8) return fail(MWW_ERR_INVALID, "assemble_split out of range"); c->asm_split = (int)v; }
  else if (!strcmp(name, "profile_split")) c->profile_split = v != 0;
  else if (!strcmp(name, "pointwise_bf16")) {
    if (c->generic && v) return fail(MWW_ERR_UNSUPPORTED, "the conv/BN graph kernels have no bf16 mode");
    { std::string why; if (v && !shape_supported(c->d, &why, true)) return fail(MWW_ERR_UNSUPPORTED, "no bf16 mode for this topology: " + why); }
    c->pw_bf16 = v != 0;
    if (!v) c->st_bf16 = false;
  }
  else if (!strcmp(name, "storage_bf16")) {
    if (c->generic && v) return fail(MWW_ERR_UNSUPPORTED, "the conv/BN graph kernels have no bf16 mode");
    { std::string why; if (v && !shape_supported(c->d, &why, true)) return fail(MWW_ERR_UNSUPPORTED, "no bf16 mode for this topology: " + why); }
    c->st_bf16 = v != 0;
    if (v) c->pw_bf16 = true;
  }
  else if (!strcmp(name, "bwd_wide")) c->bwd_wide = v != 0;
  else if (!strcmp(name, "conv1_x6")) c->conv1_x6 = v != 0;
  else if (!strcmp(name, "conv1_x6_fwd")) c->conv1_x6_fwd = v != 0;
  else if (!strcmp(name, "bwd_first_wide")) c->bwd_first_wide = v != 0;
  else if (!strcmp(name, "grid_fwd")) { if (v < 1 || v > c->n_cu * 4) return fail(MWW_ERR_INVALID, "grid_fwd out of range"); c->grid_fwd = (int)v; }
  else if (!strcmp(name, "grid_bwd")) { if (v < 1 || v > c->n_cu * 2) return fail(MWW_ERR_INVALID, "grid_bwd out of range"); c->grid_bwd = (int)v; }
  else if (!strcmp(name, "grid_graph")) {
    if (v < 0 || v > c->n_cu * 4) return fail(MWW_ERR_INVALID, "grid_graph out of range");
    c->grid_g_auto = v == 0;
    if (v > 0) c->grid_g = (int)v;
  }
  else if (!strcmp(name, "dropout_seed")) { c->dropout_seed = (unsigned long long)v; c->dropout_counter = 0; }
  else if (!strcmp(name, "grid_head")) { if (v < 1 || v > c->n_cu * 4) return fail(MWW_ERR_INVALID, "grid_head out of range"); c->grid_head = (int)v; }
  else return fail(MWW_ERR_INVALID, std::string("unknown option: ") + name);
  for (auto& g : c->graphs) (void)hipGraphExecDestroy(g.exec);
  c->graphs.clear();
  return MWW_OK;
}

int mww_profile_read(mww_ctx* c, char* names, int names_cap, float* ms, int cap) {
  if (!c) return fail(MWW_ERR_INVALID, "null context");
  HIPCHK(hipStreamSynchronize(c->stream));
  int n = 0, pos = 0;
  for (auto& e : c->prof) {
    if (n >= cap) break;
    float t = 0.f;
    (void)hipEventElapsedTime(&t, e.a, e.b);
    ms[n] = t;
    const int len = (int)e.name.size();
    if (names && pos + len + 1 < names_cap) {
      memcpy(names + pos, e.name.c_str(), len);
      names[pos + len] = '\n';
      pos += len + 1;
    }
    ++n;
  }
  if (names && names_cap > 0) names[pos < names_cap ? pos : names_cap - 1] = 0;
  for (auto& e : c->prof) { (void)hipEventDestroy(e.a); (void)hipEventDestroy(e.b); }
  c->prof.clear();
  return n;
}

}

namespace mww {
int ctx_borrow(mww_ctx* c, int* device, hipStream_t* stream, void** stores, int* dtypes, int64_t* elems, int* n_cu) {
  if (!c) return fail(MWW_ERR_INVALID, "no context");
  *device = c->device;
  *stream = c->stream;
  *n_cu = c->n_cu;
  for (int i = 0; i < MWW_MAX_STORES; ++i) { stores[i] = c->store[i]; dtypes[i] = c->store_dtype[i]; elems[i] = c->store_elems[i]; }
  return MWW_OK;
}
int set_error(int code, const char* msg) { return fail(code, msg); }
}
```

microwakeword_amd/csrc/tu_bwd_first.hip:

```cpp
#define MWW_BLOCK_TU 1
#include "block_launch.hip.h"

namespace mww {

template <int K1, int C1, int CO, int K, int S, bool BF = false, bool SB = false>
static bool launch_bwd_first_x6(hipStream_t st, const BwdFirstArgs& a, int grid) {
  if constexpr (S == 1) {
    hipLaunchKernelGGL((bwd_first_kernel<K1, C1, CO, K, S, BF, SB, true>), dim3(grid), dim3(kThreads), 0, st, a);
    return true;
  } else {
    return false;
  }
}

bool k_launch_bwd_first(hipStream_t st, int mode, int k1, int c1, int cout, int k, int stride, const BwdFirstArgs& a, int grid, bool x6) {
  if (mode != 0) {
#define X(K1, C1, CO, K, S)                                                                                    \
    if (k1 == K1 && c1 == C1 && cout == CO && k == K && stride == S) {                                         \
       \
      if (x6 && mode == 2 && launch_bwd_first_x6<K1, C1, CO, K, S, true, true>(st, a, grid)) return true;     \
      if (x6 && mode == 1 && launch_bwd_first_x6<K1, C1, CO, K, S, true, false>(st, a, grid)) return true;    \
      if (mode == 2)                                                                                           \
        hipLaunchKernelGGL((bwd_first_kernel<K1, C1, CO, K, S, true, true>), dim3(grid), dim3(kThreads), 0, st, a); \
      else                                                                                                     \
        hipLaunchKernelGGL((bwd_first_kernel<K1, C1, CO, K, S, true>), dim3(grid), dim3(kThreads), 0, st, a);  \
      return true;                                                                                             \
    }
    MWW_FIRST_SHAPES_BF16(X)
#undef X
    return false;
  }
#define X(K1, C1, CO, K, S)                                                                                    \
  if (k1 == K1 && c1 == C1 && cout == CO && k == K && stride == S) {                                           \
    if (x6 && launch_bwd_first_x6<K1, C1, CO, K, S>(st, a, grid)) return true;                                 \
    hipLaunchKernelGGL((bwd_first_kernel<K1, C1, CO, K, S, false>), dim3(grid), dim3(kThreads), 0, st, a);     \
    return true;                                                                                               \
  }
  MWW_FIRST_SHAPES(X)
#undef X
  return false;
}

}
```

microwakeword_amd/csrc/tu_bwdw.hip:

```cpp
#define MWW_BLOCK_TU 1
#include "block_launch.hip.h"
#include "kernels_bwdw.hip.h"

namespace mww {

template <int C, int K, int NTH>
static void launch_w(hipStream_t st, bool last, const BwdBlockArgs& a, int grid) {
  if (last) hipLaunchKernelGGL((bwd_blockw_kernel<C, C, K, true, NTH>), dim3(grid), dim3(NTH), 0, st, a);
  else hipLaunchKernelGGL((bwd_blockw_kernel<C, C, K, false, NTH>), dim3(grid), dim3(NTH), 0, st, a);
}
template <int C, int K, int NTH>
static void launch_w_bf16(hipStream_t st, int mode, bool last, const BwdBlockArgs& a, int grid) {
  if (mode == 2) {
    if (last) hipLaunchKernelGGL((bwd_blockw_kernel<C, C, K, true, NTH, true, true>), dim3(grid), dim3(NTH), 0, st, a);
    else hipLaunchKernelGGL((bwd_blockw_kernel<C, C, K, false, NTH, true, true>), dim3(grid), dim3(NTH), 0, st, a);
  } else {
    if (last) hipLaunchKernelGGL((bwd_blockw_kernel<C, C, K, true, NTH, true>), dim3(grid), dim3(NTH), 0, st, a);
    else hipLaunchKernelGGL((bwd_blockw_kernel<C, C, K, false, NTH, true>), dim3(grid), dim3(NTH), 0, st, a);
  }
}

bool k_launch_bwd_blockw(hipStream_t st, int mode, int cin, int cout, int k, bool last, const BwdBlockArgs& a, int grid) {
  if (cin != cout) return false;
  if (mode != 0) {
#define X(CI, CO, K)                                                                                           \
    if (cin == CI && k == K) {                                                                                 \
      if constexpr (CI == CO && (CI == 48 || CI == 64)) {                                                      \
        launch_w_bf16<CI, K, 512>(st, mode, last, a, grid);                                                    \
        return true;                                                                                           \
      }                                                                                                        \
    }
    MWW_BLOCK_SHAPES_BF16(X)
#undef X
    return false;
  }
#define X(CI, CO, K)                                                                                           \
  if (cin == CI && k == K) {                                                                                   \
    if constexpr (CI == CO && (CI == 48 || CI == 64)) {                                                        \
      launch_w<CI, K, 512>(st, last, a, grid);                                                                 \
      return true;                                                                                             \
    }                                                                                                          \
  }
  MWW_BLOCK_SHAPES(X)
#undef X
  return false;
}

template <int K1, int C1, int CO, int K, int S>
static bool launch_bwd_firstw_x6(hipStream_t st, const BwdFirstArgs& a, int grid) {
  if constexpr (S == 1 && K1 == 3 && CO <= 64) {
    hipLaunchKernelGGL((bwd_firstw_kernel<K1, C1, CO, K, S, 512, true>), dim3(grid), dim3(512), 0, st, a);
    return true;
  } else {
    return false;
  }
}

bool k_launch_bwd_firstw(hipStream_t st, int k1, int c1, int cout, int k, int stride, const BwdFirstArgs& a, int grid, bool wide_x6) {
#define X(K1, C1, CO, K, S)                                                                                    \
  if (k1 == K1 && c1 == C1 && cout == CO && k == K && stride == S) {                                           \
    if (wide_x6 && launch_bwd_firstw_x6<K1, C1, CO, K, S>(st, a, grid)) return true;                           \
    if constexpr (S > 1) {                                                                                     \
      hipLaunchKernelGGL((bwd_firstw_kernel<K1, C1, CO, K, S, 512>), dim3(grid), dim3(512), 0, st, a);         \
      return true;                                                                                             \
    }                                                                                                          \
  }
  MWW_FIRST_SHAPES(X)
#undef X
  return false;
}

}
```

Measured before the change: 3.497 million.

## Defer DP-stage commit and split next-tile prefetch in backward kernels

Adds a LATE template variant to the backward block and first-block kernels. It splits the next-tile prefetch into two parts: the activation/input loads are issued before the first barrier, and the dP/gradient staging is committed to LDS, with its next load issued, after the depthwise compute phase. The goal is to hide the dP commit and global-load latency behind depthwise work and to shorten the time before the first barrier. The variant is on by default for non-last blocks and the first block, off for the last block, and can be overridden at runtime. It keeps prefetch registers live for longer and adds template instantiations, plus phase-clock instrumentation.

```diff
diff --git a/microwakeword_amd/csrc/block_launch.hip.h b/microwakeword_amd/csrc/block_launch.hip.h
--- a/microwakeword_amd/csrc/block_launch.hip.h
+++ b/microwakeword_amd/csrc/block_launch.hip.h
@@ -27,9 +27,9 @@
 
 bool k_launch_fwd_first(hipStream_t st, int mode, int k1, int c1, int cout, int k, int stride, const FwdFirstArgs& a, int grid, bool x6);
 bool k_launch_fwd_block(hipStream_t st, int mode, int cin, int cout, int k, const FwdBlockArgs& a, int grid);
-bool k_launch_bwd_first(hipStream_t st, int mode, int k1, int c1, int cout, int k, int stride, const BwdFirstArgs& a, int grid, bool x6);
+bool k_launch_bwd_first(hipStream_t st, int mode, int k1, int c1, int cout, int k, int stride, const BwdFirstArgs& a, int grid, bool x6, bool late);
 bool k_launch_bwd_block(hipStream_t st, int mode, int cin, int cout, int k, bool last, const BwdBlockArgs& a, int grid);
-bool k_launch_bwd_blockw(hipStream_t st, int mode, int cin, int cout, int k, bool last, const BwdBlockArgs& a, int grid);
-bool k_launch_bwd_firstw(hipStream_t st, int k1, int c1, int cout, int k, int stride, const BwdFirstArgs& a, int grid, bool wide_x6);
+bool k_launch_bwd_blockw(hipStream_t st, int mode, int cin, int cout, int k, bool last, const BwdBlockArgs& a, int grid, bool late);
+bool k_launch_bwd_firstw(hipStream_t st, int k1, int c1, int cout, int k, int stride, const BwdFirstArgs& a, int grid, bool wide_x6, bool late);
 
 }
diff --git a/microwakeword_amd/csrc/bwd_first_body.inc b/microwakeword_amd/csrc/bwd_first_body.inc
--- a/microwakeword_amd/csrc/bwd_first_body.inc
+++ b/microwakeword_amd/csrc/bwd_first_body.inc
@@ -31,6 +31,8 @@
   const int c = tid % CIN, chunk = tid / CIN;
   const bool dw_active = chunk < NCH;
   const int Ta = (a.T - K1) / S + 1;
+  MWW_PC_DECL
+  MWW_PC_AT(0);
 
   const bool tailmode = TAIL > 0 && Ta > TT && Ta <= TT + TAIL;
   const int ntiles = tailmode ? 1 : (Ta + TT - 1) / TT;
@@ -40,14 +42,17 @@
   DpStage<COUT, false, SB> dps;
   constexpr int NA = (RA * QI + kThreads - 1) / kThreads;
   float4 pre_a[NA];
-  auto issue = [&](int it) {
-    const int s = it / ntiles, b = blockIdx.x + s * gridDim.x, t0 = (it % ntiles) * TT;
-    const int nrx = ((tailmode ? Ta : min(TT, Ta - t0)) - 1) * S + K1;
+  auto issue_a = [&](int it, bool live) {
+    const int s = live ? it / ntiles : nsamp - 1, b = blockIdx.x + s * gridDim.x, t0 = (it % ntiles) * TT;
+    const int nrx = live ? ((tailmode ? Ta : min(TT, Ta - t0)) - 1) * S + K1 : 0;
     xs.issue(a.x, a.xg, sXg, s, b, a.T, t0 * S, nrx, tid);
-    const BufRsrc ra = tile_rsrc(a.a0 + ((size_t)b * Ta + t0) * CIN, min(RA, Ta - t0) * QI * 16);
+    const BufRsrc ra = tile_rsrc(a.a0 + ((size_t)b * Ta + t0) * CIN, live ? min(RA, Ta - t0) * QI * 16 : 0);
 #pragma unroll
     for (int j = 0; j < NA; ++j) pre_a[j] = tile_load4<MWW_AUX_LD_A0>(ra, (tid + j * kThreads) * 16);
-    const int nvk = max(0, min(TT, a.Tout - t0)) * (COUT / 4);
+  };
+  auto issue_b = [&](int it, bool live) {
+    const int b = blockIdx.x + (it / ntiles) * gridDim.x, t0 = (it % ntiles) * TT;
+    const int nvk = live ? max(0, min(TT, a.Tout - t0)) * (COUT / 4) : 0;
     const size_t koff = ((size_t)b * a.Tout + t0) * COUT;
     dps.issue(elem_ptr<SB>(a.pk, koff), elem_ptr<SB>(a.gk, koff), nvk, tid);
   };
@@ -73,7 +78,10 @@
   }
   if (a.xg.win) xgather_setup(a.xg, sXg, nsamp, tid);
   stagger_start<MWW_STAGGER_BWD>();
-  if (nitems > 0) issue(0);
+  if (nitems > 0) {
+    issue_a(0, true);
+    issue_b(0, true);
+  }
 
   WeightStage<CIN, COUT, 0, pitch_wt(CIN, BF)> wst;
   wst.load(a.pw_w, nullptr, tid);
@@ -125,6 +133,8 @@
     for (int nt = 0; nt < NT1; ++nt) w1acc[mi][nt] = zero4();
   __syncthreads();
 
+  MWW_PC_AT(1);
+  MWW_PC_START(MWW_ABLATE(a, 16) && tid == 0);
   for (int it = 0; it < nitems; ++it) {
     rotate_priority(it, 2);
     const int t0 = (it % ntiles) * TT;
@@ -140,10 +150,19 @@
         *reinterpret_cast<float4*>(sA + r * CPI + q * 4) = pre_a[j];
       }
     }
-    dps.commit(sDP, sKp, 0.f, nrows_new * (COUT / 4), tid);
+    MWW_PC_MARK(0);
+    if constexpr (!LATE) dps.commit(sDP, sKp, 0.f, nrows_new * (COUT / 4), tid);
     carry_du<K, CPI>(sDU, t0 == 0, tid);
-    __syncthreads();
-    if (it + 1 < nitems) issue(it + 1);
+    if constexpr (LATE) issue_a(it + 1, it + 1 < nitems);
+    MWW_PC_MARK(LATE ? 0 : 8);
+    __syncthreads();
+    MWW_PC_MARK(1);
+    if constexpr (!LATE) {
+      if (it + 1 < nitems) {
+        issue_a(it + 1, true);
+        issue_b(it + 1, true);
+      }
+    }
     if (dw_active) {
       if (chunk * L < nrows_new) {
         float o[L];
@@ -158,9 +177,18 @@
         for (int t = 0; t < L; ++t) sU[(chunk * L + t) * CPI + c] = 0.f;
       }
     }
-    __syncthreads();
+    MWW_PC_MARK(2);
+    if constexpr (LATE) {
+      dps.commit(sDP, sKp, 0.f, nrows_new * (COUT / 4), tid);
+      issue_b(it + 1, it + 1 < nitems);
+      MWW_PC_MARK(8);
+    }
+    __syncthreads();
+    MWW_PC_MARK(3);
     pointwise_backward_tile<CIN, COUT, K, BF>(sU, sDP, sDU, wave, r16, g, sWt, dwacc, wave * 16 < nrows_new);
-    __syncthreads();
+    MWW_PC_MARK(4);
+    __syncthreads();
+    MWW_PC_MARK(5);
     if (dw_active) {
       float wdu[L + K - 1], wa[L + K - 1];
 #pragma unroll
@@ -205,6 +233,7 @@
         }
       }
     }
+    MWW_PC_MARK(6);
     __syncthreads();
     if constexpr (X6) {
       const char* xb = reinterpret_cast<const char*>(sX);
@@ -267,8 +296,11 @@
         }
       }
     }
-    __syncthreads();
-  }
+    MWW_PC_MARK(7);
+    __syncthreads();
+    MWW_PC_MARK(5);
+  }
+  MWW_PC_AT(2);
   float* gdst = a.grad_part + (size_t)blockIdx.x * (M1 * C1 + (K + 1) * CIN + CIN * COUT);
 #pragma unroll
   for (int mi = 0; mi < MPW; ++mi)
@@ -280,3 +312,5 @@
         if (m < M1) gdst[m * C1 + nt * 16 + r16] = w1acc[mi][nt][r];
       }
   write_block_grad_partials<CIN, COUT, K>(smem, gdst + M1 * C1, dwacc, accw, accb, dw_active, c, chunk, tid, wave, r16, g);
+  MWW_PC_AT(3);
+  MWW_PC_DUMP(a.phase_clk ? a.phase_clk + (size_t)blockIdx.x * kClkSlots : nullptr);
diff --git a/microwakeword_amd/csrc/common.hip.h b/microwakeword_amd/csrc/common.hip.h
--- a/microwakeword_amd/csrc/common.hip.h
+++ b/microwakeword_amd/csrc/common.hip.h
@@ -294,9 +294,10 @@
 #define MWW_PC_MARK(i) ((void)0)
 #define MWW_PC_DUMP(p) ((void)0)
 #endif
-constexpr int kClkSlots = 12;
+constexpr int kClkPhases = 9;
+constexpr int kClkSlots = kClkPhases + 4;
 struct PhaseClock {
-  unsigned long long last = 0, acc[8] = {0, 0, 0, 0, 0, 0, 0, 0}, stamp[4] = {0, 0, 0, 0};
+  unsigned long long last = 0, acc[kClkPhases] = {0, 0, 0, 0, 0, 0, 0, 0, 0}, stamp[4] = {0, 0, 0, 0};
   bool on = false;
   __device__ __forceinline__ void at(int i) { stamp[i] = __builtin_amdgcn_s_memtime(); }
   __device__ __forceinline__ void start(bool enable) {
@@ -312,8 +313,8 @@
   }
   __device__ __forceinline__ void dump(unsigned long long* dst) const {
     if (on) {
-      for (int i = 0; i < 8; ++i) dst[i] = acc[i];
-      for (int i = 0; i < 4; ++i) dst[8 + i] = stamp[i];
+      for (int i = 0; i < kClkPhases; ++i) dst[i] = acc[i];
+      for (int i = 0; i < 4; ++i) dst[kClkPhases + i] = stamp[i];
     }
   }
 };
diff --git a/microwakeword_amd/csrc/engine.hip.h b/microwakeword_amd/csrc/engine.hip.h
--- a/microwakeword_amd/csrc/engine.hip.h
+++ b/microwakeword_amd/csrc/engine.hip.h
@@ -21,6 +21,15 @@
 #endif
 #ifndef MWW_BWD_WIDE_DEFAULT
 #define MWW_BWD_WIDE_DEFAULT 1
+#endif
+#ifndef MWW_DP_COMMIT_LATE_BLOCK_DEFAULT
+#define MWW_DP_COMMIT_LATE_BLOCK_DEFAULT 1
+#endif
+#ifndef MWW_DP_COMMIT_LATE_LAST_DEFAULT
+#define MWW_DP_COMMIT_LATE_LAST_DEFAULT 0
+#endif
+#ifndef MWW_DP_COMMIT_LATE_FIRST_DEFAULT
+#define MWW_DP_COMMIT_LATE_FIRST_DEFAULT 1
 #endif
 
 namespace mww {
@@ -105,6 +114,7 @@
   bool conv1_x6_fwd = MWW_CONV1_X6_FWD_DEFAULT != 0;
   bool bwd_first_wide = MWW_BWD_FIRST_WIDE_DEFAULT != 0;
   bool bwd_wide = MWW_BWD_WIDE_DEFAULT != 0;
+  int dp_commit_late = -1;
   int64_t P = 0, S = 0;
   int64_t o_conv1 = 0, o_dense_w = 0, o_dense_b = 0;
   int t_last = 0, c_last = 0, dwd_stride = 0;
diff --git a/microwakeword_amd/csrc/kernels_bwd.hip.h b/microwakeword_amd/csrc/kernels_bwd.hip.h
--- a/microwakeword_amd/csrc/kernels_bwd.hip.h
+++ b/microwakeword_amd/csrc/kernels_bwd.hip.h
@@ -282,9 +282,11 @@
   int B, T, Tout;
   BnGradFoldArgs gfold;
   XGather xg;
-};
-
-template <int K1, int C1, int COUT, int K, int S, bool BF, bool SB = false, bool X6 = false>
+  int ablate;
+  unsigned long long* phase_clk;
+};
+
+template <int K1, int C1, int COUT, int K, int S, bool BF, bool SB = false, bool X6 = false, bool LATE = false>
 __global__ __launch_bounds__(kThreads, (S > 1 ? 1 : 2)) void bwd_first_kernel(BwdFirstArgs a) {
   typedef BwdFirstLds<K1, C1, COUT, K, S> Lds;
   __shared__ __attribute__((aligned(16))) float sX[X6 ? 3 * Lds::XR * 96 / 4 : Lds::XR * Lds::PX];
diff --git a/microwakeword_amd/csrc/kernels_bwdw.hip.h b/microwakeword_amd/csrc/kernels_bwdw.hip.h
--- a/microwakeword_amd/csrc/kernels_bwdw.hip.h
+++ b/microwakeword_amd/csrc/kernels_bwdw.hip.h
@@ -271,7 +271,7 @@
   return (BwdWideLds<C, K, NTH>::BYTES <= 80 * 1024 ? 2 : 1) * (NTH / 64) / 4;
 }
 
-template <int CIN, int COUT, int K, bool LAST, int NTH, bool BF = false, bool SB = false>
+template <int CIN, int COUT, int K, bool LAST, int NTH, bool BF = false, bool SB = false, bool LATE = false>
 __global__ __launch_bounds__(NTH, (wide_waves_per_simd<CIN, K, NTH>())) void bwd_blockw_kernel(BwdBlockArgs a) {
   static_assert(CIN == COUT, "the wide form is instantiated for square blocks");
   constexpr int C = CIN;
@@ -308,19 +308,25 @@
   float4 pre_p[NP];
   DpStageW<C, LAST, SB, NTH, P> dps;
   float pre_dz = 0.f;
-  auto issue = [&](int it) {
+  auto issue_a = [&](int it, bool live) {
     const int b = blockIdx.x + (it / ntiles) * gridDim.x, t0 = (it % ntiles) * TT;
-    const int nvp = min(RA, a.Tin - t0) * Q;
+    const int nvp = live ? min(RA, a.Tin - t0) * Q : 0;
     const BufRsrc src = tile_rsrc(elem_ptr<SB>(a.in, ((size_t)b * a.Tin + t0) * C), nvp * 4 * elem_bytes(SB));
 #pragma unroll
     for (int j = 0; j < NP; ++j) pre_p[j] = tile_load4s<SB, MWW_AUX_LD_BP>(src, tid + j * NTH);
-    const int nvk = max(0, min(TT, a.Tout - t0)) * Q;
+  };
+  auto issue_b = [&](int it, bool live) {
+    const int b = blockIdx.x + (it / ntiles) * gridDim.x, t0 = (it % ntiles) * TT;
+    const int nvk = live ? max(0, min(TT, a.Tout - t0)) * Q : 0;
     const size_t koff = ((size_t)b * a.Tout + t0) * C;
     dps.issue(elem_ptr<SB>(a.pk, koff), LAST ? a.wd + (size_t)t0 * C : elem_ptr<SB>(a.gk, koff), nvk, tid);
-    if (LAST) pre_dz = tile_load1(tile_rsrc(a.dz, a.B * 4), b * 4);
+    if (LAST) pre_dz = tile_load1(tile_rsrc(a.dz, live ? a.B * 4 : 0), b * 4);
   };
   stagger_start<MWW_STAGGER_BWD>();
-  if (nitems > 0) issue(0);
+  if (nitems > 0) {
+    issue_a(0, true);
+    issue_b(0, true);
+  }
 
   constexpr int NWL = (C * C + NTH - 1) / NTH, NDL = (K * C + NTH - 1) / NTH;
   float wl[NWL], dl[NDL];
@@ -406,12 +412,19 @@
         *reinterpret_cast<float4*>(sP + r * P + q * 4) = v;
       }
     }
-    dps.commit(sDP, sKp, pre_dz, nrows_new * Q, tid);
+    MWW_PC_MARK(0);
+    if constexpr (!LATE) dps.commit(sDP, sKp, pre_dz, nrows_new * Q, tid);
     for (int i = tid; i < (K - 1) * P; i += NTH) sDU[i] = (t0 == 0) ? 0.f : sDU[TT * P + i];
-    MWW_PC_MARK(0);
+    if constexpr (LATE) issue_a(it + 1, it + 1 < nitems);
+    MWW_PC_MARK(LATE ? 0 : 8);
     __syncthreads();
     MWW_PC_MARK(1);
-    if (it + 1 < nitems) issue(it + 1);
+    if constexpr (!LATE) {
+      if (it + 1 < nitems) {
+        issue_a(it + 1, true);
+        issue_b(it + 1, true);
+      }
+    }
     if (dw_active) {
       if (chunk * L < nrows_new) {
         float o[L];
@@ -429,6 +442,11 @@
       }
     }
     MWW_PC_MARK(2);
+    if constexpr (LATE) {
+      dps.commit(sDP, sKp, pre_dz, nrows_new * Q, tid);
+      issue_b(it + 1, it + 1 < nitems);
+      MWW_PC_MARK(8);
+    }
     __syncthreads();
     MWW_PC_MARK(3);
     int r16 = r16_, g = g_;
@@ -568,7 +586,7 @@
   return (BwdFirstWideLds<K1, C1, COUT, K, S, NTH, X6>::BYTES <= 80 * 1024 ? 2 : 1) * (NTH / 64) / 4;
 }
 
-template <int K1, int C1, int COUT, int K, int S, int NTH, bool X6 = false>
+template <int K1, int C1, int COUT, int K, int S, int NTH, bool X6 = false, bool LATE = false>
 __global__ __launch_bounds__(NTH, (wide_first_waves_per_simd<K1, C1, COUT, K, S, NTH, X6>())) void bwd_firstw_kernel(BwdFirstArgs a) {
   typedef BwdFirstWideLds<K1, C1, COUT, K, S, NTH, X6> Lds;
   constexpr bool SB = false;
@@ -607,14 +625,17 @@
   DpStageW<COUT, false, SB, NTH, PO> dps;
   constexpr int NA = (RA * QI + NTH - 1) / NTH;
   float4 pre_a[NA];
-  auto issue = [&](int it) {
-    const int s = it / ntiles, b = blockIdx.x + s * gridDim.x, t0 = (it % ntiles) * TT;
-    const int nrx = ((tailmode ? Ta : min(TT, Ta - t0)) - 1) * S + K1;
+  auto issue_a = [&](int it, bool live) {
+    const int s = live ? it / ntiles : nsamp - 1, b = blockIdx.x + s * gridDim.x, t0 = (it % ntiles) * TT;
+    const int nrx = live ? ((tailmode ? Ta : min(TT, Ta - t0)) - 1) * S + K1 : 0;
     xs.issue(a.x, a.xg, sXg, s, b, a.T, t0 * S, nrx, tid);
-    const BufRsrc ra = tile_rsrc(a.a0 + ((size_t)b * Ta + t0) * CIN, min(RA, Ta - t0) * QI * 16);
+    const BufRsrc ra = tile_rsrc(a.a0 + ((size_t)b * Ta + t0) * CIN, live ? min(RA, Ta - t0) * QI * 16 : 0);
 #pragma unroll
     for (int j = 0; j < NA; ++j) pre_a[j] = tile_load4<MWW_AUX_LD_A0>(ra, (tid + j * NTH) * 16);
-    const int nvk = max(0, min(TT, a.Tout - t0)) * QO;
+  };
+  auto issue_b = [&](int it, bool live) {
+    const int b = blockIdx.x + (it / ntiles) * gridDim.x, t0 = (it % ntiles) * TT;
+    const int nvk = live ? max(0, min(TT, a.Tout - t0)) * QO : 0;
     const size_t koff = ((size_t)b * a.Tout + t0) * COUT;
     dps.issue(elem_ptr<SB>(a.pk, koff), elem_ptr<SB>(a.gk, koff), nvk, tid);
   };
@@ -640,7 +661,10 @@
   }
   if (a.xg.win) xgather_setup(a.xg, sXg, nsamp, tid);
   stagger_start<MWW_STAGGER_BWD>();
-  if (nitems > 0) issue(0);
+  if (nitems > 0) {
+    issue_a(0, true);
+    issue_b(0, true);
+  }
 
   constexpr int NWL = (CIN * COUT + NTH - 1) / NTH;
   float wl[NWL];
@@ -713,10 +737,16 @@
         *reinterpret_cast<float4*>(sA + r * PI + q * 4) = pre_a[j];
       }
     }
-    dps.commit(sDP, sKp, 0.f, nrows_new * QO, tid);
+    if constexpr (!LATE) dps.commit(sDP, sKp, 0.f, nrows_new * QO, tid);
     for (int i = tid; i < (K - 1) * PI; i += NTH) sDU[i] = (t0 == 0) ? 0.f : sDU[TT * PI + i];
+    if constexpr (LATE) issue_a(it + 1, it + 1 < nitems);
     __syncthreads();
-    if (it + 1 < nitems) issue(it + 1);
+    if constexpr (!LATE) {
+      if (it + 1 < nitems) {
+        issue_a(it + 1, true);
+        issue_b(it + 1, true);
+      }
+    }
     if (chunk * L < nrows_new) {
       float o[L];
       dw_chunk<K, L>(sA, PI, chunk * L, c, dww, dwb, o);
@@ -728,6 +758,10 @@
     } else {
 #pragma unroll
       for (int t = 0; t < L; ++t) sU[(chunk * L + t) * PI + c] = 0.f;
+    }
+    if constexpr (LATE) {
+      dps.commit(sDP, sKp, 0.f, nrows_new * QO, tid);
+      issue_b(it + 1, it + 1 < nitems);
     }
     __syncthreads();
     if (wave < 4) {
diff --git a/microwakeword_amd/csrc/mww_lib.hip b/microwakeword_amd/csrc/mww_lib.hip
--- a/microwakeword_amd/csrc/mww_lib.hip
+++ b/microwakeword_amd/csrc/mww_lib.hip
@@ -35,8 +35,9 @@
 }
 
 int launch_bwd_first(mww_ctx* c, int k1, int c1, int cout, int k, int st, const BwdFirstArgs& a, int grid) {
-  if (c->bwd_wide && !c->pw_bf16 && !c->st_bf16 && k_launch_bwd_firstw(c->stream, k1, c1, cout, k, st, a, grid, c->conv1_x6 && c->bwd_first_wide)) return MWW_OK;
-  if (k_launch_bwd_first(c->stream, c->st_bf16 ? 2 : (c->pw_bf16 ? 1 : 0), k1, c1, cout, k, st, a, grid, c->conv1_x6)) return MWW_OK;
+  const bool late = c->dp_commit_late < 0 ? MWW_DP_COMMIT_LATE_FIRST_DEFAULT != 0 : c->dp_commit_late != 0;
+  if (c->bwd_wide && !c->pw_bf16 && !c->st_bf16 && k_launch_bwd_firstw(c->stream, k1, c1, cout, k, st, a, grid, c->conv1_x6 && c->bwd_first_wide, late)) return MWW_OK;
+  if (k_launch_bwd_first(c->stream, c->st_bf16 ? 2 : (c->pw_bf16 ? 1 : 0), k1, c1, cout, k, st, a, grid, c->conv1_x6, late)) return MWW_OK;
   return fail(MWW_ERR_UNSUPPORTED, "no first-block backward kernel for this shape");
 }
 
@@ -47,7 +48,8 @@
 
 int launch_bwd_block(mww_ctx* c, int cin, int cout, int k, bool last, const BwdBlockArgs& a, int grid) {
   const int mode = c->st_bf16 ? 2 : (c->pw_bf16 ? 1 : 0);
-  if (c->bwd_wide && k_launch_bwd_blockw(c->stream, mode, cin, cout, k, last, a, grid)) return MWW_OK;
+  const bool late = c->dp_commit_late < 0 ? (last ? MWW_DP_COMMIT_LATE_LAST_DEFAULT : MWW_DP_COMMIT_LATE_BLOCK_DEFAULT) != 0 : c->dp_commit_late != 0;
+  if (c->bwd_wide && k_launch_bwd_blockw(c->stream, mode, cin, cout, k, last, a, grid, late)) return MWW_OK;
   if (k_launch_bwd_block(c->stream, c->st_bf16 ? 2 : (c->pw_bf16 ? 1 : 0), cin, cout, k, last, a, grid)) return MWW_OK;
   return fail(MWW_ERR_UNSUPPORTED, "no block backward kernel for this shape");
 }
@@ -595,7 +597,8 @@
       if (last) return fail(MWW_ERR_UNSUPPORTED, "single-block models are not supported");
       BwdFirstArgs a{c->x, c->a0, l.p, l.g, bn_slot(l, BN_MEAN), bn_slot(l, BN_RSTD), bn_slot(l, BN_C1),
                      bn_slot(l, BN_MG), bn_slot(l, BN_MGX), c->params + l.o_dw_w, c->params + l.o_dw_b,
-                     c->params + l.o_pw_w, l.grad_part, B, d.frames, l.tout, gf, x_gather(c)};
+                     c->params + l.o_pw_w, l.grad_part, B, d.frames, l.tout, gf, x_gather(c), c->ablate,
+                     c->phase_clk + (size_t)(2 * i + 1) * 2048 * kClkSlots};
       lp.begin("bwd_block", i);
       int rc = launch_bwd_first(c, d.conv1_kernel, d.conv1_filters, l.cout, l.k, d.conv1_stride, a, gbwd);
       lp.end();
@@ -1626,6 +1629,7 @@
   else if (!strcmp(name, "conv1_x6")) c->conv1_x6 = v != 0;
   else if (!strcmp(name, "conv1_x6_fwd")) c->conv1_x6_fwd = v != 0;
   else if (!strcmp(name, "bwd_first_wide")) c->bwd_first_wide = v != 0;
+  else if (!strcmp(name, "dp_commit_late")) { if (v < -1 || v > 1) return fail(MWW_ERR_INVALID, "dp_commit_late must be -1 (per-family defaults), 0 or 1"); c->dp_commit_late = (int)v; }
   else if (!strcmp(name, "grid_fwd")) { if (v < 1 || v > c->n_cu * 4) return fail(MWW_ERR_INVALID, "grid_fwd out of range"); c->grid_fwd = (int)v; }
   else if (!strcmp(name, "grid_bwd")) { if (v < 1 || v > c->n_cu * 2) return fail(MWW_ERR_INVALID, "grid_bwd out of range"); c->grid_bwd = (int)v; }
   else if (!strcmp(name, "grid_graph")) {
diff --git a/microwakeword_amd/csrc/tu_bwd_first.hip b/microwakeword_amd/csrc/tu_bwd_first.hip
--- a/microwakeword_amd/csrc/tu_bwd_first.hip
+++ b/microwakeword_amd/csrc/tu_bwd_first.hip
@@ -4,8 +4,14 @@
 namespace mww {
 
 template <int K1, int C1, int CO, int K, int S, bool BF = false, bool SB = false>
-static bool launch_bwd_first_x6(hipStream_t st, const BwdFirstArgs& a, int grid) {
+static bool launch_bwd_first_x6(hipStream_t st, const BwdFirstArgs& a, int grid, bool late = false) {
   if constexpr (S == 1) {
+    if constexpr (!BF && !SB) {
+      if (late) {
+        hipLaunchKernelGGL((bwd_first_kernel<K1, C1, CO, K, S, BF, SB, true, true>), dim3(grid), dim3(kThreads), 0, st, a);
+        return true;
+      }
+    }
     hipLaunchKernelGGL((bwd_first_kernel<K1, C1, CO, K, S, BF, SB, true>), dim3(grid), dim3(kThreads), 0, st, a);
     return true;
   } else {
@@ -13,7 +19,7 @@
   }
 }
 
-bool k_launch_bwd_first(hipStream_t st, int mode, int k1, int c1, int cout, int k, int stride, const BwdFirstArgs& a, int grid, bool x6) {
+bool k_launch_bwd_first(hipStream_t st, int mode, int k1, int c1, int cout, int k, int stride, const BwdFirstArgs& a, int grid, bool x6, bool late) {
   if (mode != 0) {
 #define X(K1, C1, CO, K, S)                                                                                    \
     if (k1 == K1 && c1 == C1 && cout == CO && k == K && stride == S) {                                         \
@@ -32,7 +38,7 @@
   }
 #define X(K1, C1, CO, K, S)                                                                                    \
   if (k1 == K1 && c1 == C1 && cout == CO && k == K && stride == S) {                                           \
-    if (x6 && launch_bwd_first_x6<K1, C1, CO, K, S>(st, a, grid)) return true;                                 \
+    if (x6 && launch_bwd_first_x6<K1, C1, CO, K, S>(st, a, grid, late)) return true;                              \
     hipLaunchKernelGGL((bwd_first_kernel<K1, C1, CO, K, S, false>), dim3(grid), dim3(kThreads), 0, st, a);     \
     return true;                                                                                               \
   }
diff --git a/microwakeword_amd/csrc/tu_bwdw.hip b/microwakeword_amd/csrc/tu_bwdw.hip
--- a/microwakeword_amd/csrc/tu_bwdw.hip
+++ b/microwakeword_amd/csrc/tu_bwdw.hip
@@ -4,10 +4,10 @@
 
 namespace mww {
 
-template <int C, int K, int NTH>
+template <int C, int K, int NTH, bool LATE>
 static void launch_w(hipStream_t st, bool last, const BwdBlockArgs& a, int grid) {
-  if (last) hipLaunchKernelGGL((bwd_blockw_kernel<C, C, K, true, NTH>), dim3(grid), dim3(NTH), 0, st, a);
-  else hipLaunchKernelGGL((bwd_blockw_kernel<C, C, K, false, NTH>), dim3(grid), dim3(NTH), 0, st, a);
+  if (last) hipLaunchKernelGGL((bwd_blockw_kernel<C, C, K, true, NTH, false, false, LATE>), dim3(grid), dim3(NTH), 0, st, a);
+  else hipLaunchKernelGGL((bwd_blockw_kernel<C, C, K, false, NTH, false, false, LATE>), dim3(grid), dim3(NTH), 0, st, a);
 }
 template <int C, int K, int NTH>
 static void launch_w_bf16(hipStream_t st, int mode, bool last, const BwdBlockArgs& a, int grid) {
@@ -20,7 +20,7 @@
   }
 }
 
-bool k_launch_bwd_blockw(hipStream_t st, int mode, int cin, int cout, int k, bool last, const BwdBlockArgs& a, int grid) {
+bool k_launch_bwd_blockw(hipStream_t st, int mode, int cin, int cout, int k, bool last, const BwdBlockArgs& a, int grid, bool late) {
   if (cin != cout) return false;
   if (mode != 0) {
 #define X(CI, CO, K)                                                                                           \
@@ -37,7 +37,8 @@
 #define X(CI, CO, K)                                                                                           \
   if (cin == CI && k == K) {                                                                                   \
     if constexpr (CI == CO && (CI == 48 || CI == 64)) {                                                        \
-      launch_w<CI, K, 512>(st, last, a, grid);                                                                 \
+      if (late) launch_w<CI, K, 512, true>(st, last, a, grid);                                                 \
+      else launch_w<CI, K, 512, false>(st, last, a, grid);                                                     \
       return true;                                                                                             \
     }                                                                                                          \
   }
@@ -47,21 +48,23 @@
 }
 
 template <int K1, int C1, int CO, int K, int S>
-static bool launch_bwd_firstw_x6(hipStream_t st, const BwdFirstArgs& a, int grid) {
+static bool launch_bwd_firstw_x6(hipStream_t st, const BwdFirstArgs& a, int grid, bool late) {
   if constexpr (S == 1 && K1 == 3 && CO <= 64) {
-    hipLaunchKernelGGL((bwd_firstw_kernel<K1, C1, CO, K, S, 512, true>), dim3(grid), dim3(512), 0, st, a);
+    if (late) hipLaunchKernelGGL((bwd_firstw_kernel<K1, C1, CO, K, S, 512, true, true>), dim3(grid), dim3(512), 0, st, a);
+    else hipLaunchKernelGGL((bwd_firstw_kernel<K1, C1, CO, K, S, 512, true>), dim3(grid), dim3(512), 0, st, a);
     return true;
   } else {
     return false;
   }
 }
 
-bool k_launch_bwd_firstw(hipStream_t st, int k1, int c1, int cout, int k, int stride, const BwdFirstArgs& a, int grid, bool wide_x6) {
+bool k_launch_bwd_firstw(hipStream_t st, int k1, int c1, int cout, int k, int stride, const BwdFirstArgs& a, int grid, bool wide_x6, bool late) {
 #define X(K1, C1, CO, K, S)                                                                                    \
   if (k1 == K1 && c1 == C1 && cout == CO && k == K && stride == S) {                                           \
-    if (wide_x6 && launch_bwd_firstw_x6<K1, C1, CO, K, S>(st, a, grid)) return true;                           \
+    if (wide_x6 && launch_bwd_firstw_x6<K1, C1, CO, K, S>(st, a, grid, late)) return true;                     \
     if constexpr (S > 1) {                                                                                     \
-      hipLaunchKernelGGL((bwd_firstw_kernel<K1, C1, CO, K, S, 512>), dim3(grid), dim3(512), 0, st, a);         \
+      if (late) hipLaunchKernelGGL((bwd_firstw_kernel<K1, C1, CO, K, S, 512, false, true>), dim3(grid), dim3(512), 0, st, a); \
+      else hipLaunchKernelGGL((bwd_firstw_kernel<K1, C1, CO, K, S, 512>), dim3(grid), dim3(512), 0, st, a);    \
       return true;                                                                                             \
     }                                                                                                          \
   }
```

Result: faster. 3.541 million, median of 6 (+1.3%).
